# aerius-labs/indexed-merkle-tree-halo2

Hardware: AMD Instinct MI355X
Metric: indexed-tree insertions/sec at depth=32 (bn256::Fr) (higher is better)
Workload: dtype u32 limbs (9 x 29-bit, Montgomery mod p), 64-bit accumulate

## Files before the change

### indexed-merkle-tree-halo2_amd/csrc/imt_device.hpp

```cpp
#pragma once
#include <cstddef>
#include <cstdint>
#include "imt_consts.hpp"

#if defined(__HIPCC__)
#include <hip/hip_runtime.h>
#define IMT_HD __host__ __device__ __forceinline__
#else
#define IMT_HD inline
#endif

namespace imt {
namespace dev {

#define IMT_P29_0 0x10000001u
#define IMT_P29_1 0x1f0fac9fu
#define IMT_P29_2 0x0e5c2450u
#define IMT_P29_3 0x07d090f3u
#define IMT_P29_4 0x1585d283u
#define IMT_P29_5 0x02db40c0u
#define IMT_P29_6 0x00a6e141u
#define IMT_P29_7 0x0e5c2634u
#define IMT_P29_8 0x0030644eu
constexpr uint32_t N0INV29 = 0x0fffffffu;
constexpr uint32_t N0INV32 = 0xefffffffu;

IMT_HD constexpr uint32_t p29(int i) {
    return i == 0 ? IMT_P29_0 : i == 1 ? IMT_P29_1 : i == 2 ? IMT_P29_2 : i == 3 ? IMT_P29_3 :
           i == 4 ? IMT_P29_4 : i == 5 ? IMT_P29_5 : i == 6 ? IMT_P29_6 : i == 7 ? IMT_P29_7 : IMT_P29_8;
}


template <bool WIDE_M>
IMT_HD uint32_t mont_digit(uint64_t acc) {
    return WIDE_M ? (uint32_t)acc * N0INV32 : (((uint32_t)acc * N0INV29) & MASK29);
}

}
}
#if defined(__HIP_DEVICE_COMPILE__) && !defined(IMT_NO_MONT_ASM)
#define IMT_MONT_ASM 1
#include "imt_mont_asm.hpp"
#include "imt_mont_asm_rec.hpp"
#endif
namespace imt {
namespace dev {

template <int NT, bool ADD, bool WIDE_M = true>
IMT_HD void mont_dot(Fe& r, const Fe* a, const Fe* b, const Fe& addend) {
    uint32_t m[NL];
    uint64_t acc = 0;
#pragma unroll
    for (int k = 0; k < NL; k++) {
#pragma unroll
        for (int t = 0; t < NT; t++) {
#pragma unroll
            for (int i = 0; i <= k; i++) acc += (uint64_t)a[t].v[i] * b[t].v[k - i];
        }
#pragma unroll
        for (int i = 0; i < k; i++) acc += (uint64_t)m[i] * p29(k - i);
        m[k] = mont_digit<WIDE_M>(acc);
        acc += (uint64_t)m[k] * p29(0);
        acc >>= 29;
    }
#pragma unroll
    for (int k = NL; k < 2 * NL - 1; k++) {
#pragma unroll
        for (int t = 0; t < NT; t++) {
#pragma unroll
            for (int i = k - (NL - 1); i < NL; i++) acc += (uint64_t)a[t].v[i] * b[t].v[k - i];
        }
#pragma unroll
        for (int i = k - (NL - 1); i < NL; i++) acc += (uint64_t)m[i] * p29(k - i);
        if (ADD) acc += addend.v[k - NL];
        r.v[k - NL] = (uint32_t)acc & MASK29;
        acc >>= 29;
    }
    if (ADD) acc += addend.v[NL - 1];
    r.v[NL - 1] = (uint32_t)acc;
}

IMT_HD void mont_mul(Fe& r, const Fe& a, const Fe& b) {
#ifdef IMT_MONT_ASM
    masm::mul_vv(r, &a, &b);
#else
    mont_dot<1, false>(r, &a, &b, a);
#endif
}

template <int NT, bool ADD, bool WIDE_M = true>
IMT_HD void mont_dot_uc(Fe& r, const Fe* c, const Fe* v, const Fe& addend) {
#ifdef IMT_MONT_ASM
    static_assert((NT == 3 && !ADD && WIDE_M) || (NT == 4 && WIDE_M) || (NT == 2 && ADD && !WIDE_M),
                  "no assembly form for this shape");
    if constexpr (NT == 3) masm::dot3_uc(r, c, v);
    else if constexpr (NT == 4 && ADD) masm::dot4_add_uc(r, c, v, addend);
    else if constexpr (NT == 4) masm::dot4_uc(r, c, v);
    else masm::dot2_add_uc_narrow(r, c, v, addend);
#else
    mont_dot<NT, ADD, WIDE_M>(r, c, v, addend);
#endif
}

IMT_HD void mont_sqr(Fe& r, const Fe& a) {
#ifdef IMT_MONT_ASM
    masm::sqr_v(r, a);
    return;
#endif
    uint32_t m[NL], a2[NL];
#pragma unroll
    for (int i = 0; i < NL; i++) a2[i] = a.v[i] << 1;
    uint64_t acc = 0;
#pragma unroll
    for (int k = 0; k < NL; k++) {
#pragma unroll
        for (int i = 0; 2 * i < k; i++) acc += (uint64_t)a2[i] * a.v[k - i];
        if ((k & 1) == 0) acc += (uint64_t)a.v[k / 2] * a.v[k / 2];
#pragma unroll
        for (int i = 0; i < k; i++) acc += (uint64_t)m[i] * p29(k - i);
        m[k] = mont_digit<true>(acc);
        acc += (uint64_t)m[k] * p29(0);
        acc >>= 29;
    }
#pragma unroll
    for (int k = NL; k < 2 * NL - 1; k++) {
#pragma unroll
        for (int i = k - (NL - 1); 2 * i < k; i++) acc += (uint64_t)a2[i] * a.v[k - i];
        if ((k & 1) == 0) acc += (uint64_t)a.v[k / 2] * a.v[k / 2];
#pragma unroll
        for (int i = k - (NL - 1); i < NL; i++) acc += (uint64_t)m[i] * p29(k - i);
        r.v[k - NL] = (uint32_t)acc & MASK29;
        acc >>= 29;
    }
    r.v[NL - 1] = (uint32_t)acc;
}

IMT_HD void mont_redc(Fe& r, const Fe& a) {
    uint32_t m[NL];
    uint64_t acc = 0;
#pragma unroll
    for (int k = 0; k < NL; k++) {
        acc += a.v[k];
#pragma unroll
        for (int i = 0; i < k; i++) acc += (uint64_t)m[i] * p29(k - i);
        m[k] = mont_digit<false>(acc);
        acc += (uint64_t)m[k] * p29(0);
        acc >>= 29;
    }
#pragma unroll
    for (int k = NL; k < 2 * NL - 1; k++) {
#pragma unroll
        for (int i = k - (NL - 1); i < NL; i++) acc += (uint64_t)m[i] * p29(k - i);
        r.v[k - NL] = (uint32_t)acc & MASK29;
        acc >>= 29;
    }
    r.v[NL - 1] = (uint32_t)acc;
}

IMT_HD void add_lazy(Fe& r, const Fe& a, const Fe& b) {
#pragma unroll
    for (int i = 0; i < NL; i++) r.v[i] = a.v[i] + b.v[i];
}

IMT_HD void normalize(Fe& a) {
#pragma unroll
    for (int i = 0; i < NL - 1; i++) {
        a.v[i + 1] += a.v[i] >> 29;
        a.v[i] &= MASK29;
    }
}

IMT_HD bool geq_p(const Fe& a) {
    bool ge = true;
#pragma unroll
    for (int i = 0; i < NL; i++) {
        uint32_t pi = p29(i);
        if (a.v[i] != pi) ge = a.v[i] > pi;
    }
    return ge;
}

IMT_HD void sub_p(Fe& a) {
    uint32_t borrow = 0;
#pragma unroll
    for (int i = 0; i < NL; i++) {
        uint32_t d = a.v[i] - p29(i) - borrow;
        borrow = (i < NL - 1) ? (d >> 31) : 0;
        a.v[i] = (i < NL - 1) ? (d & MASK29) : d;
    }
}

template <int SH>
IMT_HD constexpr uint32_t p29_shl(int i) {
    return i == 0 ? ((p29(0) << SH) & MASK29)
         : i < NL - 1 ? (((p29(i) << SH) | (p29(i - 1) >> (29 - SH))) & MASK29)
                      : ((p29(i) << SH) | (p29(i - 1) >> (29 - SH)));
}
template <int SH>
IMT_HD void cond_sub_p_shl(Fe& a) {
    bool ge = true;
#pragma unroll
    for (int i = 0; i < NL; i++) {
        const uint32_t pi = p29_shl<SH>(i);
        if (a.v[i] != pi) ge = a.v[i] > pi;
    }
    if (ge) {
        uint32_t borrow = 0;
#pragma unroll
        for (int i = 0; i < NL; i++) {
            uint32_t d = a.v[i] - p29_shl<SH>(i) - borrow;
            borrow = (i < NL - 1) ? (d >> 31) : 0;
            a.v[i] = (i < NL - 1) ? (d & MASK29) : d;
        }
    }
}

IMT_HD void canonicalize(Fe& a) {
    cond_sub_p_shl<4>(a);
    cond_sub_p_shl<3>(a);
    cond_sub_p_shl<2>(a);
    cond_sub_p_shl<1>(a);
    cond_sub_p_shl<0>(a);
}

IMT_HD void unpack(Fe& r, const uint32_t w[8]) {
#pragma unroll
    for (int i = 0; i < NL; i++) {
        const int bit = 29 * i, wi = bit >> 5, sh = bit & 31;
        uint32_t lo = w[wi] >> sh;
        if (sh > 3 && wi + 1 < 8) lo |= w[wi + 1] << (32 - sh);
        r.v[i] = lo & MASK29;
    }
}
IMT_HD void pack(uint32_t w[8], const Fe& a) {
#pragma unroll
    for (int j = 0; j < 8; j++) {
        const int lo_limb = (32 * j) / 29, off = 32 * j - 29 * lo_limb;
        uint32_t x = a.v[lo_limb] >> off;
        const int have = 29 - off;
        if (have < 32 && lo_limb + 1 < NL) x |= a.v[lo_limb + 1] << have;
        if (have + 29 < 32 && lo_limb + 2 < NL) x |= a.v[lo_limb + 2] << (have + 29);
        w[j] = x;
    }
}

struct alignas(16) Word4 { uint32_t x, y, z, w; };
IMT_HD void load_packed(Fe& r, const void* ptr) {
    const Word4* q = reinterpret_cast<const Word4*>(ptr);
    Word4 x = q[0], y = q[1];
    uint32_t w[8] = {x.x, x.y, x.z, x.w, y.x, y.y, y.z, y.w};
    unpack(r, w);
}
IMT_HD void store_packed(void* ptr, const Fe& a) {
    uint32_t w[8];
    pack(w, a);
    Word4* q = reinterpret_cast<Word4*>(ptr);
    q[0] = Word4{w[0], w[1], w[2], w[3]};
    q[1] = Word4{w[4], w[5], w[6], w[7]};
}



IMT_HD void sbox(Fe& x) {
    Fe x2, x4;
    mont_sqr(x2, x);
    mont_sqr(x4, x2);
    mont_mul(x, x4, x);
}

IMT_HD constexpr uint32_t pc29(int i) { return i == 0 ? (1u << 29) - p29(0) : MASK29 - p29(i); }
constexpr uint32_t FOLD_RECIP = 1354;

IMT_HD void fold_p(Fe& a) {
    const uint32_t q = (uint32_t)(((uint64_t)a.v[NL - 1] * FOLD_RECIP) >> 32);
    uint64_t acc = 0;
#pragma unroll
    for (int i = 0; i < NL; i++) {
        acc = (acc >> 29) + a.v[i] + (uint64_t)q * pc29(i);
        a.v[i] = i < NL - 1 ? (uint32_t)acc & MASK29 : (uint32_t)(acc - ((uint64_t)q << 29));
    }
}

IMT_HD void permute(const PoseidonConsts& pc, Fe s[3], const Fe* first_rc) {
    constexpr int NSTEP = RF + RP;
    Fe z3;
#pragma unroll
    for (int i = 0; i < NL; i++) z3.v[i] = 0;
#pragma unroll 1
    for (int st = 0; st < NSTEP; st++) {
        if (st < RF / 2 || st >= RF / 2 + RP) {
            const int fr = st < RF / 2 ? st : st - RP;
            if (fr == RF / 2) {
                const Fe v[3] = {s[0], s[1], z3};
                const Fe zl = s[2];
#pragma unroll 1
                for (int i = 0; i < 2; i++) {
                    Fe n;
                    mont_dot_uc<3, false>(n, pc.rec_exit[i], v, v[0]);
                    add_lazy(n, n, zl);
                    normalize(n);
                    s[1] = s[2]; s[2] = n;
                }
            }
            const Fe* rc = (st == 0) ? first_rc : pc.sc_rc[fr];
            add_lazy(s[0], s[0], rc[0]);
            add_lazy(s[1], s[1], rc[1]);
            add_lazy(s[2], s[2], rc[2]);
            sbox(s[0]); sbox(s[1]); sbox(s[2]);
            const Fe(*mat)[3] = pc.sc_mats[fr];
            Fe n0, n1, n2;
            if (fr == 0 || fr == RF / 2) {
                mont_dot_uc<3, false>(n0, mat[0], s, s[0]);
            } else {
                add_lazy(n0, s[0], s[1]);
                add_lazy(n0, n0, s[2]);
                normalize(n0);
            }
            mont_dot_uc<3, false>(n1, mat[1], s, s[0]);
            mont_dot_uc<3, false>(n2, mat[2], s, s[0]);
            s[0] = n0; s[1] = n1; s[2] = n2;
        } else {
            const int r = st - RF / 2;
            Fe z, w;
            add_lazy(z, s[0], pc.rec_k[r]);
            sbox(z);
            if (r >= 2) {
                const Fe v[4] = {s[0], s[1], z3, s[2]};
                mont_dot_uc<4, true>(w, pc.rec_c[r], v, z);
            } else if (r == 1) {
                const Fe v[2] = {s[0], s[2]};
                Fe e;
                add_lazy(e, z3, z);
                mont_dot_uc<2, true, false>(w, pc.rec_c[1], v, e);
            } else {
                add_lazy(w, s[1], z);
                normalize(w);
            }
            s[1] = s[0]; s[0] = w; z3 = s[2]; s[2] = z;
        }
    }
}

IMT_HD void hash23(const PoseidonConsts& pc, Fe& out, const Fe& a, const Fe& b, const Fe& c, bool three) {
    Fe s[3] = {pc.cap0, a, b};
#pragma unroll 1
    for (int blk = 0; blk < 2; blk++) {
        const Fe* rc0 = pc.rc_full[0];
        if (blk == 1) {
            if (three) {
                add_lazy(s[1], s[1], c);
                add_lazy(s[2], s[2], pc.one);
                normalize(s[1]);
                normalize(s[2]);
            } else {
                rc0 = pc.rc_h2p2;
            }
        }
        permute(pc, s, rc0);
    }
    out = s[1];
    canonicalize(out);
}
IMT_HD void hash23_stashed(const PoseidonConsts& pc, Fe& out, const Fe& a, const Fe& b, bool three,
                           const uint32_t* stash, unsigned stride) {
    Fe s[3] = {pc.cap0, a, b};
#pragma unroll 1
    for (int blk = 0; blk < 2; blk++) {
        const Fe* rc0 = pc.rc_full[0];
        if (blk == 1) {
            if (three) {
                Fe c;
#pragma unroll
                for (int i = 0; i < NL; i++) c.v[i] = stash[(size_t)i * stride];
                add_lazy(s[1], s[1], c);
                add_lazy(s[2], s[2], pc.one);
                normalize(s[1]);
                normalize(s[2]);
            } else {
                rc0 = pc.rc_h2p2;
            }
        }
        permute(pc, s, rc0);
    }
    out = s[1];
    canonicalize(out);
}
template <class LoadInput>
IMT_HD void hash_sponge(const PoseidonConsts& pc, Fe& out, unsigned len, LoadInput load) {
    Fe s[3];
    s[0] = pc.cap0;
#pragma unroll
    for (int i = 0; i < NL; i++) s[1].v[i] = s[2].v[i] = 0;
    const unsigned full = len >> 1;
#pragma unroll 1
    for (unsigned ch = 0; ch <= full; ch++) {
        const Fe* rc0 = pc.rc_full[0];
        if (ch < full || (len & 1u)) {
            Fe x;
            load(2 * ch, x);
            add_lazy(s[1], s[1], x);
            normalize(s[1]);
            if (ch < full) load(2 * ch + 1, x);
            else x = pc.one;
            add_lazy(s[2], s[2], x);
            normalize(s[2]);
        } else {
            rc0 = pc.rc_h2p2;
        }
        permute(pc, s, rc0);
    }
    out = s[1];
    canonicalize(out);
}
IMT_HD void hash2(const PoseidonConsts& pc, Fe& out, const Fe& a, const Fe& b) { hash23(pc, out, a, b, a, false); }
IMT_HD void hash3(const PoseidonConsts& pc, Fe& out, const Fe& a, const Fe& b, const Fe& c) { hash23(pc, out, a, b, c, true); }

enum : unsigned { FMT_CANONICAL = 0, FMT_MONT256 = 1, FMT_DEVICE = 2 };

IMT_HD bool load_fe(const PoseidonConsts& pc, Fe& r, const void* ptr, unsigned fmt) {
    Fe raw;
    load_packed(raw, ptr);
    bool ok = !geq_p(raw) && (raw.v[NL - 1] >> 24) == 0;
    if (fmt == FMT_DEVICE) { r = raw; return ok; }
    mont_mul(r, raw, fmt == FMT_CANONICAL ? pc.from_canon : pc.from_mont256);
    canonicalize(r);
    return ok;
}
IMT_HD void store_fe(const PoseidonConsts& pc, void* ptr, const Fe& a, unsigned fmt) {
    if (fmt == FMT_DEVICE) { store_packed(ptr, a); return; }
    Fe t;
    mont_mul(t, a, fmt == FMT_CANONICAL ? pc.int_one : pc.to_mont256);
    canonicalize(t);
    store_packed(ptr, t);
}

IMT_HD bool fe_eq(const Fe& a, const Fe& b) {
    uint32_t d = 0;
#pragma unroll
    for (int i = 0; i < NL; i++) d |= a.v[i] ^ b.v[i];
    return d == 0;
}
IMT_HD bool fe_is_zero(const Fe& a) {
    uint32_t d = 0;
#pragma unroll
    for (int i = 0; i < NL; i++) d |= a.v[i];
    return d == 0;
}

}
}
```

### indexed-merkle-tree-halo2_amd/csrc/imt_kernels.hip

```cpp
#include <algorithm>
#include <hip/hip_runtime.h>
#include <hip/hip_ext.h>

#include "imt_device.hpp"
#include "imt_trace_device.hpp"
#include "imt_launch.hpp"
#include "imt_sweep.hpp"
#include "imt_resize.hpp"
#if defined(__HIP_DEVICE_COMPILE__)
#include "imt_coop_device.hpp"
#endif

namespace imt {

__constant__ dev::PoseidonConsts g_pc;
__constant__ dev::TraceConsts g_tc;

namespace {
using namespace dev;

#ifndef IMT_BLOCK
#define IMT_BLOCK 256
#endif
#ifndef IMT_HASH_WAVES
#define IMT_HASH_WAVES __attribute__((amdgpu_waves_per_eu(5, 5)))
#endif
#ifndef IMT_COOP_WAVES
#define IMT_COOP_WAVES __attribute__((amdgpu_waves_per_eu(1, 2)))
#endif
constexpr int BLOCK = IMT_BLOCK;

__device__ __forceinline__ size_t gtid() { return (size_t)blockIdx.x * blockDim.x + threadIdx.x; }
__device__ __forceinline__ size_t gtid_again() {
    uint32_t lo = blockIdx.x * blockDim.x + threadIdx.x, hi = (uint32_t)(((uint64_t)blockIdx.x * blockDim.x + threadIdx.x) >> 32);
    asm volatile("" : "+v"(lo), "+v"(hi));
    return ((size_t)hi << 32) | lo;
}
__device__ __forceinline__ void flag_err(int* err, bool ok) {
    if (!ok && err) atomicOr(err, 1);
}

__device__ __forceinline__ void to_int(Fe& r, const Fe& a) {
    mont_mul(r, a, g_pc.int_one);
    canonicalize(r);
}
__device__ __forceinline__ bool int_lt(const Fe& a, const Fe& b) {
    bool lt = false;
#pragma unroll
    for (int i = 0; i < NL; i++) {
        if (a.v[i] != b.v[i]) lt = a.v[i] < b.v[i];
    }
    return lt;
}
__device__ __forceinline__ void fe_from_u64(Fe& r, uint64_t x) {
    Fe t;
#pragma unroll
    for (int i = 0; i < NL; i++) t.v[i] = 0;
    t.v[0] = (uint32_t)x & MASK29;
    t.v[1] = (uint32_t)(x >> 29) & MASK29;
    t.v[2] = (uint32_t)(x >> 58);
    mont_mul(r, t, g_pc.from_canon);
    canonicalize(r);
}

__device__ __forceinline__ void order_pair(Fe& A, Fe& B, bool right, const Fe& cur, const Fe& sv) {
#pragma unroll
    for (int i = 0; i < NL; i++) {
        A.v[i] = right ? sv.v[i] : cur.v[i];
        B.v[i] = right ? cur.v[i] : sv.v[i];
    }
}
__device__ __forceinline__ void store_proof_row(const launch::SweepArgs& a, uint32_t e, const Fe& sv) {
    uint8_t* row = (e & 1u) ? a.new_sib : a.low_sib;
    if (row) store_fe(g_pc, row + ((uint64_t)a.level * a.lay.level_stride + (uint64_t)(e >> 1) * a.lay.item_stride) * 32, sv, a.fmt_out);
}
struct InsertRows {
    __device__ __forceinline__ void operator()(const launch::SweepArgs& a, uint32_t e, const Fe& sv) const { store_proof_row(a, e, sv); }
};
struct MixedRows {
    const uint32_t* erow;
    uint8_t* read_sib;
    __device__ __forceinline__ void operator()(const launch::SweepArgs& a, uint32_t e, const Fe& sv) const {
        const uint32_t w = erow[e], kind = w & 3u;
        uint8_t* row = kind == 0u ? a.low_sib : (kind == 1u ? a.new_sib : read_sib);
        if (row) store_fe(g_pc, row + ((uint64_t)a.level * a.lay.level_stride + (uint64_t)(w >> 2) * a.lay.item_stride) * 32, sv, a.fmt_out);
    }
};

struct NoLevelHook {
    __device__ __forceinline__ void operator()(unsigned, const Fe&, const Fe&) const {}
    __device__ __forceinline__ void operator()(unsigned, const Fe&) const {}
};
struct NoLeafHook {
    __device__ __forceinline__ void operator()(const Fe&) const {}
};
template <class LoadLeaf, class OnLeaf = NoLeafHook, class OnLevel = NoLevelHook>
__device__ __forceinline__ void chain_inline(Fe& cur, bool with_leaf, LoadLeaf load_leaf, OnLeaf on_leaf,
                                             const uint64_t* __restrict__ index, uint64_t flip, const uint8_t* sib,
                                             launch::SibLayout lay, unsigned depth, unsigned fmt_in, bool& ok, uint32_t* stash,
                                             OnLevel on_level = OnLevel()) {
#pragma unroll 1
    for (int it = with_leaf ? -1 : 0; it < (int)depth; it++) {
        Fe A, B;
        const bool three = it < 0;
        if (three) {
            Fe C;
            load_leaf(A, B, C, ok);
#pragma unroll
            for (int i = 0; i < NL; i++) stash[(size_t)i * BLOCK] = C.v[i];
        } else {
            const size_t item = gtid_again();
            Fe sv;
            ok &= load_fe(g_pc, sv, sib + ((uint64_t)it * lay.level_stride + item * lay.item_stride) * 32, fmt_in);
            order_pair(A, B, ((index[item] ^ flip) >> it) & 1, cur, sv);
            on_level((unsigned)it, A, B);
        }
        hash23_stashed(g_pc, cur, A, B, three, stash, BLOCK);
        if (three) on_leaf(cur);
    }
}
struct LeafAt {
    const uint8_t* base;
    unsigned fmt_in;
    __device__ __forceinline__ void operator()(Fe& a, Fe& b, Fe& c, bool& ok) const {
        const uint8_t* p = base + gtid_again() * 96;
        ok &= load_fe(g_pc, a, p, fmt_in);
        ok &= load_fe(g_pc, b, p + 32, fmt_in);
        ok &= load_fe(g_pc, c, p + 64, fmt_in);
    }
};

#if defined(__HIP_DEVICE_COMPILE__)
__device__ __forceinline__ bool leaf_inputs_quad(Fe& X, Fe& C3, const uint8_t* p, unsigned fmt, unsigned ri) {
    Fe seen;
    bool ok = load_fe(g_pc, X, p + (ri == 2u ? 32 : 0), fmt);
    ok &= load_fe(g_pc, C3, p + 64, fmt);
    if (ri == 1u) ok &= load_fe(g_pc, seen, p + 32, fmt);
    return ok;
}
__device__ __forceinline__ void pick_input(Fe& X, unsigned ri, bool right, const Fe& cur, const Fe& sv) {
    coop::sel(X, (ri == 2u) != right, sv, cur);
}
__device__ __forceinline__ void hash_to_quad(const uint32_t* tab, Fe& cur, const Fe& X, const Fe& C3, bool three, unsigned ri) {
    Fe o;
    coop::hash23(tab, o, X, C3, three, ri);
    coop::quad_bcast<1>(cur, o);
}
__device__ __forceinline__ void leaf_start_quad(const uint32_t* tab, Fe& cur, const uint8_t* p, unsigned fmt, unsigned ri, bool& ok) {
    Fe X, C3;
    ok &= leaf_inputs_quad(X, C3, p, fmt, ri);
    hash_to_quad(tab, cur, X, C3, true, ri);
}
template <class OnLevel = NoLevelHook>
__device__ __forceinline__ void chain_quad(const uint32_t* tab, Fe& cur, uint64_t idx, const uint8_t* sib, launch::SibLayout lay,
                                           size_t item, unsigned depth, unsigned fmt_in, unsigned ri, bool& ok,
                                           OnLevel on_level = OnLevel()) {
#pragma unroll 1
    for (unsigned l = 0; l < depth; l++) {
        Fe sv, X;
        ok &= load_fe(g_pc, sv, sib + ((uint64_t)l * lay.level_stride + item * lay.item_stride) * 32, fmt_in);
        pick_input(X, ri, (idx >> l) & 1, cur, sv);
        on_level(l, X);
        hash_to_quad(tab, cur, X, X, false, ri);
    }
}
#endif

__global__ IMT_HASH_WAVES void __launch_bounds__(BLOCK) k_hash_batch(const uint8_t* __restrict__ in, uint8_t* __restrict__ out,
                                                      size_t n, int arity, unsigned fmt_in, unsigned fmt_out,
                                                      int* err) {
    const size_t i = gtid();
    if (i >= n) return;
    const uint8_t* p = in + i * 32 * (size_t)arity;
    __shared__ uint32_t stash[NL][BLOCK];
    Fe a, b, o;
    bool ok = load_fe(g_pc, a, p, fmt_in);
    ok &= load_fe(g_pc, b, p + 32, fmt_in);
    if (arity == 3) {
        Fe c;
        ok &= load_fe(g_pc, c, p + 64, fmt_in);
#pragma unroll
        for (int q = 0; q < NL; q++) stash[q][threadIdx.x] = c.v[q];
    }
    hash23_stashed(g_pc, o, a, b, arity == 3, &stash[0][threadIdx.x], BLOCK);
    store_fe(g_pc, out + i * 32, o, fmt_out);
    flag_err(err, ok);
}

__global__ IMT_HASH_WAVES void __launch_bounds__(BLOCK) k_hash_batch_coop(const uint8_t* __restrict__ in, uint8_t* __restrict__ out,
                                                           size_t n, int arity, unsigned fmt_in, unsigned fmt_out,
                                                           int* err) {
#if defined(__HIP_DEVICE_COMPILE__)
    __shared__ uint32_t tab[coop::TAB_DWORDS];
    coop::tab_fill(tab, g_pc);
    const size_t t = gtid();
    const size_t i = t >> 2;
    if (i >= n) return;
    const unsigned role = (unsigned)t & 3u, ri = role == 3u ? 0u : role;
    const uint8_t* p = in + i * 32 * (size_t)arity;
    Fe X, C3, o;
    C3 = g_pc.one;
    bool ok = load_fe(g_pc, X, p + (ri == 2u ? 32 : 0), fmt_in);
    if (ri == 1u) ok &= load_fe(g_pc, o, p + 32, fmt_in);
    if (arity == 3) ok &= load_fe(g_pc, C3, p + 64, fmt_in);
    coop::hash23(tab, o, X, C3, arity == 3, ri);
    if (role == 1u) store_fe(g_pc, out + i * 32, o, fmt_out);
    flag_err(err, ok);
#endif
}

__global__ void __launch_bounds__(BLOCK) k_permute_batch(const uint8_t* __restrict__ in, uint8_t* __restrict__ out,
                                                         size_t n, unsigned fmt_in, unsigned fmt_out, int* err) {
    const size_t i = gtid();
    if (i >= n) return;
    Fe s[3];
    bool ok = true;
#pragma unroll
    for (int j = 0; j < 3; j++) ok &= load_fe(g_pc, s[j], in + (i * 3 + j) * 32, fmt_in);
    permute(g_pc, s, g_pc.rc_full[0]);
#pragma unroll
    for (int j = 0; j < 3; j++) {
        canonicalize(s[j]);
        store_fe(g_pc, out + (i * 3 + j) * 32, s[j], fmt_out);
    }
    flag_err(err, ok);
}

__global__ void __launch_bounds__(BLOCK) k_convert(const uint8_t* __restrict__ in, uint8_t* __restrict__ out, size_t n,
                                                   unsigned fmt_in, unsigned fmt_out, int* err) {
    const size_t i = gtid();
    if (i >= n) return;
    Fe x;
    bool ok = load_fe(g_pc, x, in + i * 32, fmt_in);
    store_fe(g_pc, out + i * 32, x, fmt_out);
    flag_err(err, ok);
}

#ifndef IMT_TRACE_WAVES
#define IMT_TRACE_WAVES
#endif
template <unsigned FMT_OUT>
__global__ IMT_TRACE_WAVES void __launch_bounds__(BLOCK) k_hash_trace(launch::TraceJobs a) {
    const launch::TraceJobs::Job jb = a.j[blockIdx.y];
    const size_t q = gtid();
    if (q >= jb.n_items) return;
    const uint8_t* p = jb.in + q * 32 * (size_t)jb.arity;
    Fe x, y, z;
    bool ok = load_fe(g_pc, x, p, jb.fmt_in);
    ok &= load_fe(g_pc, y, p + 32, jb.fmt_in);
    z = x;
    if (jb.arity == 3) ok &= load_fe(g_pc, z, p + 64, jb.fmt_in);
    const size_t l = q / a.n_per, i = q - l * a.n_per;
    const size_t first = jb.row0 + l * (size_t)(jb.arity == 3 ? TRACE_ROWS_H3 : TRACE_ROWS_H2);
    TraceSink o{a.item_major ? a.trace + (i * a.rows_total + first) * 32 : a.trace + (first * a.n_per + i) * 32,
                a.item_major ? (uint64_t)32 : (uint64_t)a.n_per * 32};
    hash_trace<FMT_OUT>(g_pc, g_tc, o, x, y, z, jb.arity == 3);
    flag_err(a.err, ok);
}

__global__ __attribute__((amdgpu_waves_per_eu(4, 5))) void __launch_bounds__(BLOCK) k_path_pairs(launch::PathChains a) {
    const size_t i = gtid();
    if (i >= a.n) return;
    const launch::PathChains::Chain ch = a.c[blockIdx.y];
    __shared__ uint32_t stash[NL][BLOCK];
    bool ok = true;
    Fe cur;
    if (!ch.leaf3) ok &= load_fe(g_pc, cur, ch.leaf + i * 32, a.fmt_in);
    uint8_t* const pairs = ch.pairs;
    const size_t n = a.n;
    auto store_pair = [pairs, n](unsigned l, const Fe& x, const Fe& y) {
        uint8_t* dst = pairs + ((size_t)l * n + gtid_again()) * 64;
        store_packed(dst, x);
        store_packed(dst + 32, y);
    };
    chain_inline(cur, ch.leaf3 != nullptr, LeafAt{ch.leaf3, a.fmt_in}, NoLeafHook(), ch.index, 0, ch.sib, a.lay, a.depth,
                 a.fmt_in, ok, &stash[0][threadIdx.x], store_pair);
    if (ch.root_out) store_fe(g_pc, ch.root_out + gtid_again() * 32, cur, a.fmt_out);
    flag_err(a.err, ok);
}

__global__ IMT_COOP_WAVES void __launch_bounds__(BLOCK) k_path_pairs_coop(launch::PathChains a) {
#if defined(__HIP_DEVICE_COMPILE__)
    __shared__ uint32_t tab[coop::TAB_DWORDS];
    coop::tab_fill(tab, g_pc);
    const size_t t = gtid();
    const size_t i = t >> 2;
    if (i >= a.n) return;
    const launch::PathChains::Chain ch = a.c[blockIdx.y];
    const unsigned role = (unsigned)t & 3u, ri = role == 3u ? 0u : role;
    bool ok = true;
    Fe cur;
    if (ch.leaf3) leaf_start_quad(tab, cur, ch.leaf3 + i * 96, a.fmt_in, ri, ok);
    else ok &= load_fe(g_pc, cur, ch.leaf + i * 32, a.fmt_in);
    uint8_t* const pairs = ch.pairs;
    const size_t n = a.n;
    auto store_input = [pairs, n, i, role](unsigned l, const Fe& X) {
        if (role == 1u || role == 2u) store_packed(pairs + ((size_t)l * n + i) * 64 + (role == 2u ? 32 : 0), X);
    };
    chain_quad(tab, cur, ch.index[i], ch.sib, a.lay, i, a.depth, a.fmt_in, ri, ok, store_input);
    if (role == 1u && ch.root_out) store_fe(g_pc, ch.root_out + i * 32, cur, a.fmt_out);
    flag_err(a.err, ok);
#endif
}

__global__ void __launch_bounds__(BLOCK)
k_insert_trace_inputs(const uint8_t* __restrict__ low_leaf, const uint8_t* __restrict__ new_leaf,
                      const uint64_t* __restrict__ new_index, size_t n, uint8_t* __restrict__ new_low,
                      uint8_t* __restrict__ zero_leaf, unsigned fmt, int* err) {
    const size_t i = gtid();
    if (i >= n) return;
    Fe a, b, c;
    bool ok = load_fe(g_pc, a, low_leaf + (i * 3 + 0) * 32, fmt);
    ok &= load_fe(g_pc, b, new_leaf + (i * 3 + 0) * 32, fmt);
    fe_from_u64(c, new_index[i]);
    store_fe(g_pc, new_low + (i * 3 + 0) * 32, a, fmt);
    store_fe(g_pc, new_low + (i * 3 + 1) * 32, b, fmt);
    store_fe(g_pc, new_low + (i * 3 + 2) * 32, c, fmt);
    store_fe(g_pc, zero_leaf + i * 32, g_pc.zero_leaf, fmt);
    flag_err(err, ok);
}

__global__ IMT_HASH_WAVES void __launch_bounds__(BLOCK)
k_path_root(const uint8_t* __restrict__ leaf, const uint8_t* __restrict__ leaf3, const uint64_t* __restrict__ index,
            int is_helper, const uint8_t* __restrict__ sib, launch::SibLayout lay, unsigned depth, size_t n,
            uint8_t* __restrict__ root_out, const uint8_t* __restrict__ expect, unsigned expect_stride,
            uint8_t* __restrict__ ok_out, unsigned fmt_in, unsigned fmt_out, int* err) {
    const size_t i0 = gtid();
    if (i0 >= n) return;
    __shared__ uint32_t stash[NL][BLOCK];
    bool ok = true;
    Fe cur;
    if (!leaf3) ok &= load_fe(g_pc, cur, leaf + i0 * 32, fmt_in);
    chain_inline(cur, leaf3 != nullptr, LeafAt{leaf3, fmt_in}, NoLeafHook(), index, is_helper ? ~(uint64_t)0 : 0, sib, lay, depth,
                 fmt_in, ok, &stash[0][threadIdx.x]);
    const size_t i = gtid_again();
    if (root_out) store_fe(g_pc, root_out + i * 32, cur, fmt_out);
    if (ok_out) {
        Fe e;
        ok &= load_fe(g_pc, e, expect + i * (size_t)expect_stride, fmt_in);
        ok_out[i] = fe_eq(cur, e) ? 1 : 0;
    }
    flag_err(err, ok);
}

__global__ IMT_COOP_WAVES void __launch_bounds__(BLOCK)
k_path_root_coop(const uint8_t* __restrict__ leaf, const uint8_t* __restrict__ leaf3, const uint64_t* __restrict__ index,
                 int is_helper, const uint8_t* __restrict__ sib, launch::SibLayout lay, unsigned depth, size_t n,
                 uint8_t* __restrict__ root_out, const uint8_t* __restrict__ expect, unsigned expect_stride,
                 uint8_t* __restrict__ ok_out, unsigned fmt_in, unsigned fmt_out, int* err) {
#if defined(__HIP_DEVICE_COMPILE__)
    __shared__ uint32_t tab[coop::TAB_DWORDS];
    coop::tab_fill(tab, g_pc);
    const size_t t = gtid();
    const size_t i = t >> 2;
    if (i >= n) return;
    const unsigned role = (unsigned)t & 3u, ri = role == 3u ? 0u : role;
    bool ok = true;
    Fe cur;
    if (leaf3) leaf_start_quad(tab, cur, leaf3 + i * 96, fmt_in, ri, ok);
    else ok &= load_fe(g_pc, cur, leaf + i * 32, fmt_in);
    chain_quad(tab, cur, is_helper ? ~index[i] : index[i], sib, lay, i, depth, fmt_in, ri, ok);
    if (role == 1u) {
        if (root_out) store_fe(g_pc, root_out + i * 32, cur, fmt_out);
        if (ok_out) {
            Fe e;
            ok &= load_fe(g_pc, e, expect + i * (size_t)expect_stride, fmt_in);
            ok_out[i] = fe_eq(cur, e) ? 1 : 0;
        }
    }
    flag_err(err, ok);
#endif
}

__device__ __forceinline__ unsigned range_fail(const Fe& low_val, const Fe& low_next, const Fe& new_val, const uint8_t* is_largest) {
    Fe nvi, lvi, lni;
    to_int(nvi, new_val); to_int(lvi, low_val); to_int(lni, low_next);
    const unsigned s = *is_largest;
    unsigned fail = 0;
    if (s > 1) fail |= 0x80;
    if (!(s ? fe_is_zero(low_next) : int_lt(nvi, lni))) fail |= 0x01;
    if (!int_lt(lvi, nvi)) fail |= 0x04;
    return fail;
}
__global__ IMT_HASH_WAVES void __launch_bounds__(BLOCK)
k_non_membership(const uint8_t* __restrict__ root, unsigned root_stride, const uint8_t* __restrict__ low_leaf,
                 const uint64_t* __restrict__ low_index, const uint8_t* __restrict__ sib, launch::SibLayout lay,
                 unsigned depth, const uint8_t* __restrict__ new_val, const uint8_t* __restrict__ is_largest,
                 size_t n, uint8_t* __restrict__ fail_out, uint8_t* __restrict__ root_out, unsigned fmt_in,
                 unsigned fmt_out, int* err) {
    const size_t i0 = gtid();
    if (i0 >= n) return;
    bool ok = true;
    unsigned fail = 0;
    __shared__ uint32_t stash[NL][BLOCK];
    Fe cur;
    chain_inline(cur, true, LeafAt{low_leaf, fmt_in}, NoLeafHook(), low_index, 0, sib, lay, depth, fmt_in, ok,
                 &stash[0][threadIdx.x]);
    const size_t i = gtid_again();
    {
        Fe rt;
        ok &= load_fe(g_pc, rt, root + i * (size_t)root_stride, fmt_in);
        if (!fe_eq(cur, rt)) fail |= 0x02;
    }
    if (root_out) store_fe(g_pc, root_out + i * 32, cur, fmt_out);
    fail_out[i] = (uint8_t)fail;
    flag_err(err, ok);
}
__global__ void __launch_bounds__(BLOCK)
k_non_membership_pred(const uint8_t* __restrict__ low_leaf, const uint8_t* __restrict__ new_val, const uint8_t* __restrict__ is_largest,
                      size_t n, uint8_t* __restrict__ fail_out, unsigned fmt_in, int* err) {
    const size_t i = gtid();
    if (i >= n) return;
    Fe v, nx, nv;
    bool ok = load_fe(g_pc, v, low_leaf + (i * 3 + 0) * 32, fmt_in);
    ok &= load_fe(g_pc, nx, low_leaf + (i * 3 + 1) * 32, fmt_in);
    ok &= load_fe(g_pc, nv, new_val + i * 32, fmt_in);
    fail_out[i] |= (uint8_t)range_fail(v, nx, nv, is_largest + i);
    flag_err(err, ok);
}

__global__ IMT_COOP_WAVES void __launch_bounds__(BLOCK)
k_non_membership_coop(const uint8_t* __restrict__ root, unsigned root_stride, const uint8_t* __restrict__ low_leaf,
                      const uint64_t* __restrict__ low_index, const uint8_t* __restrict__ sib, launch::SibLayout lay,
                      unsigned depth, const uint8_t* __restrict__ new_val, const uint8_t* __restrict__ is_largest,
                      size_t n, uint8_t* __restrict__ fail_out, uint8_t* __restrict__ root_out, unsigned fmt_in,
                      unsigned fmt_out, int* err) {
#if defined(__HIP_DEVICE_COMPILE__)
    __shared__ uint32_t tab[coop::TAB_DWORDS];
    coop::tab_fill(tab, g_pc);
    const size_t t = gtid();
    const size_t i = t >> 2;
    if (i >= n) return;
    const unsigned role = (unsigned)t & 3u, ri = role == 3u ? 0u : role;
    bool ok = true;
    unsigned fail;
    {
        Fe v, nx, nv;
        ok &= load_fe(g_pc, v, low_leaf + (i * 3 + 0) * 32, fmt_in);
        ok &= load_fe(g_pc, nx, low_leaf + (i * 3 + 1) * 32, fmt_in);
        ok &= load_fe(g_pc, nv, new_val + i * 32, fmt_in);
        fail = range_fail(v, nx, nv, is_largest + i);
    }
    Fe cur;
    leaf_start_quad(tab, cur, low_leaf + i * 96, fmt_in, ri, ok);
    chain_quad(tab, cur, low_index[i], sib, lay, i, depth, fmt_in, ri, ok);
    if (role == 1u) {
        Fe rt;
        ok &= load_fe(g_pc, rt, root + i * (size_t)root_stride, fmt_in);
        if (!fe_eq(cur, rt)) fail |= 0x02;
        fail_out[i] = (uint8_t)fail;
        if (root_out) store_fe(g_pc, root_out + i * 32, cur, fmt_out);
    }
    flag_err(err, ok);
#endif
}

__global__ void __launch_bounds__(BLOCK) k_split128(const uint8_t* __restrict__ vals, uint8_t* __restrict__ q,
                                                    uint8_t* __restrict__ r, size_t n, unsigned fmt, int* err) {
    const size_t i = gtid();
    if (i >= n) return;
    Fe x, xi;
    bool ok = load_fe(g_pc, x, vals + i * 32, fmt);
    to_int(xi, x);
    uint32_t w[8];
    pack(w, xi);
    Fe lo, hi, t;
    const uint32_t wl[8] = {w[0], w[1], w[2], w[3], 0, 0, 0, 0};
    const uint32_t wh[8] = {w[4], w[5], w[6], w[7], 0, 0, 0, 0};
    unpack(t, wl);
    mont_mul(lo, t, g_pc.from_canon);
    canonicalize(lo);
    unpack(t, wh);
    mont_mul(hi, t, g_pc.from_canon);
    canonicalize(hi);
    store_fe(g_pc, r + i * 32, lo, fmt);
    store_fe(g_pc, q + i * 32, hi, fmt);
    flag_err(err, ok);
}

__global__ IMT_HASH_WAVES void __launch_bounds__(BLOCK)
k_insert_chains(const uint8_t* __restrict__ low_leaf, const uint64_t* __restrict__ low_index,
                const uint8_t* __restrict__ low_sib, const uint8_t* __restrict__ new_leaf,
                const uint64_t* __restrict__ new_index, const uint64_t* __restrict__ new_path_index,
                const uint8_t* __restrict__ new_sib, launch::SibLayout lay, unsigned depth, size_t n,
                uint8_t* __restrict__ trace, unsigned fmt_in, int* err) {
    const size_t i = gtid();
    if (i >= n) return;
    const int chain = blockIdx.y;
    __shared__ uint32_t stash[NL][BLOCK];
    bool ok = true;
    Fe cur;
    const uint8_t* sib = chain < 2 ? low_sib : new_sib;
    const uint64_t* index = chain < 2 ? low_index : new_path_index;
    const int leaf_row = chain == 0 ? 0 : chain == 1 ? 2 : 5, root_row = chain == 0 ? 1 : chain == 1 ? 3 : chain == 2 ? 4 : 6;
    if (chain == 2) cur = g_pc.zero_leaf;
    auto load_leaf = [=](Fe& a, Fe& b, Fe& c, bool& okk) {
        const size_t it = gtid_again();
        const uint8_t* const p0 = (chain == 3 ? new_leaf : low_leaf) + it * 96;
        okk &= load_fe(g_pc, a, p0, fmt_in);
        if (chain == 1) {
            okk &= load_fe(g_pc, b, new_leaf + it * 96, fmt_in);
            fe_from_u64(c, new_index[it]);
        } else {
            okk &= load_fe(g_pc, b, p0 + 32, fmt_in);
            okk &= load_fe(g_pc, c, p0 + 64, fmt_in);
        }
    };
    auto store_leaf = [=](const Fe& h) { store_packed(trace + ((size_t)leaf_row * n + gtid_again()) * 32, h); };
    chain_inline(cur, chain != 2, load_leaf, store_leaf, index, 0, sib, lay, depth, fmt_in, ok, &stash[0][threadIdx.x]);
    store_packed(trace + ((size_t)root_row * n + gtid_again()) * 32, cur);
    flag_err(err, ok);
}

__global__ IMT_COOP_WAVES void __launch_bounds__(BLOCK)
k_insert_chains_coop(const uint8_t* __restrict__ low_leaf, const uint64_t* __restrict__ low_index,
                     const uint8_t* __restrict__ low_sib, const uint8_t* __restrict__ new_leaf,
                     const uint64_t* __restrict__ new_index, const uint64_t* __restrict__ new_path_index,
                     const uint8_t* __restrict__ new_sib, launch::SibLayout lay, unsigned depth, size_t n,
                     uint8_t* __restrict__ trace, unsigned fmt_in, int* err) {
#if defined(__HIP_DEVICE_COMPILE__)
    __shared__ uint32_t tab[coop::TAB_DWORDS];
    coop::tab_fill(tab, g_pc);
    const size_t t = gtid();
    const size_t i = t >> 2;
    if (i >= n) return;
    const unsigned role = (unsigned)t & 3u, ri = role == 3u ? 0u : role;
    const int chain = blockIdx.y;
    bool ok = true;
    const uint8_t* sib = chain < 2 ? low_sib : new_sib;
    const uint64_t idx = chain < 2 ? low_index[i] : new_path_index[i];
    uint8_t* leaf_out = nullptr;
    uint8_t* root_out;
    Fe cur;
    if (chain == 2) {
        cur = g_pc.zero_leaf;
        root_out = trace + (4 * n + i) * 32;
    } else {
        Fe X, C3;
        if (chain == 1) {
            ok &= load_fe(g_pc, X, (ri == 2u ? new_leaf : low_leaf) + (i * 3 + 0) * 32, fmt_in);
            fe_from_u64(C3, new_index[i]);
            leaf_out = trace + (2 * n + i) * 32;
            root_out = trace + (3 * n + i) * 32;
        } else {
            const uint8_t* lf = chain == 0 ? low_leaf : new_leaf;
            ok &= leaf_inputs_quad(X, C3, lf + i * 96, fmt_in, ri);
            leaf_out = trace + ((chain == 0 ? 0 : 5) * n + i) * 32;
            root_out = trace + ((chain == 0 ? 1 : 6) * n + i) * 32;
        }
        hash_to_quad(tab, cur, X, C3, true, ri);
        if (role == 1u) store_packed(leaf_out, cur);
    }
    chain_quad(tab, cur, idx, sib, lay, i, depth, fmt_in, ri, ok);
    if (role == 1u) store_packed(root_out, cur);
    flag_err(err, ok);
#endif
}

__global__ void __launch_bounds__(BLOCK)
k_insert_check(const uint8_t* __restrict__ old_root, const uint8_t* __restrict__ low_leaf,
               const uint8_t* __restrict__ new_root, const uint8_t* __restrict__ new_leaf,
               const uint8_t* __restrict__ is_largest, size_t n, const uint8_t* __restrict__ trace,
               uint8_t* __restrict__ fail_out, unsigned fmt_in, int* err) {
    const size_t i = gtid();
    if (i >= n) return;
    bool ok = true;
    Fe low[3], nl[3], r0, r1, t;
#pragma unroll
    for (int j = 0; j < 3; j++) {
        ok &= load_fe(g_pc, low[j], low_leaf + (i * 3 + j) * 32, fmt_in);
        ok &= load_fe(g_pc, nl[j], new_leaf + (i * 3 + j) * 32, fmt_in);
    }
    ok &= load_fe(g_pc, r0, old_root + i * 32, fmt_in);
    ok &= load_fe(g_pc, r1, new_root + i * 32, fmt_in);
    unsigned fail = range_fail(low[0], low[1], nl[0], is_largest + i);
    load_packed(t, trace + (1 * n + i) * 32);
    if (!fe_eq(t, r0)) fail |= 0x02;
    Fe interim, z;
    load_packed(interim, trace + (3 * n + i) * 32);
    load_packed(z, trace + (4 * n + i) * 32);
    if (!fe_eq(z, interim)) fail |= 0x08;
    if (!fe_eq(nl[1], low[1])) fail |= 0x10;
    if (!fe_eq(nl[2], low[2])) fail |= 0x20;
    load_packed(t, trace + (6 * n + i) * 32);
    if (!fe_eq(t, r1)) fail |= 0x40;
    fail_out[i] = (uint8_t)fail;
    flag_err(err, ok);
}

__global__ IMT_HASH_WAVES void __launch_bounds__(BLOCK) k_tree_level(const uint8_t* __restrict__ prev, uint8_t* __restrict__ next,
                                                      size_t n_parents) {
    const size_t i = gtid();
    if (i >= n_parents) return;
    Fe a, b, o;
    load_packed(a, prev + (2 * i) * 32);
    load_packed(b, prev + (2 * i + 1) * 32);
    hash23_stashed(g_pc, o, a, b, false, nullptr, 0);
    store_packed(next + i * 32, o);
}

__global__ IMT_HASH_WAVES void __launch_bounds__(BLOCK) k_index_leaves(const uint8_t* __restrict__ val,
                                                        const uint32_t* __restrict__ sorted, uint32_t M, uint64_t base,
                                                        uint8_t* __restrict__ tree0, int* err) {
    const size_t r = gtid();
    if (r >= M) return;
    __shared__ uint32_t stash[NL][BLOCK];
    Fe a, b, o;
    bool ok;
    {
        const bool last = r + 1 == M;
        const uint32_t su = last ? 0u : sorted[r + 1];
        Fe c;
        fe_from_u64(c, last ? 0 : base + su);
#pragma unroll
        for (int q = 0; q < NL; q++) stash[q][threadIdx.x] = c.v[q];
        ok = load_fe(g_pc, b, val + (size_t)su * 32, FMT_CANONICAL);
    }
    ok &= load_fe(g_pc, a, val + (size_t)sorted[r] * 32, FMT_CANONICAL);
    hash23_stashed(g_pc, o, a, b, true, &stash[0][threadIdx.x], BLOCK);
    store_packed(tree0 + (size_t)sorted[gtid_again()] * 32, o);
    flag_err(err, ok);
}

__device__ __forceinline__ void force_vector(Fe& x) {
#pragma unroll
    for (int i = 0; i < NL; i++) asm volatile("" : "+v"(x.v[i]));
}

__global__ IMT_HASH_WAVES void k_zero_chain(uint8_t* out, unsigned depth) {
#if defined(__HIP_DEVICE_COMPILE__)
    __shared__ uint32_t tab[coop::TAB_DWORDS];
    coop::tab_fill(tab, g_pc);
    if (blockIdx.x != 0 || threadIdx.x >= 4) return;
    const unsigned role = threadIdx.x, ri = role == 3u ? 0u : role;
    Fe cur = g_pc.zero_leaf;
    force_vector(cur);
    if (role == 1u) store_packed(out, cur);
#pragma unroll 1
    for (unsigned l = 0; l < depth; l++) {
        Fe o;
        coop::hash23(tab, o, cur, cur, false, ri);
        coop::quad_bcast<1>(cur, o);
        if (role == 1u) store_packed(out + (size_t)(l + 1) * 32, cur);
    }
#endif
}

__global__ IMT_HASH_WAVES void k_extend_root(uint8_t* cur_io, const uint8_t* zero, unsigned from, unsigned to) {
    if (threadIdx.x != 0 || blockIdx.x != 0) return;
    Fe cur;
    load_packed(cur, cur_io);
    force_vector(cur);
#pragma unroll 1
    for (unsigned l = from; l < to; l++) {
        Fe z, o;
        load_packed(z, zero + (size_t)l * 32);
        hash23_stashed(g_pc, o, cur, z, false, nullptr, 0);
        cur = o;
    }
    store_packed(cur_io, cur);
}

__global__ void __launch_bounds__(BLOCK) k_gather_proof(launch::TreeView tv, const uint64_t* __restrict__ index,
                                                        size_t n, unsigned depth, uint8_t* __restrict__ out,
                                                        launch::SibLayout lay, unsigned fmt_out) {
    const size_t t = gtid();
    if (t >= n * depth) return;
    const size_t i = t % n;
    const unsigned l = (unsigned)(t / n);
    const uint64_t s = ((index[i] - tv.index_base) >> l) ^ 1;
    const uint8_t* src = s < tv.len[l] ? tv.nodes + (tv.off[l] + s) * 32 : tv.zero + (size_t)l * 32;
    Fe x;
    load_packed(x, src);
    store_fe(g_pc, out + ((uint64_t)l * lay.level_stride + i * lay.item_stride) * 32, x, fmt_out);
}

__global__ void k_write_helpers(uint64_t index, unsigned depth, uint8_t* out, unsigned fmt_out) {
    const unsigned l = threadIdx.x + blockIdx.x * blockDim.x;
    if (l >= depth) return;
    Fe x;
    fe_from_u64(x, ((index >> l) & 1) ? 0 : 1);
    store_fe(g_pc, out + (size_t)l * 32, x, fmt_out);
}


__global__ void __launch_bounds__(BLOCK) k_fill_level(uint8_t* __restrict__ nodes, size_t n,
                                                      const uint8_t* __restrict__ zero_l) {
    const size_t i = gtid();
    if (i >= n) return;
    const Word4* z = reinterpret_cast<const Word4*>(zero_l);
    Word4* o = reinterpret_cast<Word4*>(nodes + i * 32);
    o[0] = z[0];
    o[1] = z[1];
}

__global__ void __launch_bounds__(BLOCK) k_restride_levels(const uint8_t* __restrict__ old_nodes,
                                                           const uint64_t* __restrict__ old_off,
                                                           const uint64_t* __restrict__ old_len,
                                                           uint8_t* __restrict__ new_nodes,
                                                           const uint64_t* __restrict__ new_off, uint64_t new_total,
                                                           const uint8_t* __restrict__ zero, unsigned depth) {
    const size_t pieces = (size_t)new_total * 2, step = (size_t)gridDim.x * blockDim.x;
    for (size_t p = gtid(); p < pieces; p += step) {
        unsigned l;
        const uint64_t src = resize::source_of(new_off, old_off, old_len, depth, p >> 1, &l);
        const uint8_t* row = src != ~(uint64_t)0 ? old_nodes + src * 32 : zero + (size_t)l * 32;
        reinterpret_cast<Word4*>(new_nodes)[p] = reinterpret_cast<const Word4*>(row)[p & 1];
    }
}

__global__ void __launch_bounds__(BLOCK) k_merge_level(sweep::LevelTable in, sweep::LevelOut out, uint32_t total) {
    const size_t k = gtid();
    if (k >= total) return;
    sweep::merge_element(in, out, (uint32_t)k, total);
}

__global__ void __launch_bounds__(BLOCK)
k_writeback(const uint8_t* __restrict__ val_l, const uint32_t* __restrict__ from,
            const uint32_t* __restrict__ node_below, uint8_t* __restrict__ tree_l, uint32_t total) {
    const size_t kp = gtid();
    if (kp >= total) return;
    const uint32_t f = from[kp];
    if (!(f & sweep::LAST_BIT)) return;
    const Word4* s = reinterpret_cast<const Word4*>(val_l + (size_t)(f & ~sweep::LAST_BIT) * 32);
    Word4* d = reinterpret_cast<Word4*>(tree_l + (size_t)node_below[kp] * 32);
    d[0] = s[0];
    d[1] = s[1];
}

struct StoredSibling {
    __device__ __forceinline__ const uint8_t* operator()(const launch::SweepArgs& a, int32_t ss, uint64_t sn) const {
        return ss >= 0 ? a.val_in + (size_t)ss * 32 : (sn < a.len_l ? a.tree_l + sn * 32 : a.zero_l);
    }
};
struct ViewSibling {
    const view::Side& side;
    __device__ __forceinline__ const uint8_t* operator()(const launch::SweepArgs& a, int32_t ss, uint64_t sn) const {
        return replay::sibling_row(side, ss, a.level, sn, a.val_in, a.tree_l, a.len_l, a.zero_l);
    }
};
#if defined(__HIP_DEVICE_COMPILE__)
template <bool TABLES, class Sibling, class Rows = InsertRows>
__device__ __forceinline__ void sweep_body_quad(const launch::SweepArgs& a, Sibling sibling, uint32_t* tab, Rows rows = Rows()) {
    coop::tab_fill(tab, g_pc);
    const size_t t = gtid();
    const size_t q = t >> 2;
    if (q >= a.count) return;
    const unsigned role = (unsigned)t & 3u, ri = role == 3u ? 0u : role;
    const uint32_t x = a.begin + (uint32_t)q;
    const bool leaves = !TABLES && a.mode == launch::SWEEP_LEAVES;
    Fe X, C3, o;
    C3 = g_pc.one;
    if (leaves) {
        flag_err(a.err, leaf_inputs_quad(X, C3, a.pre + (size_t)a.time0[x] * 96, a.fmt_in, ri));
    } else {
        uint32_t k = x, n = 0, e = x;
        const uint8_t* sp = a.zero_l;
        if (TABLES || a.from) {
            k = a.from[x] & ~sweep::LAST_BIT;
            n = a.node_below[x];
            e = a.time_next[x];
            sp = sibling(a, a.sibsrc[x], (uint64_t)(n ^ 1u));
        }
        Fe cur, sv;
        load_packed(cur, a.val_in + (size_t)k * 32);
        load_packed(sv, sp);
        pick_input(X, ri, n & 1u, cur, sv);
        if (role == 0u) {
            if (!TABLES && x == a.last_event && a.node_in) store_packed(a.node_in, cur);
            rows(a, e, sv);
        }
    }
    coop::hash23(tab, o, X, C3, leaves, ri);
    if (role == 1u) {
        store_packed(a.val_out + (size_t)x * 32, o);
        if (!TABLES && x == a.last_event && a.node_out) store_packed(a.node_out, o);
    }
}
#endif
__global__ IMT_HASH_WAVES void __launch_bounds__(BLOCK) k_sweep(launch::SweepArgs a) {
    __shared__ uint32_t stash[NL][BLOCK];
    const size_t t = gtid();
    if (t >= a.count) return;
    const uint32_t x = a.begin + (uint32_t)t;
    Fe A, B, o;
    if (a.mode == launch::SWEEP_LEAVES) {
        const uint8_t* p = a.pre + (size_t)a.time0[x] * 96;
        Fe C;
        bool ok = load_fe(g_pc, A, p, a.fmt_in);
        ok &= load_fe(g_pc, B, p + 32, a.fmt_in);
        ok &= load_fe(g_pc, C, p + 64, a.fmt_in);
#pragma unroll
        for (int i = 0; i < NL; i++) stash[i][threadIdx.x] = C.v[i];
        flag_err(a.err, ok);
    } else {
        uint32_t k = x, n = 0, e = x;
        const uint8_t* sp = a.zero_l;
        if (a.from) {
            k = a.from[x] & ~sweep::LAST_BIT;
            n = a.node_below[x];
            e = a.time_next[x];
            const int32_t ss = a.sibsrc[x];
            const uint64_t sn = (uint64_t)(n ^ 1u);
            sp = ss >= 0 ? a.val_in + (size_t)ss * 32 : (sn < a.len_l ? a.tree_l + sn * 32 : a.zero_l);
        }
        Fe cur, sv;
        load_packed(cur, a.val_in + (size_t)k * 32);
        load_packed(sv, sp);
        if (x == a.last_event && a.node_in) store_packed(a.node_in, cur);
        const bool right = n & 1u;
#pragma unroll
        for (int i = 0; i < NL; i++) {
            A.v[i] = right ? sv.v[i] : cur.v[i];
            B.v[i] = right ? cur.v[i] : sv.v[i];
        }
        uint8_t* row = (e & 1u) ? a.new_sib : a.low_sib;
        if (row) store_fe(g_pc, row + ((uint64_t)a.level * a.lay.level_stride + (uint64_t)(e >> 1) * a.lay.item_stride) * 32, sv, a.fmt_out);
    }
    hash23_stashed(g_pc, o, A, B, a.mode == launch::SWEEP_LEAVES, &stash[0][threadIdx.x], BLOCK);
    store_packed(a.val_out + (size_t)x * 32, o);
    if (x == a.last_event && a.node_out) store_packed(a.node_out, o);
}

__global__ IMT_HASH_WAVES void __launch_bounds__(BLOCK) k_sweep_coop(launch::SweepArgs a) {
#if defined(__HIP_DEVICE_COMPILE__)
    __shared__ uint32_t tab[coop::TAB_DWORDS];
    sweep_body_quad<false>(a, StoredSibling(), tab);
#endif
}

__global__ IMT_HASH_WAVES void __launch_bounds__(BLOCK) k_sweep_mixed(launch::SweepMixedArgs m) {
    const launch::SweepArgs& a = m.sweep;
    const size_t t = gtid();
    if (t >= a.count) return;
    const uint32_t x = a.begin + (uint32_t)t;
    uint32_t k = x, n = 0, e = x;
    const uint8_t* sp = a.zero_l;
    if (a.from) {
        k = a.from[x] & ~sweep::LAST_BIT;
        n = a.node_below[x];
        e = a.time_next[x];
        sp = StoredSibling()(a, a.sibsrc[x], (uint64_t)(n ^ 1u));
    }
    Fe A, B, o, cur, sv;
    load_packed(cur, a.val_in + (size_t)k * 32);
    load_packed(sv, sp);
    if (x == a.last_event && a.node_in) store_packed(a.node_in, cur);
    order_pair(A, B, n & 1u, cur, sv);
    MixedRows{m.erow, m.read_sib}(a, e, sv);
    hash23_stashed(g_pc, o, A, B, false, nullptr, 0);
    store_packed(a.val_out + (size_t)x * 32, o);
    if (x == a.last_event && a.node_out) store_packed(a.node_out, o);
}

__global__ IMT_HASH_WAVES void __launch_bounds__(BLOCK) k_sweep_mixed_coop(launch::SweepMixedArgs m) {
#if defined(__HIP_DEVICE_COMPILE__)
    __shared__ uint32_t tab[coop::TAB_DWORDS];
    sweep_body_quad<false>(m.sweep, StoredSibling(), tab, MixedRows{m.erow, m.read_sib});
#endif
}

__global__ void __launch_bounds__(BLOCK)
k_emit_roots_mixed(const uint8_t* __restrict__ val, uint32_t total, const uint32_t* __restrict__ erow, uint32_t n_ins,
                   uint8_t* __restrict__ old_root, uint8_t* __restrict__ interim_root, uint8_t* __restrict__ new_root,
                   uint8_t* __restrict__ read_root, unsigned fmt_out, uint8_t* __restrict__ node_store) {
    const size_t t = gtid();
    if (t >= total) return;
    const uint32_t e = (uint32_t)t;
    Fe cur;
    load_packed(cur, val + (size_t)e * 32);
    if (e == total - 1 && node_store) store_packed(node_store, cur);
    const uint32_t w = erow[e], kind = w & 3u;
    const size_t i = w >> 2;
    if (kind == 1u) {
        if (new_root) store_fe(g_pc, new_root + i * 32, cur, fmt_out);
        if (old_root && i + 1 < (size_t)n_ins) store_fe(g_pc, old_root + (i + 1) * 32, cur, fmt_out);
    } else if (kind == 0u) {
        if (interim_root) store_fe(g_pc, interim_root + i * 32, cur, fmt_out);
    } else {
        if (read_root) store_fe(g_pc, read_root + i * 32, cur, fmt_out);
    }
}

__global__ void __launch_bounds__(BLOCK)
k_emit_roots(const uint8_t* __restrict__ val, uint32_t e_begin, uint32_t e_count, uint32_t total,
             uint8_t* __restrict__ old_root, uint8_t* __restrict__ interim_root, uint8_t* __restrict__ new_root,
             unsigned fmt_out, uint8_t* __restrict__ roots_dev, uint8_t* __restrict__ node_store) {
    const size_t t = gtid();
    if (t >= e_count) return;
    const uint32_t e = e_begin + (uint32_t)t;
    Fe cur;
    load_packed(cur, val + (size_t)e * 32);
    if (e == total - 1 && node_store) store_packed(node_store, cur);
    if (roots_dev) { store_packed(roots_dev + (size_t)e * 32, cur); return; }
    const uint32_t i = e >> 1;
    if (e & 1u) {
        if (new_root) store_fe(g_pc, new_root + (size_t)i * 32, cur, fmt_out);
        if (old_root && (size_t)i + 1 < (size_t)(total >> 1)) store_fe(g_pc, old_root + ((size_t)i + 1) * 32, cur, fmt_out);
    } else {
        if (interim_root) store_fe(g_pc, interim_root + (size_t)i * 32, cur, fmt_out);
    }
}

__global__ void __launch_bounds__(BLOCK)
k_emit_roots_bulk(const uint8_t* __restrict__ val, uint32_t total, uint8_t* __restrict__ root_before,
                  uint8_t* __restrict__ root_after, unsigned fmt_out, uint8_t* __restrict__ node_store) {
    const size_t t = gtid();
    if (t >= total) return;
    Fe cur;
    load_packed(cur, val + t * 32);
    if (t == total - 1 && node_store) store_packed(node_store, cur);
    if (root_after) store_fe(g_pc, root_after + t * 32, cur, fmt_out);
    if (root_before && t + 1 < total) store_fe(g_pc, root_before + (t + 1) * 32, cur, fmt_out);
}

__global__ void k_gather_frontier(launch::TreeView tv, uint64_t index, unsigned depth, uint8_t* __restrict__ out,
                                  unsigned fmt_out) {
    const unsigned l = threadIdx.x + blockIdx.x * blockDim.x;
    if (l >= depth) return;
    const uint64_t p = index >> l, s = p ^ 1;
    const uint8_t* src = ((p & 1) && s < tv.len[l]) ? tv.nodes + (tv.off[l] + s) * 32 : tv.zero + (size_t)l * 32;
    Fe x;
    load_packed(x, src);
    store_fe(g_pc, out + (size_t)l * 32, x, fmt_out);
}

__global__ void k_bulk_frontier_base(view::Side sd, launch::TreeView tv, unsigned depth, uint8_t* __restrict__ out) {
    const unsigned l = threadIdx.x + blockIdx.x * blockDim.x;
    if (l >= depth) return;
    const uint8_t* zero_l = tv.zero + (size_t)l * 32;
    const uint8_t* src = replay::frontier_base(sd.size, l) == replay::FRONTIER_VIEW
                             ? view::node_row(sd, l, replay::frontier_node(sd.size, l), tv.nodes + tv.off[l] * 32, tv.len[l], zero_l)
                             : zero_l;
    const Word4* s = reinterpret_cast<const Word4*>(src);
    Word4* d = reinterpret_cast<Word4*>(out + (size_t)l * 32);
    d[0] = s[0];
    d[1] = s[1];
}
__global__ void __launch_bounds__(BLOCK)
k_bulk_frontier_level(uint64_t size, unsigned l, const uint8_t* __restrict__ val_l, const uint32_t* __restrict__ from,
                      const uint32_t* __restrict__ node_below, uint32_t total, uint8_t* __restrict__ out_l) {
    const size_t kp = gtid();
    if (kp >= total) return;
    uint32_t slot;
    if (!replay::frontier_version(size, l, from[kp], node_below[kp], slot) || slot >= total) return;
    const Word4* s = reinterpret_cast<const Word4*>(val_l + (size_t)slot * 32);
    Word4* d = reinterpret_cast<Word4*>(out_l);
    d[0] = s[0];
    d[1] = s[1];
}

__global__ void k_frontier_bounds(launch::FrontierArgs a) {
    const unsigned l = threadIdx.x + blockIdx.x * blockDim.x;
    if (l == 0) {
        a.idx[0] = a.start;
        a.idx[1] = a.start >> a.top;
    }
    if (l > a.depth) return;
    const uint64_t first = a.start >> l, last = (a.start + a.n - 1) >> l;
    const bool left = first & 1;
    Fe x, z;
    load_packed(z, a.zero + (size_t)l * 32);
    x = z;
    if (l < a.depth) {
        if (left) flag_err(a.err, load_fe(g_pc, x, a.sib + (size_t)l * 32, a.fmt_in));
        store_packed(a.fsib + (size_t)l * 32, x);
    }
    if (l > a.top) return;
    uint8_t* row = a.rows + a.off[l] * 32;
    if (left) store_packed(row, x);
    if (!(last & 1)) store_packed(row + (last - (first & ~(uint64_t)1) + 1) * 32, z);
}

#if defined(__HIP_DEVICE_COMPILE__)
template <class Rule, class Args>
__device__ __forceinline__ void listed_body_quad(const Args& a, uint32_t* tab) {
    coop::tab_fill(tab, g_pc);
    const size_t t = gtid();
    const size_t j = t >> 2;
    if (j >= a.bound || j >= *a.count) return;
    const unsigned role = (unsigned)t & 3u, ri = role == 3u ? 0u : role;
    const uint64_t p = a.list[j];
    if (p >= a.len_out) return;
    const Rule rule{a};
    Fe X, C3, o;
    C3 = g_pc.one;
    if (a.mode == launch::APPLY_LEAVES) {
        flag_err(a.err, leaf_inputs_quad(X, C3, a.pre + (size_t)a.src[j] * 96, a.fmt_in, ri));
    } else {
        load_packed(X, rule.child(2 * p + (ri == 2u ? 1u : 0u)));
    }
    coop::hash23(tab, o, X, C3, a.mode == launch::APPLY_LEAVES, ri);
    if (role == 1u) store_packed(rule.out(j, p), o);
}
#endif
struct StoredLevel {
    const launch::ApplyArgs& a;
    __device__ __forceinline__ const uint8_t* child(uint64_t c) const { return c < a.len_in ? a.tree_in + c * 32 : a.zero_in; }
    __device__ __forceinline__ uint8_t* out(size_t, uint64_t p) const { return a.tree_out + p * 32; }
};
struct ViewLevel {
    const launch::ViewArgs& a;
    __device__ __forceinline__ const uint8_t* child(uint64_t c) const {
        return view::node_row(a.side, a.level_in, c, a.tree_in, a.len_in, a.zero_in);
    }
    __device__ __forceinline__ uint8_t* out(size_t j, uint64_t) const { return a.out + j * 32; }
};

__global__ IMT_HASH_WAVES void __launch_bounds__(BLOCK) k_apply_level(launch::ApplyArgs a) {
    __shared__ uint32_t stash[NL][BLOCK];
    const size_t j = gtid();
    if (j >= a.bound || j >= *a.count) return;
    const uint64_t p = a.list[j];
    if (p >= a.len_out) return;
    Fe A, B, o;
    if (a.mode == launch::APPLY_LEAVES) {
        const uint8_t* q = a.pre + (size_t)a.src[j] * 96;
        Fe C;
        bool ok = load_fe(g_pc, A, q, a.fmt_in);
        ok &= load_fe(g_pc, B, q + 32, a.fmt_in);
        ok &= load_fe(g_pc, C, q + 64, a.fmt_in);
#pragma unroll
        for (int i = 0; i < NL; i++) stash[i][threadIdx.x] = C.v[i];
        flag_err(a.err, ok);
    } else {
        const uint64_t c0 = 2 * p, c1 = 2 * p + 1;
        load_packed(A, c0 < a.len_in ? a.tree_in + c0 * 32 : a.zero_in);
        load_packed(B, c1 < a.len_in ? a.tree_in + c1 * 32 : a.zero_in);
    }
    hash23_stashed(g_pc, o, A, B, a.mode == launch::APPLY_LEAVES, &stash[0][threadIdx.x], BLOCK);
    store_packed(a.tree_out + p * 32, o);
}

__global__ IMT_HASH_WAVES void __launch_bounds__(BLOCK) k_apply_level_coop(launch::ApplyArgs a) {
#if defined(__HIP_DEVICE_COMPILE__)
    __shared__ uint32_t tab[coop::TAB_DWORDS];
    listed_body_quad<StoredLevel>(a, tab);
#endif
}

#if defined(__HIP_DEVICE_COMPILE__)
template <class Store>
__device__ __forceinline__ void node0_chain_quad(uint32_t* tab, const uint8_t* first, const uint8_t* first_sib,
                                                 const uint8_t* __restrict__ zero, unsigned from, unsigned to, Store store) {
    coop::tab_fill(tab, g_pc);
    if (blockIdx.x != 0 || threadIdx.x >= 4) return;
    const unsigned role = threadIdx.x, ri = role == 3u ? 0u : role;
    Fe cur;
    load_packed(cur, first);
#pragma unroll 1
    for (unsigned l = from; l < to; l++) {
        Fe z, X, o;
        load_packed(z, l == from ? first_sib : zero + (size_t)l * 32);
        coop::sel(X, ri == 2u, z, cur);
        coop::hash23(tab, o, X, X, false, ri);
        coop::quad_bcast<1>(cur, o);
        if (role == 1u) store_packed(store(l + 1), cur);
    }
}
struct StoredPair {
    const uint8_t *first, *sib;
    __device__ __forceinline__ StoredPair(const uint8_t* nodes, const uint64_t* off, const uint64_t* len, const uint8_t* zero,
                                          unsigned from)
        : first(nodes + off[from] * 32), sib(len[from] > 1 ? nodes + (off[from] + 1) * 32 : zero + (size_t)from * 32) {}
};
#endif

__global__ IMT_HASH_WAVES void k_apply_top(uint8_t* nodes, const uint64_t* __restrict__ off, const uint64_t* __restrict__ len,
                                           const uint8_t* __restrict__ zero, unsigned from, unsigned to) {
#if defined(__HIP_DEVICE_COMPILE__)
    __shared__ uint32_t tab[coop::TAB_DWORDS];
    const StoredPair p(nodes, off, len, zero, from);
    node0_chain_quad(tab, p.first, p.sib, zero, from, to, [&](unsigned l) { return nodes + off[l] * 32; });
#endif
}

__global__ IMT_HASH_WAVES void k_apply_chain(const uint8_t* __restrict__ nodes, const uint64_t* __restrict__ off,
                                             const uint64_t* __restrict__ len, const uint8_t* __restrict__ zero,
                                             uint8_t* __restrict__ chain, unsigned from, unsigned to) {
#if defined(__HIP_DEVICE_COMPILE__)
    __shared__ uint32_t tab[coop::TAB_DWORDS];
    const StoredPair p(nodes, off, len, zero, from);
    node0_chain_quad(tab, p.first, p.sib, zero, from, to, [&](unsigned l) { return chain + (size_t)l * 32; });
#endif
}

__global__ void __launch_bounds__(BLOCK) k_apply_chain_store(const uint32_t* __restrict__ chain, uint32_t* __restrict__ nodes,
                                                             const uint64_t* __restrict__ off, unsigned from, unsigned to,
                                                             uint32_t* __restrict__ root) {
    const size_t t = gtid();
    const unsigned l = from + (unsigned)(t >> 3), w = (unsigned)t & 7u;
    if (l > to) return;
    const uint32_t x = chain[(size_t)l * 8 + w];
    nodes[off[l] * 8 + w] = x;
    if (l == to) root[w] = x;
}

__global__ IMT_HASH_WAVES void __launch_bounds__(BLOCK) k_view_level(launch::ViewArgs a) {
    __shared__ uint32_t stash[NL][BLOCK];
    const size_t j = gtid();
    if (j >= a.bound || j >= *a.count) return;
    const uint64_t p = a.list[j];
    if (p >= a.len_out) return;
    Fe A, B, o;
    if (a.mode == launch::APPLY_LEAVES) {
        const uint8_t* q = a.pre + (size_t)a.src[j] * 96;
        Fe C;
        bool ok = load_fe(g_pc, A, q, a.fmt_in);
        ok &= load_fe(g_pc, B, q + 32, a.fmt_in);
        ok &= load_fe(g_pc, C, q + 64, a.fmt_in);
#pragma unroll
        for (int i = 0; i < NL; i++) stash[i][threadIdx.x] = C.v[i];
        flag_err(a.err, ok);
    } else {
        load_packed(A, view::node_row(a.side, a.level_in, 2 * p, a.tree_in, a.len_in, a.zero_in));
        load_packed(B, view::node_row(a.side, a.level_in, 2 * p + 1, a.tree_in, a.len_in, a.zero_in));
    }
    hash23_stashed(g_pc, o, A, B, a.mode == launch::APPLY_LEAVES, &stash[0][threadIdx.x], BLOCK);
    store_packed(a.out + j * 32, o);
}

__global__ IMT_HASH_WAVES void __launch_bounds__(BLOCK) k_view_level_coop(launch::ViewArgs a) {
#if defined(__HIP_DEVICE_COMPILE__)
    __shared__ uint32_t tab[coop::TAB_DWORDS];
    listed_body_quad<ViewLevel>(a, tab);
#endif
}

__global__ IMT_HASH_WAVES void k_view_top(view::Side sd, launch::TreeView tv, uint8_t* chain, unsigned from, unsigned to) {
#if defined(__HIP_DEVICE_COMPILE__)
    __shared__ uint32_t tab[coop::TAB_DWORDS];
    const uint8_t* stored = tv.nodes + tv.off[from] * 32;
    const uint8_t* zf = tv.zero + (size_t)from * 32;
    node0_chain_quad(tab, view::node_row(sd, from, 0, stored, tv.len[from], zf), view::node_row(sd, from, 1, stored, tv.len[from], zf),
                     tv.zero, from, to, [&](unsigned l) { return chain + (size_t)l * 32; });
#endif
}

__global__ void __launch_bounds__(BLOCK) k_view_gather_proof(view::Side sd, launch::TreeView tv,
                                                             const uint64_t* __restrict__ index, size_t n, unsigned depth,
                                                             uint8_t* __restrict__ out, launch::SibLayout lay,
                                                             unsigned fmt_out) {
    const size_t t = gtid();
    if (t >= n * depth) return;
    const size_t i = t % n;
    const unsigned l = (unsigned)(t / n);
    const uint64_t s = ((index[i] - tv.index_base) >> l) ^ 1;
    Fe x;
    load_packed(x, view::node_row(sd, l, s, tv.nodes + tv.off[l] * 32, tv.len[l], tv.zero + (size_t)l * 32));
    store_fe(g_pc, out + ((uint64_t)l * lay.level_stride + i * lay.item_stride) * 32, x, fmt_out);
}

__global__ IMT_HASH_WAVES void __launch_bounds__(BLOCK) k_sweep_view(launch::SweepViewArgs v) {
    const launch::SweepArgs& a = v.sweep;
    const size_t t = gtid();
    if (t >= a.count) return;
    const uint32_t x = a.begin + (uint32_t)t;
    const uint32_t k = a.from[x] & ~sweep::LAST_BIT, n = a.node_below[x], e = a.time_next[x];
    const uint8_t* sp = ViewSibling{v.side}(a, a.sibsrc[x], (uint64_t)(n ^ 1u));
    Fe A, B, o, cur, sv;
    load_packed(cur, a.val_in + (size_t)k * 32);
    load_packed(sv, sp);
    order_pair(A, B, n & 1u, cur, sv);
    store_proof_row(a, e, sv);
    hash23_stashed(g_pc, o, A, B, false, nullptr, 0);
    store_packed(a.val_out + (size_t)x * 32, o);
}

__global__ IMT_HASH_WAVES void __launch_bounds__(BLOCK) k_sweep_view_coop(launch::SweepViewArgs v) {
#if defined(__HIP_DEVICE_COMPILE__)
    __shared__ uint32_t tab[coop::TAB_DWORDS];
    sweep_body_quad<true>(v.sweep, ViewSibling{v.side}, tab);
#endif
}

__global__ IMT_HASH_WAVES void __launch_bounds__(BLOCK) k_sweep_view_mixed(launch::SweepViewMixedArgs v) {
    const launch::SweepArgs& a = v.sweep;
    const size_t t = gtid();
    if (t >= a.count) return;
    const uint32_t x = a.begin + (uint32_t)t;
    const uint32_t k = a.from[x] & ~sweep::LAST_BIT, n = a.node_below[x], e = a.time_next[x];
    const uint8_t* sp = ViewSibling{v.side}(a, a.sibsrc[x], (uint64_t)(n ^ 1u));
    Fe A, B, o, cur, sv;
    load_packed(cur, a.val_in + (size_t)k * 32);
    load_packed(sv, sp);
    order_pair(A, B, n & 1u, cur, sv);
    MixedRows{v.erow, v.read_sib}(a, e, sv);
    hash23_stashed(g_pc, o, A, B, false, nullptr, 0);
    store_packed(a.val_out + (size_t)x * 32, o);
}

__global__ IMT_HASH_WAVES void __launch_bounds__(BLOCK) k_sweep_view_mixed_coop(launch::SweepViewMixedArgs v) {
#if defined(__HIP_DEVICE_COMPILE__)
    __shared__ uint32_t tab[coop::TAB_DWORDS];
    sweep_body_quad<true>(v.sweep, ViewSibling{v.side}, tab, MixedRows{v.erow, v.read_sib});
#endif
}

__global__ IMT_HASH_WAVES void __launch_bounds__(BLOCK)
k_lift_roots(uint8_t* __restrict__ old_root, uint8_t* __restrict__ interim_root, uint8_t* __restrict__ new_root,
             uint32_t n, const uint8_t* __restrict__ top, uint64_t pos_bits, unsigned levels, unsigned fmt, int* err) {
    const size_t t = gtid();
    const uint32_t n_int = interim_root ? n : 0, n_new = new_root ? n : 0;
    const uint32_t n_old = old_root ? (new_root ? 1u : n) : 0;
    if (t >= (size_t)n_int + n_new + n_old) return;
    uint8_t* row;
    uint8_t* also = nullptr;
    if (t < n_int) {
        row = interim_root + t * 32;
    } else if (t < (size_t)n_int + n_new) {
        const size_t i = t - n_int;
        row = new_root + i * 32;
        if (old_root && i + 1 < n) also = old_root + (i + 1) * 32;
    } else {
        row = old_root + (t - n_int - n_new) * 32;
    }
    Fe cur;
    bool ok = load_fe(g_pc, cur, row, fmt);
#pragma unroll 1
    for (unsigned j = 0; j < levels; j++) {
        Fe sv, a, b, o;
        load_packed(sv, top + (size_t)j * 32);
        order_pair(a, b, (pos_bits >> j) & 1, cur, sv);
        hash23_stashed(g_pc, o, a, b, false, nullptr, 0);
        cur = o;
    }
    store_fe(g_pc, row, cur, fmt);
    if (also) store_fe(g_pc, also, cur, fmt);
    flag_err(err, ok);
}

__global__ void __launch_bounds__(BLOCK)
k_fill_sib_rows(uint8_t* __restrict__ sib, launch::SibLayout lay, unsigned first_level, unsigned levels, uint32_t n,
                const uint8_t* __restrict__ top, unsigned fmt_out) {
    const size_t t = gtid();
    if (t >= (size_t)n * levels) return;
    const uint32_t i = (uint32_t)(t % n);
    const unsigned j = (unsigned)(t / n);
    Fe x;
    load_packed(x, top + (size_t)j * 32);
    store_fe(g_pc, sib + ((uint64_t)(first_level + j) * lay.level_stride + (uint64_t)i * lay.item_stride) * 32, x, fmt_out);
}

__global__ void k_mix_roots(const uint8_t* __restrict__ before, const uint8_t* __restrict__ after,
                            uint8_t* __restrict__ mixed, uint32_t n_sub, uint32_t self, unsigned fmt_in, int* err) {
    const uint32_t r = blockIdx.x * blockDim.x + threadIdx.x;
    if (r >= n_sub) return;
    Fe x;
    const bool ok = load_fe(g_pc, x, (r < self ? after : before) + (size_t)r * 32, fmt_in);
    store_packed(mixed + (size_t)r * 32, x);
    flag_err(err, ok);
}

__global__ void k_pick_top(const uint8_t* __restrict__ levels_buf, uint32_t n_sub, uint32_t self, unsigned k,
                           unsigned levels, const uint8_t* __restrict__ zero, unsigned sub_depth,
                           uint8_t* __restrict__ top) {
    const unsigned j = threadIdx.x;
    if (j >= levels) return;
    const uint8_t* src;
    if (j < k) {
        const size_t off = 2 * (size_t)n_sub - ((2 * (size_t)n_sub) >> j);
        src = levels_buf + (off + ((self >> j) ^ 1u)) * 32;
    } else {
        src = zero + (size_t)(sub_depth + j) * 32;
    }
    const Word4* s4 = reinterpret_cast<const Word4*>(src);
    Word4* d4 = reinterpret_cast<Word4*>(top + (size_t)j * 32);
    d4[0] = s4[0];
    d4[1] = s4[1];
}

__global__ void __launch_bounds__(BLOCK) k_slot0(const uint32_t* __restrict__ time0, uint32_t* __restrict__ slot0,
                                                 uint32_t total) {
    const size_t k = gtid();
    if (k < total) slot0[time0[k]] = (uint32_t)k;
}

struct ExtractArgs {
    const uint8_t* const* val;
    const uint32_t* slot;
    const int32_t* sibsrc;
    const uint32_t* node_below;
    size_t stride;
    const uint8_t* tree_nodes;
    const uint64_t* tree_off;
    const uint64_t* tree_len;
    const uint8_t* zero;
    const uint8_t* roots;
    unsigned l0, depth;
    uint32_t ins_begin, ins_count, n_total;
    uint8_t *old_root, *interim_root, *new_root, *low_sib, *new_sib;
    launch::SibLayout lay;
    unsigned fmt_out;
};
__global__ void __launch_bounds__(BLOCK) k_extract(ExtractArgs a) {
    const size_t t = gtid();
    const size_t per = (size_t)a.depth + 1;
    if (t >= (size_t)a.ins_count * 2 * per) return;
    const uint32_t ev_local = (uint32_t)(t % ((size_t)a.ins_count * 2));
    const unsigned task = (unsigned)(t / ((size_t)a.ins_count * 2));
    const uint32_t i_local = ev_local >> 1, odd = ev_local & 1u;
    const uint32_t e = (a.ins_begin + i_local) * 2 + odd;
    Fe x;
    if (task == a.depth) {
        load_packed(x, a.roots + (size_t)e * 32);
        if (odd) {
            if (a.new_root) store_fe(g_pc, a.new_root + (size_t)i_local * 32, x, a.fmt_out);
        } else {
            if (a.interim_root) store_fe(g_pc, a.interim_root + (size_t)i_local * 32, x, a.fmt_out);
            if (a.old_root) {
                Fe o;
                if (e > 0) load_packed(o, a.roots + (size_t)(e - 1) * 32);
                else load_packed(o, a.tree_nodes + a.tree_off[a.depth] * 32);
                store_fe(g_pc, a.old_root + (size_t)i_local * 32, o, a.fmt_out);
            }
        }
        return;
    }
    uint8_t* dst = odd ? a.new_sib : a.low_sib;
    if (!dst) return;
    const unsigned l = task;
    const uint8_t* sp;
    if (l < a.l0) {
        const uint32_t kp = a.slot[(size_t)(l + 1) * a.stride + e];
        const int32_t ss = a.sibsrc[(size_t)l * a.stride + kp];
        const uint64_t sn = (uint64_t)(a.node_below[(size_t)l * a.stride + kp] ^ 1u);
        sp = ss >= 0 ? a.val[l] + (size_t)ss * 32
                     : (sn < a.tree_len[l] ? a.tree_nodes + (a.tree_off[l] + sn) * 32 : a.zero + (size_t)l * 32);
    } else {
        sp = a.zero + (size_t)l * 32;
    }
    load_packed(x, sp);
    store_fe(g_pc, dst + ((uint64_t)l * a.lay.level_stride + (uint64_t)i_local * a.lay.item_stride) * 32, x, a.fmt_out);
}

__global__ void __launch_bounds__(BLOCK)
k_pack_writeback(const uint8_t* __restrict__ val_l, const uint32_t* __restrict__ from, const uint32_t* __restrict__ node_below,
                 uint32_t total, uint8_t* __restrict__ tree_l, uint8_t* __restrict__ out_vals,
                 uint32_t* __restrict__ out_nodes, uint32_t* counter, uint32_t cap) {
    const size_t kp = gtid();
    const uint32_t f = kp < total ? from[kp] : 0u;
    const bool last = (f & sweep::LAST_BIT) != 0;
    const uint64_t mask = __ballot(last);
    if (!last) return;
    const unsigned lane = __lane_id();
    const int leader = __ffsll((unsigned long long)mask) - 1;
    uint32_t base = 0;
    if ((int)lane == leader) base = atomicAdd(counter, (uint32_t)__popcll(mask));
    base = __shfl(base, leader);
    const uint32_t i = base + (uint32_t)__popcll(mask & ((1ull << lane) - 1ull));
    const Word4* s = reinterpret_cast<const Word4*>(val_l + (size_t)(f & ~sweep::LAST_BIT) * 32);
    const Word4 lo = s[0], hi = s[1];
    const uint32_t node = node_below[kp];
    Word4* t = reinterpret_cast<Word4*>(tree_l + (size_t)node * 32);
    t[0] = lo;
    t[1] = hi;
    if (i >= cap) return;
    Word4* d = reinterpret_cast<Word4*>(out_vals + (size_t)i * 32);
    d[0] = lo;
    d[1] = hi;
    out_nodes[i] = node;
}
__global__ void __launch_bounds__(BLOCK)
k_apply_packed(const uint8_t* __restrict__ vals, const uint32_t* __restrict__ nodes, const uint32_t* __restrict__ counter,
               uint32_t cap, uint8_t* __restrict__ tree_l, uint64_t len_l) {
    const size_t i = gtid();
    const uint32_t n = *counter < cap ? *counter : cap;
    if (i >= n) return;
    const uint64_t node = nodes[i];
    if (node >= len_l) return;
    const Word4* s = reinterpret_cast<const Word4*>(vals + i * 32);
    Word4* d = reinterpret_cast<Word4*>(tree_l + node * 32);
    d[0] = s[0];
    d[1] = s[1];
}

__global__ void __launch_bounds__(BLOCK) k_apply_gathered(launch::ApplyJobs a) {
    if (a.poison && __hip_atomic_load(a.poison, __ATOMIC_RELAXED, __HIP_MEMORY_SCOPE_SYSTEM) != 0) return;
    const launch::ApplyJobs::Job j = a.j[blockIdx.y];
    const size_t i = gtid();
    if (j.pairs) {
        const uint32_t* counter = reinterpret_cast<const uint32_t*>(j.payload + 96);
        const uint32_t n = *counter < j.cap ? *counter : j.cap;
        if (i >= n) return;
        const uint32_t* nodes = reinterpret_cast<const uint32_t*>(j.payload + 128 + (size_t)j.cap * 32);
        const uint64_t node = nodes[i];
        if (node >= j.len_l) return;
        const Word4* s = reinterpret_cast<const Word4*>(j.payload + 128 + i * 32);
        Word4* d = reinterpret_cast<Word4*>(j.tree_l + node * 32);
        d[0] = s[0];
        d[1] = s[1];
        return;
    }
    if (i >= 3) return;
    uint8_t* dst = i == 0 ? j.node_in : (i == 1 ? j.node_out : j.root);
    if (!dst) return;
    const Word4* s = reinterpret_cast<const Word4*>(j.payload + i * 32);
    Word4* d = reinterpret_cast<Word4*>(dst);
    d[0] = s[0];
    d[1] = s[1];
}

__global__ void k_store_top_path(const uint8_t* __restrict__ top_path, uint8_t* __restrict__ tree_nodes,
                                 const uint64_t* __restrict__ tree_off, unsigned l0, unsigned depth) {
    const unsigned l = l0 + threadIdx.x;
    if (l > depth) return;
    const Word4* s = reinterpret_cast<const Word4*>(top_path + (size_t)(l - l0) * 32);
    Word4* d = reinterpret_cast<Word4*>(tree_nodes + tree_off[l] * 32);
    d[0] = s[0];
    d[1] = s[1];
}

__global__ void __launch_bounds__(256) k_mad_peak(uint32_t* out, uint32_t seed, int iters) {
    uint64_t a0 = threadIdx.x + seed, a1 = a0 * 3 + 1, a2 = a0 * 5 + 2, a3 = a0 * 7 + 3;
    uint64_t a4 = a0 * 11 + 4, a5 = a0 * 13 + 5, a6 = a0 * 17 + 6, a7 = a0 * 19 + 7;
    const uint32_t b = (uint32_t)a0 | 1u, c = seed * 77u + 12345u;
    for (int i = 0; i < iters; i++) {
        asm volatile("v_mad_u64_u32 %0, vcc, %8, %9, %0\n v_mad_u64_u32 %1, vcc, %8, %9, %1\n"
                     "v_mad_u64_u32 %2, vcc, %8, %9, %2\n v_mad_u64_u32 %3, vcc, %8, %9, %3\n"
                     "v_mad_u64_u32 %4, vcc, %8, %9, %4\n v_mad_u64_u32 %5, vcc, %8, %9, %5\n"
                     "v_mad_u64_u32 %6, vcc, %8, %9, %6\n v_mad_u64_u32 %7, vcc, %8, %9, %7\n"
                     : "+v"(a0), "+v"(a1), "+v"(a2), "+v"(a3), "+v"(a4), "+v"(a5), "+v"(a6), "+v"(a7)
                     : "v"(b), "v"(c) : "vcc");
    }
    const uint64_t r = a0 ^ a1 ^ a2 ^ a3 ^ a4 ^ a5 ^ a6 ^ a7;
    out[blockIdx.x * blockDim.x + threadIdx.x] = (uint32_t)r ^ (uint32_t)(r >> 32);
}

inline unsigned nblk(size_t n) { return (unsigned)((n + BLOCK - 1) / BLOCK); }

}

namespace launch {

hipError_t upload_consts(const dev::PoseidonConsts& pc) {
    return hipMemcpyToSymbol(HIP_SYMBOL(g_pc), &pc, sizeof(pc), 0, hipMemcpyHostToDevice);
}
hipError_t upload_trace_consts(const dev::TraceConsts& tc) {
    return hipMemcpyToSymbol(HIP_SYMBOL(g_tc), &tc, sizeof(tc), 0, hipMemcpyHostToDevice);
}
void hash_trace_jobs(hipStream_t s, const TraceJobs& a, unsigned fmt_out) {
    size_t most = 0;
    for (int k = 0; k < a.n_jobs; k++) most = std::max(most, a.j[k].n_items);
    if (!most || a.n_jobs <= 0) return;
    auto* k = fmt_out == FMT_MONT256 ? k_hash_trace<FMT_MONT256>
              : fmt_out == FMT_DEVICE ? k_hash_trace<FMT_DEVICE> : k_hash_trace<FMT_CANONICAL>;
    hipLaunchKernelGGL(k, dim3(nblk(most), (unsigned)a.n_jobs), dim3(BLOCK), 0, s, a);
}
void hash_trace(hipStream_t s, const uint8_t* in, size_t n_items, int arity, uint8_t* trace, size_t n_per, size_t row0,
                size_t rows_total, bool item_major, unsigned fmt_in, unsigned fmt_out, int* err) {
    TraceJobs a{};
    a.j[0] = {in, n_items, arity, row0, fmt_in};
    a.n_jobs = 1;
    a.trace = trace; a.n_per = n_per; a.rows_total = rows_total; a.item_major = item_major ? 1 : 0; a.err = err;
    hash_trace_jobs(s, a, fmt_out);
}
void insert_trace_inputs(hipStream_t s, const uint8_t* low_leaf, const uint8_t* new_leaf, const uint64_t* new_index,
                         size_t n, uint8_t* new_low, uint8_t* zero_leaf, unsigned fmt, int* err) {
    if (!n) return;
    hipLaunchKernelGGL(k_insert_trace_inputs, dim3(nblk(n)), dim3(BLOCK), 0, s, low_leaf, new_leaf, new_index, n, new_low,
                       zero_leaf, fmt, err);
}
void path_pairs(hipStream_t s, const PathChains& a, uint32_t coop_max) {
    if (!a.n || a.n_chains <= 0) return;
    if (a.n * 4 * (size_t)a.n_chains <= coop_max)
        hipLaunchKernelGGL(k_path_pairs_coop, dim3(nblk(a.n * 4), (unsigned)a.n_chains), dim3(BLOCK), 0, s, a);
    else
        hipLaunchKernelGGL(k_path_pairs, dim3(nblk(a.n), (unsigned)a.n_chains), dim3(BLOCK), 0, s, a);
}

void hash_batch(hipStream_t s, const uint8_t* in, uint8_t* out, size_t n, int arity, unsigned fmt_in,
                unsigned fmt_out, int* err, uint32_t coop_max) {
    if (!n) return;
    if (n * 4 <= coop_max)
        hipLaunchKernelGGL(k_hash_batch_coop, dim3(nblk(n * 4)), dim3(BLOCK), 0, s, in, out, n, arity, fmt_in, fmt_out, err);
    else
        hipLaunchKernelGGL(k_hash_batch, dim3(nblk(n)), dim3(BLOCK), 0, s, in, out, n, arity, fmt_in, fmt_out, err);
}
void permute_batch(hipStream_t s, const uint8_t* in, uint8_t* out, size_t n, unsigned fmt_in, unsigned fmt_out,
                   int* err) {
    if (!n) return;
    hipLaunchKernelGGL(k_permute_batch, dim3(nblk(n)), dim3(BLOCK), 0, s, in, out, n, fmt_in, fmt_out, err);
}
void convert(hipStream_t s, const uint8_t* in, uint8_t* out, size_t n, unsigned fmt_in, unsigned fmt_out,
             int* err) {
    if (!n) return;
    hipLaunchKernelGGL(k_convert, dim3(nblk(n)), dim3(BLOCK), 0, s, in, out, n, fmt_in, fmt_out, err);
}
void split128(hipStream_t s, const uint8_t* vals, uint8_t* q, uint8_t* r, size_t n, unsigned fmt, int* err) {
    if (!n) return;
    hipLaunchKernelGGL(k_split128, dim3(nblk(n)), dim3(BLOCK), 0, s, vals, q, r, n, fmt, err);
}
void path_root(hipStream_t s, const uint8_t* leaf, const uint8_t* leaf3, const uint64_t* index, bool is_helper,
               const uint8_t* sib, SibLayout lay, unsigned depth, size_t n, uint8_t* root_out,
               const uint8_t* expect, unsigned expect_stride, uint8_t* ok_out, unsigned fmt_in, unsigned fmt_out,
               int* err, uint32_t coop_max) {
    if (!n) return;
    if (n * 4 <= coop_max)
        hipLaunchKernelGGL(k_path_root_coop, dim3(nblk(n * 4)), dim3(BLOCK), 0, s, leaf, leaf3, index, is_helper ? 1 : 0,
                           sib, lay, depth, n, root_out, expect, expect_stride, ok_out, fmt_in, fmt_out, err);
    else
        hipLaunchKernelGGL(k_path_root, dim3(nblk(n)), dim3(BLOCK), 0, s, leaf, leaf3, index, is_helper ? 1 : 0, sib,
                           lay, depth, n, root_out, expect, expect_stride, ok_out, fmt_in, fmt_out, err);
}
void non_membership(hipStream_t s, const uint8_t* root, unsigned root_stride, const uint8_t* low_leaf,
                    const uint64_t* low_index, const uint8_t* sib, SibLayout lay, unsigned depth,
                    const uint8_t* new_val, const uint8_t* is_largest, size_t n, uint8_t* fail_out,
                    uint8_t* root_out, unsigned fmt_in, unsigned fmt_out, int* err, uint32_t coop_max) {
    if (!n) return;
    if (n * 4 <= coop_max)
        hipLaunchKernelGGL(k_non_membership_coop, dim3(nblk(n * 4)), dim3(BLOCK), 0, s, root, root_stride, low_leaf,
                           low_index, sib, lay, depth, new_val, is_largest, n, fail_out, root_out, fmt_in, fmt_out, err);
    else {
        hipLaunchKernelGGL(k_non_membership, dim3(nblk(n)), dim3(BLOCK), 0, s, root, root_stride, low_leaf, low_index,
                           sib, lay, depth, new_val, is_largest, n, fail_out, root_out, fmt_in, fmt_out, err);
        hipLaunchKernelGGL(k_non_membership_pred, dim3(nblk(n)), dim3(BLOCK), 0, s, low_leaf, new_val, is_largest, n, fail_out,
                           fmt_in, err);
    }
}
void insert_witness(hipStream_t s, const uint8_t* old_root, const uint8_t* low_leaf, const uint64_t* low_index,
                    const uint8_t* low_sib, const uint8_t* new_root, const uint8_t* new_leaf,
                    const uint64_t* new_index, const uint64_t* new_path_index, const uint8_t* new_sib, SibLayout lay,
                    const uint8_t* is_largest, unsigned depth, size_t n, uint8_t* fail_out, uint8_t* trace,
                    unsigned fmt_in, unsigned fmt_out, int* err, uint32_t coop_max) {
    (void)fmt_out;
    if (!n) return;
    if (n * 16 <= coop_max)
        hipLaunchKernelGGL(k_insert_chains_coop, dim3(nblk(n * 4), 4), dim3(BLOCK), 0, s, low_leaf, low_index, low_sib,
                           new_leaf, new_index, new_path_index, new_sib, lay, depth, n, trace, fmt_in, err);
    else
        hipLaunchKernelGGL(k_insert_chains, dim3(nblk(n), 4), dim3(BLOCK), 0, s, low_leaf, low_index, low_sib, new_leaf,
                           new_index, new_path_index, new_sib, lay, depth, n, trace, fmt_in, err);
    hipLaunchKernelGGL(k_insert_check, dim3(nblk(n)), dim3(BLOCK), 0, s, old_root, low_leaf, new_root, new_leaf,
                       is_largest, n, trace, fail_out, fmt_in, err);
}
void tree_level(hipStream_t s, const uint8_t* prev, uint8_t* next, size_t n_parents, uint32_t coop_max) {
    if (!n_parents) return;
    if (n_parents * 4 <= coop_max)
        hipLaunchKernelGGL(k_hash_batch_coop, dim3(nblk(n_parents * 4)), dim3(BLOCK), 0, s, prev, next, n_parents, 2,
                           (unsigned)FMT_DEVICE, (unsigned)FMT_DEVICE, (int*)nullptr);
    else
        hipLaunchKernelGGL(k_tree_level, dim3(nblk(n_parents)), dim3(BLOCK), 0, s, prev, next, n_parents);
}
void index_leaves(hipStream_t s, const uint8_t* val, const uint32_t* sorted, uint32_t M, uint64_t base, uint8_t* tree0,
                  int* err) {
    if (!M) return;
    hipLaunchKernelGGL(k_index_leaves, dim3(nblk(M)), dim3(BLOCK), 0, s, val, sorted, M, base, tree0, err);
}
void zero_chain(hipStream_t s, uint8_t* out, unsigned depth) {
    hipLaunchKernelGGL(k_zero_chain, dim3(1), dim3(64), 0, s, out, depth);
}
void extend_root(hipStream_t s, uint8_t* cur, const uint8_t* zero, unsigned from, unsigned to) {
    hipLaunchKernelGGL(k_extend_root, dim3(1), dim3(64), 0, s, cur, zero, from, to);
}
void gather_proof(hipStream_t s, TreeView tv, const uint64_t* index, size_t n, unsigned depth, uint8_t* out,
                  SibLayout lay, unsigned fmt_out) {
    if (!n || !depth) return;
    hipLaunchKernelGGL(k_gather_proof, dim3(nblk(n * depth)), dim3(BLOCK), 0, s, tv, index, n, depth, out, lay,
                       fmt_out);
}
void write_helpers(hipStream_t s, uint64_t index, unsigned depth, uint8_t* out, unsigned fmt_out) {
    if (!depth) return;
    hipLaunchKernelGGL(k_write_helpers, dim3((depth + 63) / 64), dim3(64), 0, s, index, depth, out, fmt_out);
}


void mad_peak(hipStream_t s, uint32_t* out, unsigned blocks, int iters) {
    hipLaunchKernelGGL(k_mad_peak, dim3(blocks), dim3(256), 0, s, out, 1u, iters);
}
void fill_level(hipStream_t s, uint8_t* nodes, size_t n, const uint8_t* zero_l) {
    if (!n) return;
    hipLaunchKernelGGL(k_fill_level, dim3(nblk(n)), dim3(BLOCK), 0, s, nodes, n, zero_l);
}
void restride_levels(hipStream_t s, const uint8_t* old_nodes, const uint64_t* old_off, const uint64_t* old_len,
                     uint8_t* new_nodes, const uint64_t* new_off, uint64_t new_total, const uint8_t* zero, unsigned depth) {
    if (!new_total) return;
    const unsigned blocks = std::min(nblk((size_t)new_total * 2), 256u * 16u);
    hipLaunchKernelGGL(k_restride_levels, dim3(blocks), dim3(BLOCK), 0, s, old_nodes, old_off, old_len, new_nodes, new_off,
                       new_total, zero, depth);
}
static void launch_sweep(hipStream_t s, const SweepArgs& a, uint32_t coop_max) {
    if (a.count <= coop_max)
        hipLaunchKernelGGL(k_sweep_coop, dim3(nblk((size_t)a.count * 4)), dim3(BLOCK), 0, s, a);
    else
        hipLaunchKernelGGL(k_sweep, dim3(nblk(a.count)), dim3(BLOCK), 0, s, a);
}
void sweep_leaves(hipStream_t s, const uint8_t* pre, const uint32_t* time0, uint8_t* val0, uint32_t k_begin,
                  uint32_t k_count, unsigned fmt_in, int* err, uint32_t coop_max) {
    if (!k_count) return;
    SweepArgs a{};
    a.mode = SWEEP_LEAVES;
    a.begin = k_begin; a.count = k_count;
    a.pre = pre; a.time0 = time0; a.val_out = val0; a.fmt_in = fmt_in; a.err = err;
    a.last_event = 0xffffffffu;
    launch_sweep(s, a, coop_max);
}
void merge_level(hipStream_t s, sweep::LevelTable in, sweep::LevelOut out, uint32_t total) {
    if (!total) return;
    hipLaunchKernelGGL(k_merge_level, dim3(nblk(total)), dim3(BLOCK), 0, s, in, out, total);
}
static SweepArgs level_args(const uint8_t* val_in, uint8_t* val_out, const uint32_t* from, const int32_t* sibsrc,
                            const uint32_t* node_below, const uint32_t* time_next, const uint8_t* tree_l, uint64_t len_l,
                            const uint8_t* zero_l, uint32_t k_begin, uint32_t k_count, uint8_t* low_sib, uint8_t* new_sib,
                            SibLayout lay, unsigned level, unsigned fmt_out) {
    SweepArgs a{};
    a.mode = SWEEP_LEVEL;
    a.begin = k_begin; a.count = k_count;
    a.val_in = val_in; a.val_out = val_out; a.from = from; a.sibsrc = sibsrc; a.node_below = node_below;
    a.time_next = time_next; a.tree_l = tree_l; a.len_l = len_l; a.zero_l = zero_l; a.level = level;
    a.low_sib = low_sib; a.new_sib = new_sib; a.lay = lay; a.fmt_out = fmt_out;
    a.last_event = 0xffffffffu;
    return a;
}
void sweep_level(hipStream_t s, const uint8_t* val_in, uint8_t* val_out, const uint32_t* from, const int32_t* sibsrc,
                 const uint32_t* node_below, const uint32_t* time_next, const uint8_t* tree_l, uint64_t len_l,
                 const uint8_t* zero_l, uint32_t k_begin, uint32_t k_count, uint8_t* low_sib, uint8_t* new_sib,
                 SibLayout lay, unsigned level, unsigned fmt_out, uint32_t coop_max) {
    if (!k_count) return;
    launch_sweep(s, level_args(val_in, val_out, from, sibsrc, node_below, time_next, tree_l, len_l, zero_l, k_begin, k_count,
                               low_sib, new_sib, lay, level, fmt_out), coop_max);
}
void sweep_upper(hipStream_t s, const uint8_t* val_in, uint8_t* val_out, const uint8_t* zero_l, uint32_t e_begin,
                 uint32_t e_count, uint32_t last_event, uint8_t* node_in, uint8_t* node_out, uint8_t* low_sib,
                 uint8_t* new_sib, SibLayout lay, unsigned level, unsigned fmt_out, uint32_t coop_max) {
    if (!e_count) return;
    SweepArgs a{};
    a.mode = SWEEP_LEVEL;
    a.begin = e_begin; a.count = e_count;
    a.val_in = val_in; a.val_out = val_out; a.zero_l = zero_l; a.level = level;
    a.low_sib = low_sib; a.new_sib = new_sib; a.lay = lay; a.fmt_out = fmt_out;
    a.last_event = last_event; a.node_in = node_in; a.node_out = node_out;
    launch_sweep(s, a, coop_max);
}
static void launch_sweep_mixed(hipStream_t s, const SweepArgs& a, const MixedRoute& r, uint32_t coop_max) {
    const SweepMixedArgs m{a, r.erow, r.read_sib};
    if (a.count <= coop_max)
        hipLaunchKernelGGL(k_sweep_mixed_coop, dim3(nblk((size_t)a.count * 4)), dim3(BLOCK), 0, s, m);
    else
        hipLaunchKernelGGL(k_sweep_mixed, dim3(nblk(a.count)), dim3(BLOCK), 0, s, m);
}
void sweep_level_mixed(hipStream_t s, const MixedRoute& r, const uint8_t* val_in, uint8_t* val_out, const uint32_t* from,
                       const int32_t* sibsrc, const uint32_t* node_below, const uint32_t* time_next, const uint8_t* tree_l,
                       uint64_t len_l, const uint8_t* zero_l, uint32_t k_count, uint8_t* low_sib, uint8_t* new_sib, SibLayout lay,
                       unsigned level, unsigned fmt_out, uint32_t coop_max) {
    if (!k_count) return;
    launch_sweep_mixed(s, level_args(val_in, val_out, from, sibsrc, node_below, time_next, tree_l, len_l, zero_l, 0, k_count,
                                     low_sib, new_sib, lay, level, fmt_out), r, coop_max);
}
void sweep_upper_mixed(hipStream_t s, const MixedRoute& r, const uint8_t* val_in, uint8_t* val_out, const uint8_t* zero_l,
                       uint32_t e_count, uint8_t* node_in, uint8_t* node_out, uint8_t* low_sib, uint8_t* new_sib, SibLayout lay,
                       unsigned level, unsigned fmt_out, uint32_t coop_max) {
    if (!e_count) return;
    SweepArgs a{};
    a.mode = SWEEP_LEVEL;
    a.begin = 0; a.count = e_count;
    a.val_in = val_in; a.val_out = val_out; a.zero_l = zero_l; a.level = level;
    a.low_sib = low_sib; a.new_sib = new_sib; a.lay = lay; a.fmt_out = fmt_out;
    a.last_event = e_count - 1; a.node_in = node_in; a.node_out = node_out;
    launch_sweep_mixed(s, a, r, coop_max);
}
void emit_roots_mixed(hipStream_t s, const MixedRoute& r, const uint8_t* val, uint32_t total, uint32_t n_ins, uint8_t* old_root,
                      uint8_t* interim_root, uint8_t* new_root, uint8_t* read_root, unsigned fmt_out, uint8_t* node_store) {
    if (!total) return;
    hipLaunchKernelGGL(k_emit_roots_mixed, dim3(nblk(total)), dim3(BLOCK), 0, s, val, total, r.erow, n_ins, old_root,
                       interim_root, new_root, read_root, fmt_out, node_store);
}
void emit_roots_bulk(hipStream_t s, const uint8_t* val, uint32_t total, uint8_t* root_before, uint8_t* root_after,
                     unsigned fmt_out, uint8_t* node_store) {
    if (!total) return;
    hipLaunchKernelGGL(k_emit_roots_bulk, dim3(nblk(total)), dim3(BLOCK), 0, s, val, total, root_before, root_after, fmt_out,
                       node_store);
}
void gather_frontier(hipStream_t s, TreeView tv, uint64_t index, unsigned depth, uint8_t* out, unsigned fmt_out) {
    if (!depth) return;
    hipLaunchKernelGGL(k_gather_frontier, dim3((depth + 63) / 64), dim3(64), 0, s, tv, index, depth, out, fmt_out);
}
void bulk_frontier_base(hipStream_t s, const view::Side& side, TreeView tv, unsigned depth, uint8_t* out) {
    if (!depth) return;
    hipLaunchKernelGGL(k_bulk_frontier_base, dim3((depth + 63) / 64), dim3(64), 0, s, side, tv, depth, out);
}
void bulk_frontier_level(hipStream_t s, uint64_t size, unsigned level, const uint8_t* val_l, const uint32_t* from,
                         const uint32_t* node_below, uint32_t total, uint8_t* out_l) {
    if (!total || !replay::frontier_left(size, level)) return;
    hipLaunchKernelGGL(k_bulk_frontier_level, dim3(nblk(total)), dim3(BLOCK), 0, s, size, level, val_l, from, node_below, total,
                       out_l);
}
uint64_t frontier_rows(FrontierArgs& a) {
    uint64_t total = 0;
    a.top = a.depth;
    for (unsigned l = 0; l <= a.depth; l++) {
        const uint64_t count = ((a.start + a.n - 1) >> l) - (a.start >> l) + 1;
        a.off[l] = total;
        total += count + 2;
        if (count == 1) { a.top = l; break; }
    }
    return total;
}
void frontier_bounds(hipStream_t s, const FrontierArgs& a) {
    hipLaunchKernelGGL(k_frontier_bounds, dim3((a.depth + 64) / 64), dim3(64), 0, s, a);
}
static void launch_apply(hipStream_t s, const ApplyArgs& a, uint32_t coop_max) {
    if (!a.bound) return;
    if (a.bound <= coop_max)
        hipLaunchKernelGGL(k_apply_level_coop, dim3(nblk((size_t)a.bound * 4)), dim3(BLOCK), 0, s, a);
    else
        hipLaunchKernelGGL(k_apply_level, dim3(nblk(a.bound)), dim3(BLOCK), 0, s, a);
}
void apply_leaves(hipStream_t s, const uint64_t* count, uint32_t bound, const uint32_t* list, const uint32_t* src,
                  const uint8_t* pre, unsigned fmt_in, int* err, uint8_t* tree0, uint64_t len0, uint32_t coop_max) {
    ApplyArgs a{};
    a.mode = APPLY_LEAVES;
    a.count = count; a.bound = bound; a.list = list; a.tree_out = tree0; a.len_out = len0;
    a.src = src; a.pre = pre; a.fmt_in = fmt_in; a.err = err;
    launch_apply(s, a, coop_max);
}
void apply_level(hipStream_t s, const uint64_t* count, uint32_t bound, const uint32_t* list, const uint8_t* tree_in,
                 uint64_t len_in, const uint8_t* zero_in, uint8_t* tree_out, uint64_t len_out, uint32_t coop_max) {
    ApplyArgs a{};
    a.mode = APPLY_LEVEL;
    a.count = count; a.bound = bound; a.list = list; a.tree_out = tree_out; a.len_out = len_out;
    a.tree_in = tree_in; a.len_in = len_in; a.zero_in = zero_in;
    launch_apply(s, a, coop_max);
}
void apply_top(hipStream_t s, uint8_t* nodes, const uint64_t* off, const uint64_t* len, const uint8_t* zero, unsigned from,
               unsigned to) {
    if (from >= to) return;
    hipLaunchKernelGGL(k_apply_top, dim3(1), dim3(64), 0, s, nodes, off, len, zero, from, to);
}
void apply_chain(hipStream_t s, const uint8_t* nodes, const uint64_t* off, const uint64_t* len, const uint8_t* zero,
                 uint8_t* chain, unsigned from, unsigned to) {
    if (from >= to) return;
    hipLaunchKernelGGL(k_apply_chain, dim3(1), dim3(64), 0, s, nodes, off, len, zero, chain, from, to);
}
void apply_chain_store(hipStream_t s, const uint8_t* chain, uint8_t* nodes, const uint64_t* off, unsigned from, unsigned to,
                       uint8_t* root) {
    if (from > to) return;
    hipLaunchKernelGGL(k_apply_chain_store, dim3(nblk((size_t)(to - from + 1) * 8)), dim3(BLOCK), 0, s, (const uint32_t*)chain,
                       (uint32_t*)nodes, off, from, to, (uint32_t*)root);
}
static void launch_view(hipStream_t s, const ViewArgs& a, uint32_t coop_max) {
    if (!a.bound) return;
    if (a.bound <= coop_max)
        hipLaunchKernelGGL(k_view_level_coop, dim3(nblk((size_t)a.bound * 4)), dim3(BLOCK), 0, s, a);
    else
        hipLaunchKernelGGL(k_view_level, dim3(nblk(a.bound)), dim3(BLOCK), 0, s, a);
}
void view_leaves(hipStream_t s, const uint64_t* count, uint32_t bound, const uint32_t* list, const uint32_t* src,
                 const uint8_t* pre, unsigned fmt_in, int* err, uint8_t* out, uint64_t len0, uint32_t coop_max) {
    ViewArgs a{};
    a.mode = APPLY_LEAVES;
    a.count = count; a.bound = bound; a.list = list; a.out = out; a.len_out = len0;
    a.src = src; a.pre = pre; a.fmt_in = fmt_in; a.err = err;
    launch_view(s, a, coop_max);
}
void view_level(hipStream_t s, const view::Side& side, unsigned level_in, uint32_t bound, const uint8_t* tree_in,
                uint64_t len_in, const uint8_t* zero_in, uint8_t* out, uint64_t len_out, uint32_t coop_max) {
    ViewArgs a{};
    a.mode = APPLY_LEVEL;
    a.count = side.count + level_in + 1; a.bound = bound; a.list = side.node + (size_t)(level_in + 1) * side.stride;
    a.out = out; a.len_out = len_out;
    a.side = side; a.level_in = level_in; a.tree_in = tree_in; a.len_in = len_in; a.zero_in = zero_in;
    launch_view(s, a, coop_max);
}
void view_top(hipStream_t s, const view::Side& side, TreeView tv, uint8_t* chain, unsigned from, unsigned to) {
    if (from >= to) return;
    hipLaunchKernelGGL(k_view_top, dim3(1), dim3(64), 0, s, side, tv, chain, from, to);
}
void view_gather_proof(hipStream_t s, const view::Side& side, TreeView tv, const uint64_t* index, size_t n, unsigned depth,
                       uint8_t* out, SibLayout lay, unsigned fmt_out) {
    if (!n || !depth) return;
    hipLaunchKernelGGL(k_view_gather_proof, dim3(nblk(n * depth)), dim3(BLOCK), 0, s, side, tv, index, n, depth, out, lay,
                       fmt_out);
}
void sweep_view_level(hipStream_t s, const view::Side& side, const uint8_t* val_in, uint8_t* val_out, const uint32_t* from,
                      const int32_t* sibsrc, const uint32_t* node_below, const uint32_t* time_next, const uint8_t* tree_l,
                      uint64_t len_l, const uint8_t* zero_l, uint32_t k_count, uint8_t* low_sib, uint8_t* new_sib, SibLayout lay,
                      unsigned level, unsigned fmt_out, uint32_t coop_max) {
    if (!k_count) return;
    const SweepViewArgs v{level_args(val_in, val_out, from, sibsrc, node_below, time_next, tree_l, len_l, zero_l, 0, k_count,
                                     low_sib, new_sib, lay, level, fmt_out), side};
    if (k_count <= coop_max)
        hipLaunchKernelGGL(k_sweep_view_coop, dim3(nblk((size_t)k_count * 4)), dim3(BLOCK), 0, s, v);
    else
        hipLaunchKernelGGL(k_sweep_view, dim3(nblk(k_count)), dim3(BLOCK), 0, s, v);
}
void sweep_view_level_mixed(hipStream_t s, const view::Side& side, const MixedRoute& r, const uint8_t* val_in, uint8_t* val_out,
                            const uint32_t* from, const int32_t* sibsrc, const uint32_t* node_below, const uint32_t* time_next,
                            const uint8_t* tree_l, uint64_t len_l, const uint8_t* zero_l, uint32_t k_count, uint8_t* low_sib,
                            uint8_t* new_sib, SibLayout lay, unsigned level, unsigned fmt_out, uint32_t coop_max) {
    if (!k_count) return;
    const SweepViewMixedArgs v{level_args(val_in, val_out, from, sibsrc, node_below, time_next, tree_l, len_l, zero_l, 0, k_count,
                                          low_sib, new_sib, lay, level, fmt_out), side, r.erow, r.read_sib};
    if (k_count <= coop_max)
        hipLaunchKernelGGL(k_sweep_view_mixed_coop, dim3(nblk((size_t)k_count * 4)), dim3(BLOCK), 0, s, v);
    else
        hipLaunchKernelGGL(k_sweep_view_mixed, dim3(nblk(k_count)), dim3(BLOCK), 0, s, v);
}
void emit_roots(hipStream_t s, const uint8_t* val, uint32_t e_begin, uint32_t e_count, uint32_t total, uint8_t* old_root,
                uint8_t* interim_root, uint8_t* new_root, unsigned fmt_out, uint8_t* roots_dev, uint8_t* node_store) {
    if (!e_count) return;
    hipLaunchKernelGGL(k_emit_roots, dim3(nblk(e_count)), dim3(BLOCK), 0, s, val, e_begin, e_count, total, old_root,
                       interim_root, new_root, fmt_out, roots_dev, node_store);
}
void writeback(hipStream_t s, const uint8_t* val_l, const uint32_t* from, const uint32_t* node_below, uint8_t* tree_l,
               uint32_t total) {
    if (!total) return;
    hipLaunchKernelGGL(k_writeback, dim3(nblk(total)), dim3(BLOCK), 0, s, val_l, from, node_below, tree_l, total);
}
void lift_roots(hipStream_t s, uint8_t* old_root, uint8_t* interim_root, uint8_t* new_root, uint32_t n,
                const uint8_t* top, uint64_t pos_bits, unsigned levels, unsigned fmt, int* err) {
    const size_t jobs = (interim_root ? n : 0) + (size_t)(new_root ? n : 0) + (old_root ? (new_root ? 1u : n) : 0);
    if (!jobs) return;
    hipLaunchKernelGGL(k_lift_roots, dim3(nblk(jobs)), dim3(BLOCK), 0, s, old_root, interim_root, new_root, n, top,
                       pos_bits, levels, fmt, err);
}
void fill_sib_rows(hipStream_t s, uint8_t* sib, SibLayout lay, unsigned first_level, unsigned levels, uint32_t n,
                   const uint8_t* top, unsigned fmt_out) {
    if (!sib || !n || !levels) return;
    hipLaunchKernelGGL(k_fill_sib_rows, dim3(nblk((size_t)n * levels)), dim3(BLOCK), 0, s, sib, lay, first_level, levels,
                       n, top, fmt_out);
}
void mix_roots(hipStream_t s, const uint8_t* before, const uint8_t* after, uint8_t* mixed, uint32_t n_sub, uint32_t self,
               unsigned fmt_in, int* err) {
    hipLaunchKernelGGL(k_mix_roots, dim3((n_sub + 63) / 64), dim3(64), 0, s, before, after, mixed, n_sub, self, fmt_in,
                       err);
}
void pick_top(hipStream_t s, const uint8_t* levels_buf, uint32_t n_sub, uint32_t self, unsigned k, unsigned levels,
              const uint8_t* zero, unsigned sub_depth, uint8_t* top) {
    hipLaunchKernelGGL(k_pick_top, dim3(1), dim3(64), 0, s, levels_buf, n_sub, self, k, levels, zero, sub_depth, top);
}
void slot0(hipStream_t s, const uint32_t* time0, uint32_t* slot0_out, uint32_t total) {
    if (!total) return;
    hipLaunchKernelGGL(k_slot0, dim3(nblk(total)), dim3(BLOCK), 0, s, time0, slot0_out, total);
}
void extract(hipStream_t s, const ExtractParams& p) {
    if (!p.ins_count) return;
    ExtractArgs a{p.val, p.slot, p.sibsrc, p.node_below, p.stride, p.tree_nodes, p.tree_off, p.tree_len, p.zero, p.roots,
                  p.l0, p.depth, p.ins_begin, p.ins_count, p.n_total, p.old_root, p.interim_root, p.new_root, p.low_sib,
                  p.new_sib, p.lay, p.fmt_out};
    const size_t threads = (size_t)p.ins_count * 2 * ((size_t)p.depth + 1);
    hipLaunchKernelGGL(k_extract, dim3(nblk(threads)), dim3(BLOCK), 0, s, a);
}
void pack_writeback(hipStream_t s, const uint8_t* val_l, const uint32_t* from, const uint32_t* node_below, uint32_t total,
                    uint8_t* tree_l, uint8_t* out_vals, uint32_t* out_nodes, uint32_t* counter, uint32_t cap, hipEvent_t done) {
    if (!total) return;
    if (done)
        hipExtLaunchKernelGGL(k_pack_writeback, dim3(nblk(total)), dim3(BLOCK), 0, s, nullptr, done, 0, val_l, from, node_below, total,
                              tree_l, out_vals, out_nodes, counter, cap);
    else
        hipLaunchKernelGGL(k_pack_writeback, dim3(nblk(total)), dim3(BLOCK), 0, s, val_l, from, node_below, total, tree_l,
                           out_vals, out_nodes, counter, cap);
}
void apply_packed(hipStream_t s, const uint8_t* vals, const uint32_t* nodes, const uint32_t* counter, uint32_t cap,
                  uint8_t* tree_l, uint64_t len_l) {
    if (!cap) return;
    hipLaunchKernelGGL(k_apply_packed, dim3(nblk(cap)), dim3(BLOCK), 0, s, vals, nodes, counter, cap, tree_l, len_l);
}
void apply_gathered(hipStream_t s, const ApplyJobs& a, hipEvent_t done) {
    if (!a.n_jobs) return;
    uint32_t widest = 3;
    for (int k = 0; k < a.n_jobs; k++)
        if (a.j[k].pairs && a.j[k].cap > widest) widest = a.j[k].cap;
    if (done) hipExtLaunchKernelGGL(k_apply_gathered, dim3(nblk(widest), a.n_jobs), dim3(BLOCK), 0, s, nullptr, done, 0, a);
    else hipLaunchKernelGGL(k_apply_gathered, dim3(nblk(widest), a.n_jobs), dim3(BLOCK), 0, s, a);
}
void store_top_path(hipStream_t s, const uint8_t* top_path, uint8_t* tree_nodes, const uint64_t* tree_off, unsigned l0,
                    unsigned depth) {
    hipLaunchKernelGGL(k_store_top_path, dim3(1), dim3(64), 0, s, top_path, tree_nodes, tree_off, l0, depth);
}

}
}
```

Baseline: 3.705 million.

## Add fused paired-round Poseidon permutation with interleaved asm for sweep kernel

Adds a sweep-specific Poseidon permutation that processes partial rounds in pairs, with a hand-written inline-asm routine fusing the x^5 multiply and the 4-term Montgomery dot product into one interleaved instruction stream using two independent accumulators. Round constants are kept in scalar registers via a forced-uniform index. This is meant to raise instruction-level parallelism and cut register moves in the partial-round chain. In exchange it hard-codes registers v38-v41, which may conflict with compiler allocation, raises VGPR pressure, and adds a large asm body that must stay correct.

```diff
diff --git a/indexed-merkle-tree-halo2_amd/csrc/imt_device.hpp b/indexed-merkle-tree-halo2_amd/csrc/imt_device.hpp
--- a/indexed-merkle-tree-halo2_amd/csrc/imt_device.hpp
+++ b/indexed-merkle-tree-halo2_amd/csrc/imt_device.hpp
@@ -42,6 +42,7 @@
 #define IMT_MONT_ASM 1
 #include "imt_mont_asm.hpp"
 #include "imt_mont_asm_rec.hpp"
+#include "imt_mont_asm_pair.hpp"
 #endif
 namespace imt {
 namespace dev {
@@ -341,6 +342,94 @@
     }
 }
 
+IMT_HD int variant_index(int i) {
+#if defined(__HIP_DEVICE_COMPILE__)
+    asm("" : "+s"(i));
+#endif
+    return i;
+}
+
+IMT_HD void rec_round(const PoseidonConsts& pc, int r, const Fe& w, Fe& wp, Fe& zp, const Fe& z1) {
+    Fe x, x2, x4;
+    add_lazy(x, w, pc.rec_k[r]);
+    mont_sqr(x2, x);
+    mont_sqr(x4, x2);
+#ifdef IMT_MONT_ASM
+    masm::rec_tail_uc(wp, zp, pc.rec_c[r], w, z1, x4, x);
+#else
+    Fe z, n;
+    mont_mul(z, x4, x);
+    const Fe v[4] = {w, wp, zp, z1};
+    mont_dot<4, true>(n, pc.rec_c[r], v, z);
+    wp = n;
+    zp = z;
+#endif
+}
+
+IMT_HD void permute_sweep(const PoseidonConsts& pc, Fe s[3], const Fe* first_rc) {
+    static_assert((RP - 3) % 2 == 0, "rounds 3 .. RP-1 pair up");
+#pragma unroll 1
+    for (int half = 0; half < 2; half++) {
+        if (half == 1) {
+            Fe z3, e;
+            {
+                const int r = variant_index(0);
+                Fe z, w;
+                add_lazy(z, s[0], pc.rec_k[r]);
+                sbox(z);
+                add_lazy(w, s[1], z);
+                normalize(w);
+                s[1] = s[0]; s[0] = w; z3 = s[2]; s[2] = z;
+            }
+            {
+                const int r = variant_index(1);
+                Fe z;
+                add_lazy(z, s[0], pc.rec_k[r]);
+                sbox(z);
+                const Fe v[2] = {s[0], s[2]};
+                add_lazy(e, z3, z);
+                mont_dot_uc<2, true, false>(s[1], pc.rec_c[r], v, e);
+                z3 = z;
+            }
+#pragma unroll 1
+            for (int r = 1; r < RP; r += 2) {
+                if (r > 1) rec_round(pc, r, s[0], s[1], z3, s[2]);
+                rec_round(pc, r + 1, s[1], s[0], s[2], z3);
+            }
+            const Fe v[3] = {s[0], s[1], z3};
+            const Fe zl = s[2];
+#pragma unroll 1
+            for (int i = 0; i < 2; i++) {
+                Fe n;
+                mont_dot_uc<3, false>(n, pc.rec_exit[i], v, v[0]);
+                add_lazy(n, n, zl);
+                normalize(n);
+                s[1] = s[2]; s[2] = n;
+            }
+        }
+#pragma unroll 1
+        for (int fr = half * (RF / 2); fr < (half + 1) * (RF / 2); fr++) {
+            const Fe* rc = (fr == 0) ? first_rc : pc.sc_rc[fr];
+            add_lazy(s[0], s[0], rc[0]);
+            add_lazy(s[1], s[1], rc[1]);
+            add_lazy(s[2], s[2], rc[2]);
+            sbox(s[0]); sbox(s[1]); sbox(s[2]);
+            const Fe(*mat)[3] = pc.sc_mats[fr];
+            Fe n0, n1, n2;
+            if (fr == 0 || fr == RF / 2) {
+                mont_dot_uc<3, false>(n0, mat[0], s, s[0]);
+            } else {
+                add_lazy(n0, s[0], s[1]);
+                add_lazy(n0, n0, s[2]);
+                normalize(n0);
+            }
+            mont_dot_uc<3, false>(n1, mat[1], s, s[0]);
+            mont_dot_uc<3, false>(n2, mat[2], s, s[0]);
+            s[0] = n0; s[1] = n1; s[2] = n2;
+        }
+    }
+}
+
 IMT_HD void hash23(const PoseidonConsts& pc, Fe& out, const Fe& a, const Fe& b, const Fe& c, bool three) {
     Fe s[3] = {pc.cap0, a, b};
 #pragma unroll 1
@@ -361,6 +450,7 @@
     out = s[1];
     canonicalize(out);
 }
+template <bool SWEEP = false>
 IMT_HD void hash23_stashed(const PoseidonConsts& pc, Fe& out, const Fe& a, const Fe& b, bool three,
                            const uint32_t* stash, unsigned stride) {
     Fe s[3] = {pc.cap0, a, b};
@@ -380,7 +470,8 @@
                 rc0 = pc.rc_h2p2;
             }
         }
-        permute(pc, s, rc0);
+        if constexpr (SWEEP) permute_sweep(pc, s, rc0);
+        else permute(pc, s, rc0);
     }
     out = s[1];
     canonicalize(out);
diff --git a/indexed-merkle-tree-halo2_amd/csrc/imt_kernels.hip b/indexed-merkle-tree-halo2_amd/csrc/imt_kernels.hip
--- a/indexed-merkle-tree-halo2_amd/csrc/imt_kernels.hip
+++ b/indexed-merkle-tree-halo2_amd/csrc/imt_kernels.hip
@@ -817,7 +817,7 @@
         uint8_t* row = (e & 1u) ? a.new_sib : a.low_sib;
         if (row) store_fe(g_pc, row + ((uint64_t)a.level * a.lay.level_stride + (uint64_t)(e >> 1) * a.lay.item_stride) * 32, sv, a.fmt_out);
     }
-    hash23_stashed(g_pc, o, A, B, a.mode == launch::SWEEP_LEAVES, &stash[0][threadIdx.x], BLOCK);
+    hash23_stashed<true>(g_pc, o, A, B, a.mode == launch::SWEEP_LEAVES, &stash[0][threadIdx.x], BLOCK);
     store_packed(a.val_out + (size_t)x * 32, o);
     if (x == a.last_event && a.node_out) store_packed(a.node_out, o);
 }
diff --git a/indexed-merkle-tree-halo2_amd/csrc/imt_mont_asm_pair.hpp b/indexed-merkle-tree-halo2_amd/csrc/imt_mont_asm_pair.hpp
--- /dev/null
+++ b/indexed-merkle-tree-halo2_amd/csrc/imt_mont_asm_pair.hpp
@@ -0,0 +1,694 @@
+#pragma once
+#if !defined(__HIP_DEVICE_COMPILE__)
+#error "device-only header"
+#endif
+
+namespace imt {
+namespace dev {
+namespace masm {
+
+
+__device__ __forceinline__ void rec_tail_uc(Fe& wp, Fe& zp, const Fe* c, const Fe& w, const Fe& z1, const Fe& x4, const Fe& x) {
+    uint32_t m0, m1, m2, m3, m4, m5, m6, m7, m8;
+    uint32_t q0, q1, q2, q3, q4, q5, q6, q7, q8;
+    asm(
+        "v_mad_u64_u32 v[38:39], vcc, %[x4_0], %[x0], 0\n"
+        "v_mul_lo_u32 %[q0], v38, %[n0]\n"
+        "v_mad_u64_u32 v[38:39], vcc, %[q0], %[p0], v[38:39]\n"
+        "v_lshrrev_b64 v[38:39], 29, v[38:39]\n"
+        "v_mad_u64_u32 v[38:39], vcc, %[x4_0], %[x1], v[38:39]\n"
+        "v_mad_u64_u32 v[38:39], vcc, %[x4_1], %[x0], v[38:39]\n"
+        "v_mad_u64_u32 v[38:39], vcc, %[q0], %[p1], v[38:39]\n"
+        "v_mul_lo_u32 %[q1], v38, %[n0]\n"
+        "v_mad_u64_u32 v[38:39], vcc, %[q1], %[p0], v[38:39]\n"
+        "v_lshrrev_b64 v[38:39], 29, v[38:39]\n"
+        "v_mad_u64_u32 v[38:39], vcc, %[x4_0], %[x2], v[38:39]\n"
+        "v_mad_u64_u32 v[38:39], vcc, %[x4_1], %[x1], v[38:39]\n"
+        "v_mad_u64_u32 v[38:39], vcc, %[x4_2], %[x0], v[38:39]\n"
+        "v_mad_u64_u32 v[38:39], vcc, %[q0], %[p2], v[38:39]\n"
+        "v_mad_u64_u32 v[38:39], vcc, %[q1], %[p1], v[38:39]\n"
+        "v_mul_lo_u32 %[q2], v38, %[n0]\n"
+        "v_mad_u64_u32 v[38:39], vcc, %[q2], %[p0], v[38:39]\n"
+        "v_lshrrev_b64 v[38:39], 29, v[38:39]\n"
+        "v_mad_u64_u32 v[38:39], vcc, %[x4_0], %[x3], v[38:39]\n"
+        "v_mad_u64_u32 v[38:39], vcc, %[x4_1], %[x2], v[38:39]\n"
+        "v_mad_u64_u32 v[38:39], vcc, %[x4_2], %[x1], v[38:39]\n"
+        "v_mad_u64_u32 v[38:39], vcc, %[x4_3], %[x0], v[38:39]\n"
+        "v_mad_u64_u32 v[38:39], vcc, %[q0], %[p3], v[38:39]\n"
+        "v_mad_u64_u32 v[38:39], vcc, %[q1], %[p2], v[38:39]\n"
+        "v_mad_u64_u32 v[38:39], vcc, %[q2], %[p1], v[38:39]\n"
+        "v_mul_lo_u32 %[q3], v38, %[n0]\n"
+        "v_mad_u64_u32 v[38:39], vcc, %[q3], %[p0], v[38:39]\n"
+        "v_lshrrev_b64 v[38:39], 29, v[38:39]\n"
+        "v_mad_u64_u32 v[38:39], vcc, %[x4_0], %[x4], v[38:39]\n"
+        "v_mad_u64_u32 v[38:39], vcc, %[x4_1], %[x3], v[38:39]\n"
+        "v_mad_u64_u32 v[38:39], vcc, %[x4_2], %[x2], v[38:39]\n"
+        "v_mad_u64_u32 v[38:39], vcc, %[x4_3], %[x1], v[38:39]\n"
+        "v_mad_u64_u32 v[38:39], vcc, %[x4_4], %[x0], v[38:39]\n"
+        "v_mad_u64_u32 v[38:39], vcc, %[q0], %[p4], v[38:39]\n"
+        "v_mad_u64_u32 v[38:39], vcc, %[q1], %[p3], v[38:39]\n"
+        "v_mad_u64_u32 v[38:39], vcc, %[q2], %[p2], v[38:39]\n"
+        "v_mad_u64_u32 v[38:39], vcc, %[q3], %[p1], v[38:39]\n"
+        "v_mul_lo_u32 %[q4], v38, %[n0]\n"
+        "v_mad_u64_u32 v[38:39], vcc, %[q4], %[p0], v[38:39]\n"
+        "v_lshrrev_b64 v[38:39], 29, v[38:39]\n"
+        "v_mad_u64_u32 v[38:39], vcc, %[x4_0], %[x5], v[38:39]\n"
+        "v_mad_u64_u32 v[38:39], vcc, %[x4_1], %[x4], v[38:39]\n"
+        "v_mad_u64_u32 v[38:39], vcc, %[x4_2], %[x3], v[38:39]\n"
+        "v_mad_u64_u32 v[38:39], vcc, %[x4_3], %[x2], v[38:39]\n"
+        "v_mad_u64_u32 v[38:39], vcc, %[x4_4], %[x1], v[38:39]\n"
+        "v_mad_u64_u32 v[38:39], vcc, %[x4_5], %[x0], v[38:39]\n"
+        "v_mad_u64_u32 v[38:39], vcc, %[q0], %[p5], v[38:39]\n"
+        "v_mad_u64_u32 v[38:39], vcc, %[q1], %[p4], v[38:39]\n"
+        "v_mad_u64_u32 v[38:39], vcc, %[q2], %[p3], v[38:39]\n"
+        "v_mad_u64_u32 v[38:39], vcc, %[q3], %[p2], v[38:39]\n"
+        "v_mad_u64_u32 v[38:39], vcc, %[q4], %[p1], v[38:39]\n"
+        "v_mul_lo_u32 %[q5], v38, %[n0]\n"
+        "v_mad_u64_u32 v[38:39], vcc, %[q5], %[p0], v[38:39]\n"
+        "v_lshrrev_b64 v[38:39], 29, v[38:39]\n"
+        "v_mad_u64_u32 v[38:39], vcc, %[x4_0], %[x6], v[38:39]\n"
+        "v_mad_u64_u32 v[38:39], vcc, %[x4_1], %[x5], v[38:39]\n"
+        "v_mad_u64_u32 v[38:39], vcc, %[x4_2], %[x4], v[38:39]\n"
+        "v_mad_u64_u32 v[38:39], vcc, %[x4_3], %[x3], v[38:39]\n"
+        "v_mad_u64_u32 v[38:39], vcc, %[x4_4], %[x2], v[38:39]\n"
+        "v_mad_u64_u32 v[38:39], vcc, %[x4_5], %[x1], v[38:39]\n"
+        "v_mad_u64_u32 v[38:39], vcc, %[x4_6], %[x0], v[38:39]\n"
+        "v_mad_u64_u32 v[38:39], vcc, %[q0], %[p6], v[38:39]\n"
+        "v_mad_u64_u32 v[38:39], vcc, %[q1], %[p5], v[38:39]\n"
+        "v_mad_u64_u32 v[38:39], vcc, %[q2], %[p4], v[38:39]\n"
+        "v_mad_u64_u32 v[38:39], vcc, %[q3], %[p3], v[38:39]\n"
+        "v_mad_u64_u32 v[38:39], vcc, %[q4], %[p2], v[38:39]\n"
+        "v_mad_u64_u32 v[38:39], vcc, %[q5], %[p1], v[38:39]\n"
+        "v_mul_lo_u32 %[q6], v38, %[n0]\n"
+        "v_mad_u64_u32 v[38:39], vcc, %[q6], %[p0], v[38:39]\n"
+        "v_lshrrev_b64 v[38:39], 29, v[38:39]\n"
+        "v_mad_u64_u32 v[38:39], vcc, %[x4_0], %[x7], v[38:39]\n"
+        "v_mad_u64_u32 v[38:39], vcc, %[x4_1], %[x6], v[38:39]\n"
+        "v_mad_u64_u32 v[38:39], vcc, %[x4_2], %[x5], v[38:39]\n"
+        "v_mad_u64_u32 v[38:39], vcc, %[x4_3], %[x4], v[38:39]\n"
+        "v_mad_u64_u32 v[38:39], vcc, %[x4_4], %[x3], v[38:39]\n"
+        "v_mad_u64_u32 v[38:39], vcc, %[x4_5], %[x2], v[38:39]\n"
+        "v_mad_u64_u32 v[38:39], vcc, %[x4_6], %[x1], v[38:39]\n"
+        "v_mad_u64_u32 v[38:39], vcc, %[x4_7], %[x0], v[38:39]\n"
+        "v_mad_u64_u32 v[38:39], vcc, %[q0], %[p7], v[38:39]\n"
+        "v_mad_u64_u32 v[38:39], vcc, %[q1], %[p6], v[38:39]\n"
+        "v_mad_u64_u32 v[38:39], vcc, %[q2], %[p5], v[38:39]\n"
+        "v_mad_u64_u32 v[38:39], vcc, %[q3], %[p4], v[38:39]\n"
+        "v_mad_u64_u32 v[38:39], vcc, %[q4], %[p3], v[38:39]\n"
+        "v_mad_u64_u32 v[38:39], vcc, %[q5], %[p2], v[38:39]\n"
+        "v_mad_u64_u32 v[38:39], vcc, %[q6], %[p1], v[38:39]\n"
+        "v_mul_lo_u32 %[q7], v38, %[n0]\n"
+        "v_mad_u64_u32 v[38:39], vcc, %[q7], %[p0], v[38:39]\n"
+        "v_lshrrev_b64 v[38:39], 29, v[38:39]\n"
+        "v_mad_u64_u32 v[38:39], vcc, %[x4_0], %[x8], v[38:39]\n"
+        "v_mad_u64_u32 v[38:39], vcc, %[x4_1], %[x7], v[38:39]\n"
+        "v_mad_u64_u32 v[38:39], vcc, %[x4_2], %[x6], v[38:39]\n"
+        "v_mad_u64_u32 v[38:39], vcc, %[x4_3], %[x5], v[38:39]\n"
+        "v_mad_u64_u32 v[38:39], vcc, %[x4_4], %[x4], v[38:39]\n"
+        "v_mad_u64_u32 v[38:39], vcc, %[x4_5], %[x3], v[38:39]\n"
+        "v_mad_u64_u32 v[38:39], vcc, %[x4_6], %[x2], v[38:39]\n"
+        "v_mad_u64_u32 v[38:39], vcc, %[x4_7], %[x1], v[38:39]\n"
+        "v_mad_u64_u32 v[38:39], vcc, %[x4_8], %[x0], v[38:39]\n"
+        "v_mad_u64_u32 v[38:39], vcc, %[q0], %[p8], v[38:39]\n"
+        "v_mad_u64_u32 v[38:39], vcc, %[q1], %[p7], v[38:39]\n"
+        "v_mad_u64_u32 v[38:39], vcc, %[q2], %[p6], v[38:39]\n"
+        "v_mad_u64_u32 v[38:39], vcc, %[q3], %[p5], v[38:39]\n"
+        "v_mad_u64_u32 v[38:39], vcc, %[q4], %[p4], v[38:39]\n"
+        "v_mad_u64_u32 v[38:39], vcc, %[q5], %[p3], v[38:39]\n"
+        "v_mad_u64_u32 v[38:39], vcc, %[q6], %[p2], v[38:39]\n"
+        "v_mad_u64_u32 v[38:39], vcc, %[q7], %[p1], v[38:39]\n"
+        "v_mul_lo_u32 %[q8], v38, %[n0]\n"
+        "v_mad_u64_u32 v[38:39], vcc, %[q8], %[p0], v[38:39]\n"
+        "v_lshrrev_b64 v[38:39], 29, v[38:39]\n"
+        "v_mad_u64_u32 v[40:41], vcc, %[c0_0], %[w0], 0\n"
+        "v_mad_u64_u32 v[40:41], vcc, %[c1_0], %[wp0], v[40:41]\n"
+        "v_mad_u64_u32 v[40:41], vcc, %[c2_0], %[zp0], v[40:41]\n"
+        "v_mad_u64_u32 v[40:41], vcc, %[c3_0], %[z10], v[40:41]\n"
+        "v_mul_lo_u32 %[m0], v40, %[n0]\n"
+        "v_mad_u64_u32 v[40:41], vcc, %[m0], %[p0], v[40:41]\n"
+        "v_lshrrev_b64 v[40:41], 29, v[40:41]\n"
+        "v_mad_u64_u32 v[40:41], vcc, %[c0_0], %[w1], v[40:41]\n"
+        "v_mad_u64_u32 v[40:41], vcc, %[c0_1], %[w0], v[40:41]\n"
+        "v_mad_u64_u32 v[40:41], vcc, %[c1_0], %[wp1], v[40:41]\n"
+        "v_mad_u64_u32 v[40:41], vcc, %[c1_1], %[wp0], v[40:41]\n"
+        "v_mad_u64_u32 v[40:41], vcc, %[c2_0], %[zp1], v[40:41]\n"
+        "v_mad_u64_u32 v[40:41], vcc, %[c2_1], %[zp0], v[40:41]\n"
+        "v_mad_u64_u32 v[40:41], vcc, %[c3_0], %[z11], v[40:41]\n"
+        "v_mad_u64_u32 v[40:41], vcc, %[c3_1], %[z10], v[40:41]\n"
+        "v_mad_u64_u32 v[40:41], vcc, %[m0], %[p1], v[40:41]\n"
+        "v_mul_lo_u32 %[m1], v40, %[n0]\n"
+        "v_mad_u64_u32 v[40:41], vcc, %[m1], %[p0], v[40:41]\n"
+        "v_lshrrev_b64 v[40:41], 29, v[40:41]\n"
+        "v_mad_u64_u32 v[40:41], vcc, %[c0_0], %[w2], v[40:41]\n"
+        "v_mad_u64_u32 v[40:41], vcc, %[c0_1], %[w1], v[40:41]\n"
+        "v_mad_u64_u32 v[40:41], vcc, %[c0_2], %[w0], v[40:41]\n"
+        "v_mad_u64_u32 v[40:41], vcc, %[c1_0], %[wp2], v[40:41]\n"
+        "v_mad_u64_u32 v[40:41], vcc, %[c1_1], %[wp1], v[40:41]\n"
+        "v_mad_u64_u32 v[40:41], vcc, %[c1_2], %[wp0], v[40:41]\n"
+        "v_mad_u64_u32 v[40:41], vcc, %[c2_0], %[zp2], v[40:41]\n"
+        "v_mad_u64_u32 v[40:41], vcc, %[c2_1], %[zp1], v[40:41]\n"
+        "v_mad_u64_u32 v[40:41], vcc, %[c2_2], %[zp0], v[40:41]\n"
+        "v_mad_u64_u32 v[40:41], vcc, %[c3_0], %[z12], v[40:41]\n"
+        "v_mad_u64_u32 v[40:41], vcc, %[c3_1], %[z11], v[40:41]\n"
+        "v_mad_u64_u32 v[40:41], vcc, %[c3_2], %[z10], v[40:41]\n"
+        "v_mad_u64_u32 v[40:41], vcc, %[m0], %[p2], v[40:41]\n"
+        "v_mad_u64_u32 v[40:41], vcc, %[m1], %[p1], v[40:41]\n"
+        "v_mul_lo_u32 %[m2], v40, %[n0]\n"
+        "v_mad_u64_u32 v[40:41], vcc, %[m2], %[p0], v[40:41]\n"
+        "v_lshrrev_b64 v[40:41], 29, v[40:41]\n"
+        "v_mad_u64_u32 v[40:41], vcc, %[c0_0], %[w3], v[40:41]\n"
+        "v_mad_u64_u32 v[40:41], vcc, %[c0_1], %[w2], v[40:41]\n"
+        "v_mad_u64_u32 v[40:41], vcc, %[c0_2], %[w1], v[40:41]\n"
+        "v_mad_u64_u32 v[40:41], vcc, %[c0_3], %[w0], v[40:41]\n"
+        "v_mad_u64_u32 v[40:41], vcc, %[c1_0], %[wp3], v[40:41]\n"
+        "v_mad_u64_u32 v[40:41], vcc, %[c1_1], %[wp2], v[40:41]\n"
+        "v_mad_u64_u32 v[40:41], vcc, %[c1_2], %[wp1], v[40:41]\n"
+        "v_mad_u64_u32 v[40:41], vcc, %[c1_3], %[wp0], v[40:41]\n"
+        "v_mad_u64_u32 v[40:41], vcc, %[c2_0], %[zp3], v[40:41]\n"
+        "v_mad_u64_u32 v[40:41], vcc, %[c2_1], %[zp2], v[40:41]\n"
+        "v_mad_u64_u32 v[40:41], vcc, %[c2_2], %[zp1], v[40:41]\n"
+        "v_mad_u64_u32 v[40:41], vcc, %[c2_3], %[zp0], v[40:41]\n"
+        "v_mad_u64_u32 v[40:41], vcc, %[c3_0], %[z13], v[40:41]\n"
+        "v_mad_u64_u32 v[40:41], vcc, %[c3_1], %[z12], v[40:41]\n"
+        "v_mad_u64_u32 v[40:41], vcc, %[c3_2], %[z11], v[40:41]\n"
+        "v_mad_u64_u32 v[40:41], vcc, %[c3_3], %[z10], v[40:41]\n"
+        "v_mad_u64_u32 v[40:41], vcc, %[m0], %[p3], v[40:41]\n"
+        "v_mad_u64_u32 v[40:41], vcc, %[m1], %[p2], v[40:41]\n"
+        "v_mad_u64_u32 v[40:41], vcc, %[m2], %[p1], v[40:41]\n"
+        "v_mul_lo_u32 %[m3], v40, %[n0]\n"
+        "v_mad_u64_u32 v[40:41], vcc, %[m3], %[p0], v[40:41]\n"
+        "v_lshrrev_b64 v[40:41], 29, v[40:41]\n"
+        "v_mad_u64_u32 v[40:41], vcc, %[c0_0], %[w4], v[40:41]\n"
+        "v_mad_u64_u32 v[40:41], vcc, %[c0_1], %[w3], v[40:41]\n"
+        "v_mad_u64_u32 v[40:41], vcc, %[c0_2], %[w2], v[40:41]\n"
+        "v_mad_u64_u32 v[40:41], vcc, %[c0_3], %[w1], v[40:41]\n"
+        "v_mad_u64_u32 v[40:41], vcc, %[c0_4], %[w0], v[40:41]\n"
+        "v_mad_u64_u32 v[40:41], vcc, %[c1_0], %[wp4], v[40:41]\n"
+        "v_mad_u64_u32 v[40:41], vcc, %[c1_1], %[wp3], v[40:41]\n"
+        "v_mad_u64_u32 v[40:41], vcc, %[c1_2], %[wp2], v[40:41]\n"
+        "v_mad_u64_u32 v[40:41], vcc, %[c1_3], %[wp1], v[40:41]\n"
+        "v_mad_u64_u32 v[40:41], vcc, %[c1_4], %[wp0], v[40:41]\n"
+        "v_mad_u64_u32 v[40:41], vcc, %[c2_0], %[zp4], v[40:41]\n"
+        "v_mad_u64_u32 v[40:41], vcc, %[c2_1], %[zp3], v[40:41]\n"
+        "v_mad_u64_u32 v[40:41], vcc, %[c2_2], %[zp2], v[40:41]\n"
+        "v_mad_u64_u32 v[40:41], vcc, %[c2_3], %[zp1], v[40:41]\n"
+        "v_mad_u64_u32 v[40:41], vcc, %[c2_4], %[zp0], v[40:41]\n"
+        "v_mad_u64_u32 v[40:41], vcc, %[c3_0], %[z14], v[40:41]\n"
+        "v_mad_u64_u32 v[40:41], vcc, %[c3_1], %[z13], v[40:41]\n"
+        "v_mad_u64_u32 v[40:41], vcc, %[c3_2], %[z12], v[40:41]\n"
+        "v_mad_u64_u32 v[40:41], vcc, %[c3_3], %[z11], v[40:41]\n"
+        "v_mad_u64_u32 v[40:41], vcc, %[c3_4], %[z10], v[40:41]\n"
+        "v_mad_u64_u32 v[40:41], vcc, %[m0], %[p4], v[40:41]\n"
+        "v_mad_u64_u32 v[40:41], vcc, %[m1], %[p3], v[40:41]\n"
+        "v_mad_u64_u32 v[40:41], vcc, %[m2], %[p2], v[40:41]\n"
+        "v_mad_u64_u32 v[40:41], vcc, %[m3], %[p1], v[40:41]\n"
+        "v_mul_lo_u32 %[m4], v40, %[n0]\n"
+        "v_mad_u64_u32 v[40:41], vcc, %[m4], %[p0], v[40:41]\n"
+        "v_lshrrev_b64 v[40:41], 29, v[40:41]\n"
+        "v_mad_u64_u32 v[40:41], vcc, %[c0_0], %[w5], v[40:41]\n"
+        "v_mad_u64_u32 v[40:41], vcc, %[c0_1], %[w4], v[40:41]\n"
+        "v_mad_u64_u32 v[40:41], vcc, %[c0_2], %[w3], v[40:41]\n"
+        "v_mad_u64_u32 v[40:41], vcc, %[c0_3], %[w2], v[40:41]\n"
+        "v_mad_u64_u32 v[40:41], vcc, %[c0_4], %[w1], v[40:41]\n"
+        "v_mad_u64_u32 v[40:41], vcc, %[c0_5], %[w0], v[40:41]\n"
+        "v_mad_u64_u32 v[40:41], vcc, %[c1_0], %[wp5], v[40:41]\n"
+        "v_mad_u64_u32 v[40:41], vcc, %[c1_1], %[wp4], v[40:41]\n"
+        "v_mad_u64_u32 v[40:41], vcc, %[c1_2], %[wp3], v[40:41]\n"
+        "v_mad_u64_u32 v[40:41], vcc, %[c1_3], %[wp2], v[40:41]\n"
+        "v_mad_u64_u32 v[40:41], vcc, %[c1_4], %[wp1], v[40:41]\n"
+        "v_mad_u64_u32 v[40:41], vcc, %[c1_5], %[wp0], v[40:41]\n"
+        "v_mad_u64_u32 v[40:41], vcc, %[c2_0], %[zp5], v[40:41]\n"
+        "v_mad_u64_u32 v[40:41], vcc, %[c2_1], %[zp4], v[40:41]\n"
+        "v_mad_u64_u32 v[40:41], vcc, %[c2_2], %[zp3], v[40:41]\n"
+        "v_mad_u64_u32 v[40:41], vcc, %[c2_3], %[zp2], v[40:41]\n"
+        "v_mad_u64_u32 v[40:41], vcc, %[c2_4], %[zp1], v[40:41]\n"
+        "v_mad_u64_u32 v[40:41], vcc, %[c2_5], %[zp0], v[40:41]\n"
+        "v_mad_u64_u32 v[40:41], vcc, %[c3_0], %[z15], v[40:41]\n"
+        "v_mad_u64_u32 v[40:41], vcc, %[c3_1], %[z14], v[40:41]\n"
+        "v_mad_u64_u32 v[40:41], vcc, %[c3_2], %[z13], v[40:41]\n"
+        "v_mad_u64_u32 v[40:41], vcc, %[c3_3], %[z12], v[40:41]\n"
+        "v_mad_u64_u32 v[40:41], vcc, %[c3_4], %[z11], v[40:41]\n"
+        "v_mad_u64_u32 v[40:41], vcc, %[c3_5], %[z10], v[40:41]\n"
+        "v_mad_u64_u32 v[40:41], vcc, %[m0], %[p5], v[40:41]\n"
+        "v_mad_u64_u32 v[40:41], vcc, %[m1], %[p4], v[40:41]\n"
+        "v_mad_u64_u32 v[40:41], vcc, %[m2], %[p3], v[40:41]\n"
+        "v_mad_u64_u32 v[40:41], vcc, %[m3], %[p2], v[40:41]\n"
+        "v_mad_u64_u32 v[40:41], vcc, %[m4], %[p1], v[40:41]\n"
+        "v_mul_lo_u32 %[m5], v40, %[n0]\n"
+        "v_mad_u64_u32 v[40:41], vcc, %[m5], %[p0], v[40:41]\n"
+        "v_lshrrev_b64 v[40:41], 29, v[40:41]\n"
+        "v_mad_u64_u32 v[40:41], vcc, %[c0_0], %[w6], v[40:41]\n"
+        "v_mad_u64_u32 v[40:41], vcc, %[c0_1], %[w5], v[40:41]\n"
+        "v_mad_u64_u32 v[40:41], vcc, %[c0_2], %[w4], v[40:41]\n"
+        "v_mad_u64_u32 v[40:41], vcc, %[c0_3], %[w3], v[40:41]\n"
+        "v_mad_u64_u32 v[40:41], vcc, %[c0_4], %[w2], v[40:41]\n"
+        "v_mad_u64_u32 v[40:41], vcc, %[c0_5], %[w1], v[40:41]\n"
+        "v_mad_u64_u32 v[40:41], vcc, %[c0_6], %[w0], v[40:41]\n"
+        "v_mad_u64_u32 v[40:41], vcc, %[c1_0], %[wp6], v[40:41]\n"
+        "v_mad_u64_u32 v[40:41], vcc, %[c1_1], %[wp5], v[40:41]\n"
+        "v_mad_u64_u32 v[40:41], vcc, %[c1_2], %[wp4], v[40:41]\n"
+        "v_mad_u64_u32 v[40:41], vcc, %[c1_3], %[wp3], v[40:41]\n"
+        "v_mad_u64_u32 v[40:41], vcc, %[c1_4], %[wp2], v[40:41]\n"
+        "v_mad_u64_u32 v[40:41], vcc, %[c1_5], %[wp1], v[40:41]\n"
+        "v_mad_u64_u32 v[40:41], vcc, %[c1_6], %[wp0], v[40:41]\n"
+        "v_mad_u64_u32 v[40:41], vcc, %[c2_0], %[zp6], v[40:41]\n"
+        "v_mad_u64_u32 v[40:41], vcc, %[c2_1], %[zp5], v[40:41]\n"
+        "v_mad_u64_u32 v[40:41], vcc, %[c2_2], %[zp4], v[40:41]\n"
+        "v_mad_u64_u32 v[40:41], vcc, %[c2_3], %[zp3], v[40:41]\n"
+        "v_mad_u64_u32 v[40:41], vcc, %[c2_4], %[zp2], v[40:41]\n"
+        "v_mad_u64_u32 v[40:41], vcc, %[c2_5], %[zp1], v[40:41]\n"
+        "v_mad_u64_u32 v[40:41], vcc, %[c2_6], %[zp0], v[40:41]\n"
+        "v_mad_u64_u32 v[40:41], vcc, %[c3_0], %[z16], v[40:41]\n"
+        "v_mad_u64_u32 v[40:41], vcc, %[c3_1], %[z15], v[40:41]\n"
+        "v_mad_u64_u32 v[40:41], vcc, %[c3_2], %[z14], v[40:41]\n"
+        "v_mad_u64_u32 v[40:41], vcc, %[c3_3], %[z13], v[40:41]\n"
+        "v_mad_u64_u32 v[40:41], vcc, %[c3_4], %[z12], v[40:41]\n"
+        "v_mad_u64_u32 v[40:41], vcc, %[c3_5], %[z11], v[40:41]\n"
+        "v_mad_u64_u32 v[40:41], vcc, %[c3_6], %[z10], v[40:41]\n"
+        "v_mad_u64_u32 v[40:41], vcc, %[m0], %[p6], v[40:41]\n"
+        "v_mad_u64_u32 v[40:41], vcc, %[m1], %[p5], v[40:41]\n"
+        "v_mad_u64_u32 v[40:41], vcc, %[m2], %[p4], v[40:41]\n"
+        "v_mad_u64_u32 v[40:41], vcc, %[m3], %[p3], v[40:41]\n"
+        "v_mad_u64_u32 v[40:41], vcc, %[m4], %[p2], v[40:41]\n"
+        "v_mad_u64_u32 v[40:41], vcc, %[m5], %[p1], v[40:41]\n"
+        "v_mul_lo_u32 %[m6], v40, %[n0]\n"
+        "v_mad_u64_u32 v[40:41], vcc, %[m6], %[p0], v[40:41]\n"
+        "v_lshrrev_b64 v[40:41], 29, v[40:41]\n"
+        "v_mad_u64_u32 v[40:41], vcc, %[c0_0], %[w7], v[40:41]\n"
+        "v_mad_u64_u32 v[40:41], vcc, %[c0_1], %[w6], v[40:41]\n"
+        "v_mad_u64_u32 v[40:41], vcc, %[c0_2], %[w5], v[40:41]\n"
+        "v_mad_u64_u32 v[40:41], vcc, %[c0_3], %[w4], v[40:41]\n"
+        "v_mad_u64_u32 v[40:41], vcc, %[c0_4], %[w3], v[40:41]\n"
+        "v_mad_u64_u32 v[40:41], vcc, %[c0_5], %[w2], v[40:41]\n"
+        "v_mad_u64_u32 v[40:41], vcc, %[c0_6], %[w1], v[40:41]\n"
+        "v_mad_u64_u32 v[40:41], vcc, %[c0_7], %[w0], v[40:41]\n"
+        "v_mad_u64_u32 v[40:41], vcc, %[c1_0], %[wp7], v[40:41]\n"
+        "v_mad_u64_u32 v[40:41], vcc, %[c1_1], %[wp6], v[40:41]\n"
+        "v_mad_u64_u32 v[40:41], vcc, %[c1_2], %[wp5], v[40:41]\n"
+        "v_mad_u64_u32 v[40:41], vcc, %[c1_3], %[wp4], v[40:41]\n"
+        "v_mad_u64_u32 v[40:41], vcc, %[c1_4], %[wp3], v[40:41]\n"
+        "v_mad_u64_u32 v[40:41], vcc, %[c1_5], %[wp2], v[40:41]\n"
+        "v_mad_u64_u32 v[40:41], vcc, %[c1_6], %[wp1], v[40:41]\n"
+        "v_mad_u64_u32 v[40:41], vcc, %[c1_7], %[wp0], v[40:41]\n"
+        "v_mad_u64_u32 v[40:41], vcc, %[c2_0], %[zp7], v[40:41]\n"
+        "v_mad_u64_u32 v[40:41], vcc, %[c2_1], %[zp6], v[40:41]\n"
+        "v_mad_u64_u32 v[40:41], vcc, %[c2_2], %[zp5], v[40:41]\n"
+        "v_mad_u64_u32 v[40:41], vcc, %[c2_3], %[zp4], v[40:41]\n"
+        "v_mad_u64_u32 v[40:41], vcc, %[c2_4], %[zp3], v[40:41]\n"
+        "v_mad_u64_u32 v[40:41], vcc, %[c2_5], %[zp2], v[40:41]\n"
+        "v_mad_u64_u32 v[40:41], vcc, %[c2_6], %[zp1], v[40:41]\n"
+        "v_mad_u64_u32 v[40:41], vcc, %[c2_7], %[zp0], v[40:41]\n"
+        "v_mad_u64_u32 v[40:41], vcc, %[c3_0], %[z17], v[40:41]\n"
+        "v_mad_u64_u32 v[40:41], vcc, %[c3_1], %[z16], v[40:41]\n"
+        "v_mad_u64_u32 v[40:41], vcc, %[c3_2], %[z15], v[40:41]\n"
+        "v_mad_u64_u32 v[40:41], vcc, %[c3_3], %[z14], v[40:41]\n"
+        "v_mad_u64_u32 v[40:41], vcc, %[c3_4], %[z13], v[40:41]\n"
+        "v_mad_u64_u32 v[40:41], vcc, %[c3_5], %[z12], v[40:41]\n"
+        "v_mad_u64_u32 v[40:41], vcc, %[c3_6], %[z11], v[40:41]\n"
+        "v_mad_u64_u32 v[40:41], vcc, %[c3_7], %[z10], v[40:41]\n"
+        "v_mad_u64_u32 v[40:41], vcc, %[m0], %[p7], v[40:41]\n"
+        "v_mad_u64_u32 v[40:41], vcc, %[m1], %[p6], v[40:41]\n"
+        "v_mad_u64_u32 v[40:41], vcc, %[m2], %[p5], v[40:41]\n"
+        "v_mad_u64_u32 v[40:41], vcc, %[m3], %[p4], v[40:41]\n"
+        "v_mad_u64_u32 v[40:41], vcc, %[m4], %[p3], v[40:41]\n"
+        "v_mad_u64_u32 v[40:41], vcc, %[m5], %[p2], v[40:41]\n"
+        "v_mad_u64_u32 v[40:41], vcc, %[m6], %[p1], v[40:41]\n"
+        "v_mul_lo_u32 %[m7], v40, %[n0]\n"
+        "v_mad_u64_u32 v[40:41], vcc, %[m7], %[p0], v[40:41]\n"
+        "v_lshrrev_b64 v[40:41], 29, v[40:41]\n"
+        "v_mad_u64_u32 v[40:41], vcc, %[c0_0], %[w8], v[40:41]\n"
+        "v_mad_u64_u32 v[40:41], vcc, %[c0_1], %[w7], v[40:41]\n"
+        "v_mad_u64_u32 v[40:41], vcc, %[c0_2], %[w6], v[40:41]\n"
+        "v_mad_u64_u32 v[40:41], vcc, %[c0_3], %[w5], v[40:41]\n"
+        "v_mad_u64_u32 v[40:41], vcc, %[c0_4], %[w4], v[40:41]\n"
+        "v_mad_u64_u32 v[40:41], vcc, %[c0_5], %[w3], v[40:41]\n"
+        "v_mad_u64_u32 v[40:41], vcc, %[c0_6], %[w2], v[40:41]\n"
+        "v_mad_u64_u32 v[40:41], vcc, %[c0_7], %[w1], v[40:41]\n"
+        "v_mad_u64_u32 v[40:41], vcc, %[c0_8], %[w0], v[40:41]\n"
+        "v_mad_u64_u32 v[40:41], vcc, %[c1_0], %[wp8], v[40:41]\n"
+        "v_mad_u64_u32 v[40:41], vcc, %[c1_1], %[wp7], v[40:41]\n"
+        "v_mad_u64_u32 v[40:41], vcc, %[c1_2], %[wp6], v[40:41]\n"
+        "v_mad_u64_u32 v[40:41], vcc, %[c1_3], %[wp5], v[40:41]\n"
+        "v_mad_u64_u32 v[40:41], vcc, %[c1_4], %[wp4], v[40:41]\n"
+        "v_mad_u64_u32 v[40:41], vcc, %[c1_5], %[wp3], v[40:41]\n"
+        "v_mad_u64_u32 v[40:41], vcc, %[c1_6], %[wp2], v[40:41]\n"
+        "v_mad_u64_u32 v[40:41], vcc, %[c1_7], %[wp1], v[40:41]\n"
+        "v_mad_u64_u32 v[40:41], vcc, %[c1_8], %[wp0], v[40:41]\n"
+        "v_mad_u64_u32 v[40:41], vcc, %[c2_0], %[zp8], v[40:41]\n"
+        "v_mad_u64_u32 v[40:41], vcc, %[c2_1], %[zp7], v[40:41]\n"
+        "v_mad_u64_u32 v[40:41], vcc, %[c2_2], %[zp6], v[40:41]\n"
+        "v_mad_u64_u32 v[40:41], vcc, %[c2_3], %[zp5], v[40:41]\n"
+        "v_mad_u64_u32 v[40:41], vcc, %[c2_4], %[zp4], v[40:41]\n"
+        "v_mad_u64_u32 v[40:41], vcc, %[c2_5], %[zp3], v[40:41]\n"
+        "v_mad_u64_u32 v[40:41], vcc, %[c2_6], %[zp2], v[40:41]\n"
+        "v_mad_u64_u32 v[40:41], vcc, %[c2_7], %[zp1], v[40:41]\n"
+        "v_mad_u64_u32 v[40:41], vcc, %[c2_8], %[zp0], v[40:41]\n"
+        "v_mad_u64_u32 v[40:41], vcc, %[c3_0], %[z18], v[40:41]\n"
+        "v_mad_u64_u32 v[40:41], vcc, %[c3_1], %[z17], v[40:41]\n"
+        "v_mad_u64_u32 v[40:41], vcc, %[c3_2], %[z16], v[40:41]\n"
+        "v_mad_u64_u32 v[40:41], vcc, %[c3_3], %[z15], v[40:41]\n"
+        "v_mad_u64_u32 v[40:41], vcc, %[c3_4], %[z14], v[40:41]\n"
+        "v_mad_u64_u32 v[40:41], vcc, %[c3_5], %[z13], v[40:41]\n"
+        "v_mad_u64_u32 v[40:41], vcc, %[c3_6], %[z12], v[40:41]\n"
+        "v_mad_u64_u32 v[40:41], vcc, %[c3_7], %[z11], v[40:41]\n"
+        "v_mad_u64_u32 v[40:41], vcc, %[c3_8], %[z10], v[40:41]\n"
+        "v_mad_u64_u32 v[40:41], vcc, %[m0], %[p8], v[40:41]\n"
+        "v_mad_u64_u32 v[40:41], vcc, %[m1], %[p7], v[40:41]\n"
+        "v_mad_u64_u32 v[40:41], vcc, %[m2], %[p6], v[40:41]\n"
+        "v_mad_u64_u32 v[40:41], vcc, %[m3], %[p5], v[40:41]\n"
+        "v_mad_u64_u32 v[40:41], vcc, %[m4], %[p4], v[40:41]\n"
+        "v_mad_u64_u32 v[40:41], vcc, %[m5], %[p3], v[40:41]\n"
+        "v_mad_u64_u32 v[40:41], vcc, %[m6], %[p2], v[40:41]\n"
+        "v_mad_u64_u32 v[40:41], vcc, %[m7], %[p1], v[40:41]\n"
+        "v_mul_lo_u32 %[m8], v40, %[n0]\n"
+        "v_mad_u64_u32 v[40:41], vcc, %[m8], %[p0], v[40:41]\n"
+        "v_lshrrev_b64 v[40:41], 29, v[40:41]\n"
+        "v_mad_u64_u32 v[38:39], vcc, %[x4_1], %[x8], v[38:39]\n"
+        "v_mad_u64_u32 v[38:39], vcc, %[x4_2], %[x7], v[38:39]\n"
+        "v_mad_u64_u32 v[38:39], vcc, %[x4_3], %[x6], v[38:39]\n"
+        "v_mad_u64_u32 v[38:39], vcc, %[x4_4], %[x5], v[38:39]\n"
+        "v_mad_u64_u32 v[38:39], vcc, %[x4_5], %[x4], v[38:39]\n"
+        "v_mad_u64_u32 v[38:39], vcc, %[x4_6], %[x3], v[38:39]\n"
+        "v_mad_u64_u32 v[38:39], vcc, %[x4_7], %[x2], v[38:39]\n"
+        "v_mad_u64_u32 v[38:39], vcc, %[x4_8], %[x1], v[38:39]\n"
+        "v_mad_u64_u32 v[38:39], vcc, %[q1], %[p8], v[38:39]\n"
+        "v_mad_u64_u32 v[38:39], vcc, %[q2], %[p7], v[38:39]\n"
+        "v_mad_u64_u32 v[38:39], vcc, %[q3], %[p6], v[38:39]\n"
+        "v_mad_u64_u32 v[38:39], vcc, %[q4], %[p5], v[38:39]\n"
+        "v_mad_u64_u32 v[38:39], vcc, %[q5], %[p4], v[38:39]\n"
+        "v_mad_u64_u32 v[38:39], vcc, %[q6], %[p3], v[38:39]\n"
+        "v_mad_u64_u32 v[38:39], vcc, %[q7], %[p2], v[38:39]\n"
+        "v_mad_u64_u32 v[38:39], vcc, %[q8], %[p1], v[38:39]\n"
+        "v_and_b32_e32 %[zp0], 0x1fffffff, v38\n"
+        "v_lshrrev_b64 v[38:39], 29, v[38:39]\n"
+        "v_mad_u64_u32 v[40:41], vcc, %[c0_1], %[w8], v[40:41]\n"
+        "v_mad_u64_u32 v[40:41], vcc, %[c0_2], %[w7], v[40:41]\n"
+        "v_mad_u64_u32 v[40:41], vcc, %[c0_3], %[w6], v[40:41]\n"
+        "v_mad_u64_u32 v[40:41], vcc, %[c0_4], %[w5], v[40:41]\n"
+        "v_mad_u64_u32 v[40:41], vcc, %[c0_5], %[w4], v[40:41]\n"
+        "v_mad_u64_u32 v[40:41], vcc, %[c0_6], %[w3], v[40:41]\n"
+        "v_mad_u64_u32 v[40:41], vcc, %[c0_7], %[w2], v[40:41]\n"
+        "v_mad_u64_u32 v[40:41], vcc, %[c0_8], %[w1], v[40:41]\n"
+        "v_mad_u64_u32 v[40:41], vcc, %[c1_1], %[wp8], v[40:41]\n"
+        "v_mad_u64_u32 v[40:41], vcc, %[c1_2], %[wp7], v[40:41]\n"
+        "v_mad_u64_u32 v[40:41], vcc, %[c1_3], %[wp6], v[40:41]\n"
+        "v_mad_u64_u32 v[40:41], vcc, %[c1_4], %[wp5], v[40:41]\n"
+        "v_mad_u64_u32 v[40:41], vcc, %[c1_5], %[wp4], v[40:41]\n"
+        "v_mad_u64_u32 v[40:41], vcc, %[c1_6], %[wp3], v[40:41]\n"
+        "v_mad_u64_u32 v[40:41], vcc, %[c1_7], %[wp2], v[40:41]\n"
+        "v_mad_u64_u32 v[40:41], vcc, %[c1_8], %[wp1], v[40:41]\n"
+        "v_mad_u64_u32 v[40:41], vcc, %[c2_1], %[zp8], v[40:41]\n"
+        "v_mad_u64_u32 v[40:41], vcc, %[c2_2], %[zp7], v[40:41]\n"
+        "v_mad_u64_u32 v[40:41], vcc, %[c2_3], %[zp6], v[40:41]\n"
+        "v_mad_u64_u32 v[40:41], vcc, %[c2_4], %[zp5], v[40:41]\n"
+        "v_mad_u64_u32 v[40:41], vcc, %[c2_5], %[zp4], v[40:41]\n"
+        "v_mad_u64_u32 v[40:41], vcc, %[c2_6], %[zp3], v[40:41]\n"
+        "v_mad_u64_u32 v[40:41], vcc, %[c2_7], %[zp2], v[40:41]\n"
+        "v_mad_u64_u32 v[40:41], vcc, %[c2_8], %[zp1], v[40:41]\n"
+        "v_mad_u64_u32 v[40:41], vcc, %[c3_1], %[z18], v[40:41]\n"
+        "v_mad_u64_u32 v[40:41], vcc, %[c3_2], %[z17], v[40:41]\n"
+        "v_mad_u64_u32 v[40:41], vcc, %[c3_3], %[z16], v[40:41]\n"
+        "v_mad_u64_u32 v[40:41], vcc, %[c3_4], %[z15], v[40:41]\n"
+        "v_mad_u64_u32 v[40:41], vcc, %[c3_5], %[z14], v[40:41]\n"
+        "v_mad_u64_u32 v[40:41], vcc, %[c3_6], %[z13], v[40:41]\n"
+        "v_mad_u64_u32 v[40:41], vcc, %[c3_7], %[z12], v[40:41]\n"
+        "v_mad_u64_u32 v[40:41], vcc, %[c3_8], %[z11], v[40:41]\n"
+        "v_mad_u64_u32 v[40:41], vcc, %[m1], %[p8], v[40:41]\n"
+        "v_mad_u64_u32 v[40:41], vcc, %[m2], %[p7], v[40:41]\n"
+        "v_mad_u64_u32 v[40:41], vcc, %[m3], %[p6], v[40:41]\n"
+        "v_mad_u64_u32 v[40:41], vcc, %[m4], %[p5], v[40:41]\n"
+        "v_mad_u64_u32 v[40:41], vcc, %[m5], %[p4], v[40:41]\n"
+        "v_mad_u64_u32 v[40:41], vcc, %[m6], %[p3], v[40:41]\n"
+        "v_mad_u64_u32 v[40:41], vcc, %[m7], %[p2], v[40:41]\n"
+        "v_mad_u64_u32 v[40:41], vcc, %[m8], %[p1], v[40:41]\n"
+        "v_mad_u64_u32 v[40:41], vcc, %[zp0], 1, v[40:41]\n"
+        "v_and_b32_e32 %[wp0], 0x1fffffff, v40\n"
+        "v_lshrrev_b64 v[40:41], 29, v[40:41]\n"
+        "v_mad_u64_u32 v[38:39], vcc, %[x4_2], %[x8], v[38:39]\n"
+        "v_mad_u64_u32 v[38:39], vcc, %[x4_3], %[x7], v[38:39]\n"
+        "v_mad_u64_u32 v[38:39], vcc, %[x4_4], %[x6], v[38:39]\n"
+        "v_mad_u64_u32 v[38:39], vcc, %[x4_5], %[x5], v[38:39]\n"
+        "v_mad_u64_u32 v[38:39], vcc, %[x4_6], %[x4], v[38:39]\n"
+        "v_mad_u64_u32 v[38:39], vcc, %[x4_7], %[x3], v[38:39]\n"
+        "v_mad_u64_u32 v[38:39], vcc, %[x4_8], %[x2], v[38:39]\n"
+        "v_mad_u64_u32 v[38:39], vcc, %[q2], %[p8], v[38:39]\n"
+        "v_mad_u64_u32 v[38:39], vcc, %[q3], %[p7], v[38:39]\n"
+        "v_mad_u64_u32 v[38:39], vcc, %[q4], %[p6], v[38:39]\n"
+        "v_mad_u64_u32 v[38:39], vcc, %[q5], %[p5], v[38:39]\n"
+        "v_mad_u64_u32 v[38:39], vcc, %[q6], %[p4], v[38:39]\n"
+        "v_mad_u64_u32 v[38:39], vcc, %[q7], %[p3], v[38:39]\n"
+        "v_mad_u64_u32 v[38:39], vcc, %[q8], %[p2], v[38:39]\n"
+        "v_and_b32_e32 %[zp1], 0x1fffffff, v38\n"
+        "v_lshrrev_b64 v[38:39], 29, v[38:39]\n"
+        "v_mad_u64_u32 v[40:41], vcc, %[c0_2], %[w8], v[40:41]\n"
+        "v_mad_u64_u32 v[40:41], vcc, %[c0_3], %[w7], v[40:41]\n"
+        "v_mad_u64_u32 v[40:41], vcc, %[c0_4], %[w6], v[40:41]\n"
+        "v_mad_u64_u32 v[40:41], vcc, %[c0_5], %[w5], v[40:41]\n"
+        "v_mad_u64_u32 v[40:41], vcc, %[c0_6], %[w4], v[40:41]\n"
+        "v_mad_u64_u32 v[40:41], vcc, %[c0_7], %[w3], v[40:41]\n"
+        "v_mad_u64_u32 v[40:41], vcc, %[c0_8], %[w2], v[40:41]\n"
+        "v_mad_u64_u32 v[40:41], vcc, %[c1_2], %[wp8], v[40:41]\n"
+        "v_mad_u64_u32 v[40:41], vcc, %[c1_3], %[wp7], v[40:41]\n"
+        "v_mad_u64_u32 v[40:41], vcc, %[c1_4], %[wp6], v[40:41]\n"
+        "v_mad_u64_u32 v[40:41], vcc, %[c1_5], %[wp5], v[40:41]\n"
+        "v_mad_u64_u32 v[40:41], vcc, %[c1_6], %[wp4], v[40:41]\n"
+        "v_mad_u64_u32 v[40:41], vcc, %[c1_7], %[wp3], v[40:41]\n"
+        "v_mad_u64_u32 v[40:41], vcc, %[c1_8], %[wp2], v[40:41]\n"
+        "v_mad_u64_u32 v[40:41], vcc, %[c2_2], %[zp8], v[40:41]\n"
+        "v_mad_u64_u32 v[40:41], vcc, %[c2_3], %[zp7], v[40:41]\n"
+        "v_mad_u64_u32 v[40:41], vcc, %[c2_4], %[zp6], v[40:41]\n"
+        "v_mad_u64_u32 v[40:41], vcc, %[c2_5], %[zp5], v[40:41]\n"
+        "v_mad_u64_u32 v[40:41], vcc, %[c2_6], %[zp4], v[40:41]\n"
+        "v_mad_u64_u32 v[40:41], vcc, %[c2_7], %[zp3], v[40:41]\n"
+        "v_mad_u64_u32 v[40:41], vcc, %[c2_8], %[zp2], v[40:41]\n"
+        "v_mad_u64_u32 v[40:41], vcc, %[c3_2], %[z18], v[40:41]\n"
+        "v_mad_u64_u32 v[40:41], vcc, %[c3_3], %[z17], v[40:41]\n"
+        "v_mad_u64_u32 v[40:41], vcc, %[c3_4], %[z16], v[40:41]\n"
+        "v_mad_u64_u32 v[40:41], vcc, %[c3_5], %[z15], v[40:41]\n"
+        "v_mad_u64_u32 v[40:41], vcc, %[c3_6], %[z14], v[40:41]\n"
+        "v_mad_u64_u32 v[40:41], vcc, %[c3_7], %[z13], v[40:41]\n"
+        "v_mad_u64_u32 v[40:41], vcc, %[c3_8], %[z12], v[40:41]\n"
+        "v_mad_u64_u32 v[40:41], vcc, %[m2], %[p8], v[40:41]\n"
+        "v_mad_u64_u32 v[40:41], vcc, %[m3], %[p7], v[40:41]\n"
+        "v_mad_u64_u32 v[40:41], vcc, %[m4], %[p6], v[40:41]\n"
+        "v_mad_u64_u32 v[40:41], vcc, %[m5], %[p5], v[40:41]\n"
+        "v_mad_u64_u32 v[40:41], vcc, %[m6], %[p4], v[40:41]\n"
+        "v_mad_u64_u32 v[40:41], vcc, %[m7], %[p3], v[40:41]\n"
+        "v_mad_u64_u32 v[40:41], vcc, %[m8], %[p2], v[40:41]\n"
+        "v_mad_u64_u32 v[40:41], vcc, %[zp1], 1, v[40:41]\n"
+        "v_and_b32_e32 %[wp1], 0x1fffffff, v40\n"
+        "v_lshrrev_b64 v[40:41], 29, v[40:41]\n"
+        "v_mad_u64_u32 v[38:39], vcc, %[x4_3], %[x8], v[38:39]\n"
+        "v_mad_u64_u32 v[38:39], vcc, %[x4_4], %[x7], v[38:39]\n"
+        "v_mad_u64_u32 v[38:39], vcc, %[x4_5], %[x6], v[38:39]\n"
+        "v_mad_u64_u32 v[38:39], vcc, %[x4_6], %[x5], v[38:39]\n"
+        "v_mad_u64_u32 v[38:39], vcc, %[x4_7], %[x4], v[38:39]\n"
+        "v_mad_u64_u32 v[38:39], vcc, %[x4_8], %[x3], v[38:39]\n"
+        "v_mad_u64_u32 v[38:39], vcc, %[q3], %[p8], v[38:39]\n"
+        "v_mad_u64_u32 v[38:39], vcc, %[q4], %[p7], v[38:39]\n"
+        "v_mad_u64_u32 v[38:39], vcc, %[q5], %[p6], v[38:39]\n"
+        "v_mad_u64_u32 v[38:39], vcc, %[q6], %[p5], v[38:39]\n"
+        "v_mad_u64_u32 v[38:39], vcc, %[q7], %[p4], v[38:39]\n"
+        "v_mad_u64_u32 v[38:39], vcc, %[q8], %[p3], v[38:39]\n"
+        "v_and_b32_e32 %[zp2], 0x1fffffff, v38\n"
+        "v_lshrrev_b64 v[38:39], 29, v[38:39]\n"
+        "v_mad_u64_u32 v[40:41], vcc, %[c0_3], %[w8], v[40:41]\n"
+        "v_mad_u64_u32 v[40:41], vcc, %[c0_4], %[w7], v[40:41]\n"
+        "v_mad_u64_u32 v[40:41], vcc, %[c0_5], %[w6], v[40:41]\n"
+        "v_mad_u64_u32 v[40:41], vcc, %[c0_6], %[w5], v[40:41]\n"
+        "v_mad_u64_u32 v[40:41], vcc, %[c0_7], %[w4], v[40:41]\n"
+        "v_mad_u64_u32 v[40:41], vcc, %[c0_8], %[w3], v[40:41]\n"
+        "v_mad_u64_u32 v[40:41], vcc, %[c1_3], %[wp8], v[40:41]\n"
+        "v_mad_u64_u32 v[40:41], vcc, %[c1_4], %[wp7], v[40:41]\n"
+        "v_mad_u64_u32 v[40:41], vcc, %[c1_5], %[wp6], v[40:41]\n"
+        "v_mad_u64_u32 v[40:41], vcc, %[c1_6], %[wp5], v[40:41]\n"
+        "v_mad_u64_u32 v[40:41], vcc, %[c1_7], %[wp4], v[40:41]\n"
+        "v_mad_u64_u32 v[40:41], vcc, %[c1_8], %[wp3], v[40:41]\n"
+        "v_mad_u64_u32 v[40:41], vcc, %[c2_3], %[zp8], v[40:41]\n"
+        "v_mad_u64_u32 v[40:41], vcc, %[c2_4], %[zp7], v[40:41]\n"
+        "v_mad_u64_u32 v[40:41], vcc, %[c2_5], %[zp6], v[40:41]\n"
+        "v_mad_u64_u32 v[40:41], vcc, %[c2_6], %[zp5], v[40:41]\n"
+        "v_mad_u64_u32 v[40:41], vcc, %[c2_7], %[zp4], v[40:41]\n"
+        "v_mad_u64_u32 v[40:41], vcc, %[c2_8], %[zp3], v[40:41]\n"
+        "v_mad_u64_u32 v[40:41], vcc, %[c3_3], %[z18], v[40:41]\n"
+        "v_mad_u64_u32 v[40:41], vcc, %[c3_4], %[z17], v[40:41]\n"
+        "v_mad_u64_u32 v[40:41], vcc, %[c3_5], %[z16], v[40:41]\n"
+        "v_mad_u64_u32 v[40:41], vcc, %[c3_6], %[z15], v[40:41]\n"
+        "v_mad_u64_u32 v[40:41], vcc, %[c3_7], %[z14], v[40:41]\n"
+        "v_mad_u64_u32 v[40:41], vcc, %[c3_8], %[z13], v[40:41]\n"
+        "v_mad_u64_u32 v[40:41], vcc, %[m3], %[p8], v[40:41]\n"
+        "v_mad_u64_u32 v[40:41], vcc, %[m4], %[p7], v[40:41]\n"
+        "v_mad_u64_u32 v[40:41], vcc, %[m5], %[p6], v[40:41]\n"
+        "v_mad_u64_u32 v[40:41], vcc, %[m6], %[p5], v[40:41]\n"
+        "v_mad_u64_u32 v[40:41], vcc, %[m7], %[p4], v[40:41]\n"
+        "v_mad_u64_u32 v[40:41], vcc, %[m8], %[p3], v[40:41]\n"
+        "v_mad_u64_u32 v[40:41], vcc, %[zp2], 1, v[40:41]\n"
+        "v_and_b32_e32 %[wp2], 0x1fffffff, v40\n"
+        "v_lshrrev_b64 v[40:41], 29, v[40:41]\n"
+        "v_mad_u64_u32 v[38:39], vcc, %[x4_4], %[x8], v[38:39]\n"
+        "v_mad_u64_u32 v[38:39], vcc, %[x4_5], %[x7], v[38:39]\n"
+        "v_mad_u64_u32 v[38:39], vcc, %[x4_6], %[x6], v[38:39]\n"
+        "v_mad_u64_u32 v[38:39], vcc, %[x4_7], %[x5], v[38:39]\n"
+        "v_mad_u64_u32 v[38:39], vcc, %[x4_8], %[x4], v[38:39]\n"
+        "v_mad_u64_u32 v[38:39], vcc, %[q4], %[p8], v[38:39]\n"
+        "v_mad_u64_u32 v[38:39], vcc, %[q5], %[p7], v[38:39]\n"
+        "v_mad_u64_u32 v[38:39], vcc, %[q6], %[p6], v[38:39]\n"
+        "v_mad_u64_u32 v[38:39], vcc, %[q7], %[p5], v[38:39]\n"
+        "v_mad_u64_u32 v[38:39], vcc, %[q8], %[p4], v[38:39]\n"
+        "v_and_b32_e32 %[zp3], 0x1fffffff, v38\n"
+        "v_lshrrev_b64 v[38:39], 29, v[38:39]\n"
+        "v_mad_u64_u32 v[40:41], vcc, %[c0_4], %[w8], v[40:41]\n"
+        "v_mad_u64_u32 v[40:41], vcc, %[c0_5], %[w7], v[40:41]\n"
+        "v_mad_u64_u32 v[40:41], vcc, %[c0_6], %[w6], v[40:41]\n"
+        "v_mad_u64_u32 v[40:41], vcc, %[c0_7], %[w5], v[40:41]\n"
+        "v_mad_u64_u32 v[40:41], vcc, %[c0_8], %[w4], v[40:41]\n"
+        "v_mad_u64_u32 v[40:41], vcc, %[c1_4], %[wp8], v[40:41]\n"
+        "v_mad_u64_u32 v[40:41], vcc, %[c1_5], %[wp7], v[40:41]\n"
+        "v_mad_u64_u32 v[40:41], vcc, %[c1_6], %[wp6], v[40:41]\n"
+        "v_mad_u64_u32 v[40:41], vcc, %[c1_7], %[wp5], v[40:41]\n"
+        "v_mad_u64_u32 v[40:41], vcc, %[c1_8], %[wp4], v[40:41]\n"
+        "v_mad_u64_u32 v[40:41], vcc, %[c2_4], %[zp8], v[40:41]\n"
+        "v_mad_u64_u32 v[40:41], vcc, %[c2_5], %[zp7], v[40:41]\n"
+        "v_mad_u64_u32 v[40:41], vcc, %[c2_6], %[zp6], v[40:41]\n"
+        "v_mad_u64_u32 v[40:41], vcc, %[c2_7], %[zp5], v[40:41]\n"
+        "v_mad_u64_u32 v[40:41], vcc, %[c2_8], %[zp4], v[40:41]\n"
+        "v_mad_u64_u32 v[40:41], vcc, %[c3_4], %[z18], v[40:41]\n"
+        "v_mad_u64_u32 v[40:41], vcc, %[c3_5], %[z17], v[40:41]\n"
+        "v_mad_u64_u32 v[40:41], vcc, %[c3_6], %[z16], v[40:41]\n"
+        "v_mad_u64_u32 v[40:41], vcc, %[c3_7], %[z15], v[40:41]\n"
+        "v_mad_u64_u32 v[40:41], vcc, %[c3_8], %[z14], v[40:41]\n"
+        "v_mad_u64_u32 v[40:41], vcc, %[m4], %[p8], v[40:41]\n"
+        "v_mad_u64_u32 v[40:41], vcc, %[m5], %[p7], v[40:41]\n"
+        "v_mad_u64_u32 v[40:41], vcc, %[m6], %[p6], v[40:41]\n"
+        "v_mad_u64_u32 v[40:41], vcc, %[m7], %[p5], v[40:41]\n"
+        "v_mad_u64_u32 v[40:41], vcc, %[m8], %[p4], v[40:41]\n"
+        "v_mad_u64_u32 v[40:41], vcc, %[zp3], 1, v[40:41]\n"
+        "v_and_b32_e32 %[wp3], 0x1fffffff, v40\n"
+        "v_lshrrev_b64 v[40:41], 29, v[40:41]\n"
+        "v_mad_u64_u32 v[38:39], vcc, %[x4_5], %[x8], v[38:39]\n"
+        "v_mad_u64_u32 v[38:39], vcc, %[x4_6], %[x7], v[38:39]\n"
+        "v_mad_u64_u32 v[38:39], vcc, %[x4_7], %[x6], v[38:39]\n"
+        "v_mad_u64_u32 v[38:39], vcc, %[x4_8], %[x5], v[38:39]\n"
+        "v_mad_u64_u32 v[38:39], vcc, %[q5], %[p8], v[38:39]\n"
+        "v_mad_u64_u32 v[38:39], vcc, %[q6], %[p7], v[38:39]\n"
+        "v_mad_u64_u32 v[38:39], vcc, %[q7], %[p6], v[38:39]\n"
+        "v_mad_u64_u32 v[38:39], vcc, %[q8], %[p5], v[38:39]\n"
+        "v_and_b32_e32 %[zp4], 0x1fffffff, v38\n"
+        "v_lshrrev_b64 v[38:39], 29, v[38:39]\n"
+        "v_mad_u64_u32 v[40:41], vcc, %[c0_5], %[w8], v[40:41]\n"
+        "v_mad_u64_u32 v[40:41], vcc, %[c0_6], %[w7], v[40:41]\n"
+        "v_mad_u64_u32 v[40:41], vcc, %[c0_7], %[w6], v[40:41]\n"
+        "v_mad_u64_u32 v[40:41], vcc, %[c0_8], %[w5], v[40:41]\n"
+        "v_mad_u64_u32 v[40:41], vcc, %[c1_5], %[wp8], v[40:41]\n"
+        "v_mad_u64_u32 v[40:41], vcc, %[c1_6], %[wp7], v[40:41]\n"
+        "v_mad_u64_u32 v[40:41], vcc, %[c1_7], %[wp6], v[40:41]\n"
+        "v_mad_u64_u32 v[40:41], vcc, %[c1_8], %[wp5], v[40:41]\n"
+        "v_mad_u64_u32 v[40:41], vcc, %[c2_5], %[zp8], v[40:41]\n"
+        "v_mad_u64_u32 v[40:41], vcc, %[c2_6], %[zp7], v[40:41]\n"
+        "v_mad_u64_u32 v[40:41], vcc, %[c2_7], %[zp6], v[40:41]\n"
+        "v_mad_u64_u32 v[40:41], vcc, %[c2_8], %[zp5], v[40:41]\n"
+        "v_mad_u64_u32 v[40:41], vcc, %[c3_5], %[z18], v[40:41]\n"
+        "v_mad_u64_u32 v[40:41], vcc, %[c3_6], %[z17], v[40:41]\n"
+        "v_mad_u64_u32 v[40:41], vcc, %[c3_7], %[z16], v[40:41]\n"
+        "v_mad_u64_u32 v[40:41], vcc, %[c3_8], %[z15], v[40:41]\n"
+        "v_mad_u64_u32 v[40:41], vcc, %[m5], %[p8], v[40:41]\n"
+        "v_mad_u64_u32 v[40:41], vcc, %[m6], %[p7], v[40:41]\n"
+        "v_mad_u64_u32 v[40:41], vcc, %[m7], %[p6], v[40:41]\n"
+        "v_mad_u64_u32 v[40:41], vcc, %[m8], %[p5], v[40:41]\n"
+        "v_mad_u64_u32 v[40:41], vcc, %[zp4], 1, v[40:41]\n"
+        "v_and_b32_e32 %[wp4], 0x1fffffff, v40\n"
+        "v_lshrrev_b64 v[40:41], 29, v[40:41]\n"
+        "v_mad_u64_u32 v[38:39], vcc, %[x4_6], %[x8], v[38:39]\n"
+        "v_mad_u64_u32 v[38:39], vcc, %[x4_7], %[x7], v[38:39]\n"
+        "v_mad_u64_u32 v[38:39], vcc, %[x4_8], %[x6], v[38:39]\n"
+        "v_mad_u64_u32 v[38:39], vcc, %[q6], %[p8], v[38:39]\n"
+        "v_mad_u64_u32 v[38:39], vcc, %[q7], %[p7], v[38:39]\n"
+        "v_mad_u64_u32 v[38:39], vcc, %[q8], %[p6], v[38:39]\n"
+        "v_and_b32_e32 %[zp5], 0x1fffffff, v38\n"
+        "v_lshrrev_b64 v[38:39], 29, v[38:39]\n"
+        "v_mad_u64_u32 v[40:41], vcc, %[c0_6], %[w8], v[40:41]\n"
+        "v_mad_u64_u32 v[40:41], vcc, %[c0_7], %[w7], v[40:41]\n"
+        "v_mad_u64_u32 v[40:41], vcc, %[c0_8], %[w6], v[40:41]\n"
+        "v_mad_u64_u32 v[40:41], vcc, %[c1_6], %[wp8], v[40:41]\n"
+        "v_mad_u64_u32 v[40:41], vcc, %[c1_7], %[wp7], v[40:41]\n"
+        "v_mad_u64_u32 v[40:41], vcc, %[c1_8], %[wp6], v[40:41]\n"
+        "v_mad_u64_u32 v[40:41], vcc, %[c2_6], %[zp8], v[40:41]\n"
+        "v_mad_u64_u32 v[40:41], vcc, %[c2_7], %[zp7], v[40:41]\n"
+        "v_mad_u64_u32 v[40:41], vcc, %[c2_8], %[zp6], v[40:41]\n"
+        "v_mad_u64_u32 v[40:41], vcc, %[c3_6], %[z18], v[40:41]\n"
+        "v_mad_u64_u32 v[40:41], vcc, %[c3_7], %[z17], v[40:41]\n"
+        "v_mad_u64_u32 v[40:41], vcc, %[c3_8], %[z16], v[40:41]\n"
+        "v_mad_u64_u32 v[40:41], vcc, %[m6], %[p8], v[40:41]\n"
+        "v_mad_u64_u32 v[40:41], vcc, %[m7], %[p7], v[40:41]\n"
+        "v_mad_u64_u32 v[40:41], vcc, %[m8], %[p6], v[40:41]\n"
+        "v_mad_u64_u32 v[40:41], vcc, %[zp5], 1, v[40:41]\n"
+        "v_and_b32_e32 %[wp5], 0x1fffffff, v40\n"
+        "v_lshrrev_b64 v[40:41], 29, v[40:41]\n"
+        "v_mad_u64_u32 v[38:39], vcc, %[x4_7], %[x8], v[38:39]\n"
+        "v_mad_u64_u32 v[38:39], vcc, %[x4_8], %[x7], v[38:39]\n"
+        "v_mad_u64_u32 v[38:39], vcc, %[q7], %[p8], v[38:39]\n"
+        "v_mad_u64_u32 v[38:39], vcc, %[q8], %[p7], v[38:39]\n"
+        "v_and_b32_e32 %[zp6], 0x1fffffff, v38\n"
+        "v_lshrrev_b64 v[38:39], 29, v[38:39]\n"
+        "v_mad_u64_u32 v[40:41], vcc, %[c0_7], %[w8], v[40:41]\n"
+        "v_mad_u64_u32 v[40:41], vcc, %[c0_8], %[w7], v[40:41]\n"
+        "v_mad_u64_u32 v[40:41], vcc, %[c1_7], %[wp8], v[40:41]\n"
+        "v_mad_u64_u32 v[40:41], vcc, %[c1_8], %[wp7], v[40:41]\n"
+        "v_mad_u64_u32 v[40:41], vcc, %[c2_7], %[zp8], v[40:41]\n"
+        "v_mad_u64_u32 v[40:41], vcc, %[c2_8], %[zp7], v[40:41]\n"
+        "v_mad_u64_u32 v[40:41], vcc, %[c3_7], %[z18], v[40:41]\n"
+        "v_mad_u64_u32 v[40:41], vcc, %[c3_8], %[z17], v[40:41]\n"
+        "v_mad_u64_u32 v[40:41], vcc, %[m7], %[p8], v[40:41]\n"
+        "v_mad_u64_u32 v[40:41], vcc, %[m8], %[p7], v[40:41]\n"
+        "v_mad_u64_u32 v[40:41], vcc, %[zp6], 1, v[40:41]\n"
+        "v_and_b32_e32 %[wp6], 0x1fffffff, v40\n"
+        "v_lshrrev_b64 v[40:41], 29, v[40:41]\n"
+        "v_mad_u64_u32 v[38:39], vcc, %[x4_8], %[x8], v[38:39]\n"
+        "v_mad_u64_u32 v[38:39], vcc, %[q8], %[p8], v[38:39]\n"
+        "v_and_b32_e32 %[zp7], 0x1fffffff, v38\n"
+        "v_mad_u64_u32 v[40:41], vcc, %[c0_8], %[w8], v[40:41]\n"
+        "v_mad_u64_u32 v[40:41], vcc, %[c1_8], %[wp8], v[40:41]\n"
+        "v_mad_u64_u32 v[40:41], vcc, %[c2_8], %[zp8], v[40:41]\n"
+        "v_mad_u64_u32 v[40:41], vcc, %[c3_8], %[z18], v[40:41]\n"
+        "v_mad_u64_u32 v[40:41], vcc, %[m8], %[p8], v[40:41]\n"
+        "v_mad_u64_u32 v[40:41], vcc, %[zp7], 1, v[40:41]\n"
+        "v_and_b32_e32 %[wp7], 0x1fffffff, v40\n"
+        "v_lshrrev_b64 v[40:41], 29, v[40:41]\n"
+        "v_alignbit_b32 %[zp8], v39, v38, 29\n"
+        "v_add_u32_e32 %[wp8], %[zp8], v40\n"
+        : [m0] "=&v"(m0), [m1] "=&v"(m1), [m2] "=&v"(m2), [m3] "=&v"(m3),
+          [m4] "=&v"(m4), [m5] "=&v"(m5), [m6] "=&v"(m6), [m7] "=&v"(m7),
+          [m8] "=&v"(m8), [q0] "=&v"(q0), [q1] "=&v"(q1), [q2] "=&v"(q2),
+          [q3] "=&v"(q3), [q4] "=&v"(q4), [q5] "=&v"(q5), [q6] "=&v"(q6),
+          [q7] "=&v"(q7), [q8] "=&v"(q8), [wp0] "+v"(wp.v[0]), [wp1] "+v"(wp.v[1]),
+          [wp2] "+v"(wp.v[2]), [wp3] "+v"(wp.v[3]), [wp4] "+v"(wp.v[4]), [wp5] "+v"(wp.v[5]),
+          [wp6] "+v"(wp.v[6]), [wp7] "+v"(wp.v[7]), [wp8] "+v"(wp.v[8]), [zp0] "+v"(zp.v[0]),
+          [zp1] "+v"(zp.v[1]), [zp2] "+v"(zp.v[2]), [zp3] "+v"(zp.v[3]), [zp4] "+v"(zp.v[4]),
+          [zp5] "+v"(zp.v[5]), [zp6] "+v"(zp.v[6]), [zp7] "+v"(zp.v[7]), [zp8] "+v"(zp.v[8])
+        : [c0_0] "s"(c[0].v[0]), [c0_1] "s"(c[0].v[1]), [c0_2] "s"(c[0].v[2]), [c0_3] "s"(c[0].v[3]),
+          [c0_4] "s"(c[0].v[4]), [c0_5] "s"(c[0].v[5]), [c0_6] "s"(c[0].v[6]), [c0_7] "s"(c[0].v[7]),
+          [c0_8] "s"(c[0].v[8]), [c1_0] "s"(c[1].v[0]), [c1_1] "s"(c[1].v[1]), [c1_2] "s"(c[1].v[2]),
+          [c1_3] "s"(c[1].v[3]), [c1_4] "s"(c[1].v[4]), [c1_5] "s"(c[1].v[5]), [c1_6] "s"(c[1].v[6]),
+          [c1_7] "s"(c[1].v[7]), [c1_8] "s"(c[1].v[8]), [c2_0] "s"(c[2].v[0]), [c2_1] "s"(c[2].v[1]),
+          [c2_2] "s"(c[2].v[2]), [c2_3] "s"(c[2].v[3]), [c2_4] "s"(c[2].v[4]), [c2_5] "s"(c[2].v[5]),
+          [c2_6] "s"(c[2].v[6]), [c2_7] "s"(c[2].v[7]), [c2_8] "s"(c[2].v[8]), [c3_0] "s"(c[3].v[0]),
+          [c3_1] "s"(c[3].v[1]), [c3_2] "s"(c[3].v[2]), [c3_3] "s"(c[3].v[3]), [c3_4] "s"(c[3].v[4]),
+          [c3_5] "s"(c[3].v[5]), [c3_6] "s"(c[3].v[6]), [c3_7] "s"(c[3].v[7]), [c3_8] "s"(c[3].v[8]),
+          [w0] "v"(w.v[0]), [w1] "v"(w.v[1]), [w2] "v"(w.v[2]), [w3] "v"(w.v[3]),
+          [w4] "v"(w.v[4]), [w5] "v"(w.v[5]), [w6] "v"(w.v[6]), [w7] "v"(w.v[7]),
+          [w8] "v"(w.v[8]), [z10] "v"(z1.v[0]), [z11] "v"(z1.v[1]), [z12] "v"(z1.v[2]),
+          [z13] "v"(z1.v[3]), [z14] "v"(z1.v[4]), [z15] "v"(z1.v[5]), [z16] "v"(z1.v[6]),
+          [z17] "v"(z1.v[7]), [z18] "v"(z1.v[8]), [x4_0] "v"(x4.v[0]), [x4_1] "v"(x4.v[1]),
+          [x4_2] "v"(x4.v[2]), [x4_3] "v"(x4.v[3]), [x4_4] "v"(x4.v[4]), [x4_5] "v"(x4.v[5]),
+          [x4_6] "v"(x4.v[6]), [x4_7] "v"(x4.v[7]), [x4_8] "v"(x4.v[8]), [x0] "v"(x.v[0]),
+          [x1] "v"(x.v[1]), [x2] "v"(x.v[2]), [x3] "v"(x.v[3]), [x4] "v"(x.v[4]),
+          [x5] "v"(x.v[5]), [x6] "v"(x.v[6]), [x7] "v"(x.v[7]), [x8] "v"(x.v[8]),
+          [p0] "s"(p29(0)), [p1] "s"(p29(1)), [p2] "s"(p29(2)), [p3] "s"(p29(3)),
+          [p4] "s"(p29(4)), [p5] "s"(p29(5)), [p6] "s"(p29(6)), [p7] "s"(p29(7)),
+          [p8] "s"(p29(8)), [n0] "s"(N0INV32)
+        : "vcc", "v38", "v39", "v40", "v41");
+}
+
+}
+}
+}
```

Result: no change. 3.717 million, median of 6 (+0.3%).
